# microsoft/ISLE

Hardware: AMD Instinct MI355X
Metric: docs/sec end-to-end ISLETrain (SVD+k-means), k=1000; top-k σ rel-err (higher is better)
Workload: dtype f32

## Files before the change

include/isle_hip.h:

```cpp
#ifndef ISLE_HIP_H
#define ISLE_HIP_H

#include <stddef.h>
#include <stdint.h>

#ifdef __cplusplus
extern "C" {
#endif

typedef struct isle_ctx isle_ctx;

enum {
  ISLE_OK = 0,
  ISLE_E_ARG = -1,
  ISLE_E_HIP = -2,
  ISLE_E_NOCONV = -3,
  ISLE_E_NUMERIC = -4,
  ISLE_E_COMM = -5
};

isle_ctx* isle_hip_create(int device_id);
void isle_hip_destroy(isle_ctx* ctx);
const char* isle_hip_last_error(isle_ctx* ctx);

int isle_hip_comm_unique_id(void* out128);
int isle_hip_comm_init(isle_ctx* ctx, int world_size, int rank, const void* unique_id128);

enum { ISLE_XCHG_ALLREDUCE_SUM = 0, ISLE_XCHG_ALLREDUCE_MAX = 1, ISLE_XCHG_ALLGATHER = 2 };
typedef int (*isle_host_exchange_fn)(void* user, int kind, void* buf, uint64_t count, int dtype);
int isle_hip_comm_init_host(isle_ctx* ctx, int world_size, int rank, isle_host_exchange_fn fn, void* user);

int isle_hip_plan_shards(uint64_t num_docs, const int64_t* offsets_CSC, int parts, uint64_t* bounds);

int isle_hip_upload_csc_u64(isle_ctx* ctx, uint64_t vocab_size, uint64_t num_docs, uint64_t nnz,
                            const float* vals, const uint64_t* rows, const int64_t* offsets,
                            uint64_t doc_offset, uint64_t docs_global);
int isle_hip_upload_csc_u32(isle_ctx* ctx, uint64_t vocab_size, uint64_t num_docs, uint64_t nnz,
                            const float* vals, const uint32_t* rows, const int64_t* offsets,
                            uint64_t doc_offset, uint64_t docs_global);

int isle_hip_upload_counts_u32(isle_ctx* ctx, uint64_t vocab_size, uint64_t num_docs, uint64_t nnz,
                               const float* counts, const uint32_t* rows, const int64_t* offsets,
                               uint64_t doc_offset, uint64_t docs_global);

int isle_hip_ingest_tdf(isle_ctx* ctx, const char* text, uint64_t nbytes, uint64_t vocab_size, uint64_t num_docs,
                        uint64_t max_entries, uint64_t* entries_read, uint64_t* nnz);
int isle_hip_get_A(isle_ctx* ctx, float* counts, uint32_t* rows, int64_t* offsets);

int isle_hip_threshold(isle_ctx* ctx, uint64_t num_topics, double sample_rate, uint64_t sample_seed,
                       uint64_t* docs_kept, uint64_t* nnz_kept, uint64_t* entries_above_threshold,
                       float* avg_doc_sz);

int isle_hip_get_B(isle_ctx* ctx, float* vals, uint32_t* rows, int64_t* offsets,
                   uint64_t* original_cols, float* zetas);
int isle_hip_shape(isle_ctx* ctx, uint64_t* vocab_size, uint64_t* num_docs, uint64_t* nnz,
                   uint64_t* doc_offset, uint64_t* docs_global);

int isle_hip_frobenius(isle_ctx* ctx, float* out);

int isle_hip_gram_apply(isle_ctx* ctx, const float* X_colmajor, int b, float* Z_colmajor);

int isle_hip_operator_form(isle_ctx* ctx, int* form);

int isle_hip_switch_info(int index, const char** name, const char** kind, const char** what);

int isle_hip_block_ks(isle_ctx* ctx, int nev, int ncv, int maxit, int blk, float tol, uint64_t seed,
                      float* evals, int* nconv, int* restarts, int* napplies);

int isle_hip_block_ks_dense(isle_ctx* ctx, const float* A_colmajor, uint64_t n, int nev, int ncv, int maxit, int blk,
                            float tol, uint64_t seed, const float* start_block, float* evals, float* U_colmajor,
                            int* nconv, int* nconv_ref_rule, int* restarts, int* napplies);

int isle_hip_get_U(isle_ctx* ctx, float* U_colmajor);
int isle_hip_set_U(isle_ctx* ctx, const float* U_colmajor, int k);

int isle_hip_eig_sym(isle_ctx* ctx, const float* S_colmajor, int n, float* evals_desc, float* vecs_colmajor);

int isle_hip_kmeanspp_projected(isle_ctx* ctx, int k, const uint64_t* inject_seeds, uint64_t rng_seed,
                                uint64_t* seeds_out, float* C_lowd, float* residual, int* rounds);

int isle_hip_host_rand(uint64_t seed, int n, uint32_t* out);

int isle_hip_get_min_dist(isle_ctx* ctx, float* min_dist);

int isle_hip_lloyds_projected(isle_ctx* ctx, int k, float* C_lowd, int max_reps, int* iters_run,
                              uint32_t* assign_out);

int isle_hip_lift_centers(isle_ctx* ctx, const float* in, int ld_in, int ncols, float* centers);

int isle_hip_lloyds_sparse(isle_ctx* ctx, int k, const float* centers_in, float* centers_out,
                           uint32_t* assign, int max_reps, int* iters_run);

int isle_hip_catchwords(isle_ctx* ctx, int num_topics, const uint32_t* assign, uint64_t r, double rho,
                        float* thresholds, int32_t* catch_topic, uint64_t* num_catchwords);

int isle_hip_topic_model(isle_ctx* ctx, int num_topics, uint64_t rank_threshold, float* model,
                         float* model_threshold, int32_t* top1, int32_t* top2, uint64_t* doc_topic_sums);
int isle_hip_get_doc_topic_sums(isle_ctx* ctx, int64_t* doc_offsets, uint32_t* topic, float* val);

int isle_hip_edge_topics(isle_ctx* ctx, const int64_t* pairs, int n, float primary_ratio, float* edge);

int isle_hip_topic_coherence(isle_ctx* ctx, int num_topics, int M, const uint32_t* top_words, double eps, double* coherence,
                             uint64_t* doc_freq, uint64_t* co_doc_freq);

int isle_hip_avg_topic_model(isle_ctx* ctx, int num_topics, float* model);

#define ISLE_MODEL_CATCH 0
#define ISLE_MODEL_AVG 1
#define ISLE_MODEL_HOST 2
#define ISLE_MODEL_LOADED 3

int isle_hip_model_top_words(isle_ctx* ctx, int which, const float* model_host, uint64_t vocab, int ncols, int n, uint32_t* ids, float* weights);

int isle_hip_topic_diversity(isle_ctx* ctx, int which, int num_topics, double* dist, double* avg);

#define ISLE_TEXT_SPARSE 0
#define ISLE_TEXT_DENSE 1
typedef int (*isle_text_sink_fn)(const char* bytes, uint64_t n, void* user);
int isle_hip_model_text(isle_ctx* ctx, int which, const float* model_host, uint64_t vocab, int ncols, int format, isle_text_sink_fn sink,
                        void* user, uint64_t* nbytes, uint64_t* nentries);
int isle_hip_edge_topics_text(isle_ctx* ctx, const int64_t* pairs, int n, float primary_ratio, int format, isle_text_sink_fn sink, void* user,
                              uint64_t* nbytes, uint64_t* nentries);
int isle_hip_entry_text(float w, int format, char* out16);

int isle_hip_load_model_text(isle_ctx* ctx, const char* text, uint64_t nbytes, uint64_t vocab, int ncols, int format, unsigned base,
                             uint64_t* nentries);
int isle_hip_get_loaded_model(isle_ctx* ctx, float* model_colmajor, uint64_t* vocab, int* ncols);
int isle_hip_parse_weight(const char* token, uint64_t n, int format, float* out);

int isle_hip_log_combinatorial(isle_ctx* ctx, float* out, uint64_t* max_words);

int isle_hip_distinct_top_five(isle_ctx* ctx, int n_m, const int32_t* m, uint64_t* num_distinct, uint64_t* num_quintuples, float* quintuples,
                               uint64_t* run_lengths, uint64_t* num_runs);

int isle_hip_top_five_count_rule(const uint64_t* run_lengths, uint64_t n_runs, int32_t m, uint64_t* out);

int isle_hip_infer(isle_ctx* ctx, uint64_t vocab_size, int num_topics, const float* model_by_word,
                   uint64_t num_docs, uint64_t nnz, const float* counts, const uint32_t* rows,
                   const int64_t* offsets, int iters, float Lf_guess, float avg_doc_sz, float* weights,
                   int32_t* top_topic, float* top_weight, float* llh, uint64_t* nconverged);

int isle_hip_infer_resident(isle_ctx* ctx, int which, const float* model_host, uint64_t vocab, int ncols, uint64_t doc_begin,
                            uint64_t doc_end, int iters, float Lf_guess, float min_weight, uint64_t chunk_docs, int32_t* top_topic,
                            float* top_weight, float* llh, uint64_t* nconverged, uint64_t* nentries);
int isle_hip_get_infer_entries(isle_ctx* ctx, int64_t* doc_offsets, uint32_t* topic, float* weight);
#define ISLE_DOCTEXT_ENTRIES 0
#define ISLE_DOCTEXT_TOP 1
int isle_hip_infer_text(isle_ctx* ctx, int what, uint64_t row_begin, uint64_t row_end, uint64_t number_base, isle_text_sink_fn sink,
                        void* user, uint64_t* nbytes, uint64_t* nlines);
int isle_hip_doc_line_text(uint64_t doc_number, uint64_t topic_number, float w, char* out40);
int isle_hip_avg_doc_sz(isle_ctx* ctx, float* out);

enum {
  ISLE_T_GRAM_PASS1 = 0,
  ISLE_T_GRAM_PASS2 = 1,
  ISLE_T_ORTHO = 2,
  ISLE_T_QR = 3,
  ISLE_T_EVD = 4,
  ISLE_T_ROTATE = 5,
  ISLE_T_PROJECT = 6,
  ISLE_T_KMPP = 7,
  ISLE_T_LLOYD_PROJ = 8,
  ISLE_T_SPARSE_ASSIGN = 9,
  ISLE_T_SPARSE_UPDATE = 10,
  ISLE_T_BAND_BUILD = 11,
  ISLE_T_COMM = 12,
  ISLE_T_THRESHOLD = 13,
  ISLE_T_POST = 14,
  ISLE_T_INGEST = 15,
  ISLE_T_INFER = 16,
  ISLE_T_LIFT = 17,
  ISLE_T_COUNT = 18
};
int isle_hip_timing_enable(isle_ctx* ctx, int on);
int isle_hip_timing_reset(isle_ctx* ctx);
int isle_hip_timing_get(isle_ctx* ctx, double* ms, uint64_t* launches);
int isle_hip_synchronize(isle_ctx* ctx);

#ifdef __cplusplus
}
#endif
#endif
```

isle_amd/_lib.py:

```python
import ctypes as C
import os

_HERE = os.path.dirname(os.path.abspath(__file__))
_LIB = None

_P, _I, _U64, _F = C.c_void_p, C.c_int, C.c_uint64, C.c_float
SYMBOLS = {
    "isle_hip_create": (_P, [_I]),
    "isle_hip_destroy": (None, [_P]),
    "isle_hip_last_error": (C.c_char_p, [_P]),
    "isle_hip_switch_info": (_I, [_I, _P, _P, _P]),
    "isle_hip_comm_unique_id": (_I, [_P]),
    "isle_hip_comm_init": (_I, [_P, _I, _I, _P]),
    "isle_hip_comm_init_host": (_I, [_P, _I, _I, _P, _P]),
    "isle_hip_plan_shards": (_I, [_U64, _P, _I, _P]),
    "isle_hip_upload_csc_u64": (_I, [_P, _U64, _U64, _U64, _P, _P, _P, _U64, _U64]),
    "isle_hip_upload_csc_u32": (_I, [_P, _U64, _U64, _U64, _P, _P, _P, _U64, _U64]),
    "isle_hip_upload_counts_u32": (_I, [_P, _U64, _U64, _U64, _P, _P, _P, _U64, _U64]),
    "isle_hip_ingest_tdf": (_I, [_P, _P, _U64, _U64, _U64, _U64, _P, _P]),
    "isle_hip_get_A": (_I, [_P, _P, _P, _P]),
    "isle_hip_threshold": (_I, [_P, _U64, C.c_double, _U64, _P, _P, _P, _P]),
    "isle_hip_get_B": (_I, [_P, _P, _P, _P, _P, _P]),
    "isle_hip_shape": (_I, [_P, _P, _P, _P, _P, _P]),
    "isle_hip_catchwords": (_I, [_P, _I, _P, _U64, C.c_double, _P, _P, _P]),
    "isle_hip_topic_model": (_I, [_P, _I, _U64, _P, _P, _P, _P, _P]),
    "isle_hip_get_doc_topic_sums": (_I, [_P, _P, _P, _P]),
    "isle_hip_edge_topics": (_I, [_P, _P, _I, _F, _P]),
    "isle_hip_topic_coherence": (_I, [_P, _I, _I, _P, C.c_double, _P, _P, _P]),
    "isle_hip_avg_topic_model": (_I, [_P, _I, _P]),
    "isle_hip_model_top_words": (_I, [_P, _I, _P, _U64, _I, _I, _P, _P]),
    "isle_hip_topic_diversity": (_I, [_P, _I, _I, _P, _P]),
    "isle_hip_model_text": (_I, [_P, _I, _P, _U64, _I, _I, _P, _P, _P, _P]),
    "isle_hip_edge_topics_text": (_I, [_P, _P, _I, _F, _I, _P, _P, _P, _P]),
    "isle_hip_entry_text": (_I, [_F, _I, _P]),
    "isle_hip_load_model_text": (_I, [_P, _P, _U64, _U64, _I, _I, C.c_uint, _P]),
    "isle_hip_get_loaded_model": (_I, [_P, _P, _P, _P]),
    "isle_hip_parse_weight": (_I, [_P, _U64, _I, _P]),
    "isle_hip_log_combinatorial": (_I, [_P, _P, _P]),
    "isle_hip_distinct_top_five": (_I, [_P, _I, _P, _P, _P, _P, _P, _P]),
    "isle_hip_top_five_count_rule": (_I, [_P, _U64, C.c_int32, _P]),
    "isle_hip_frobenius": (_I, [_P, _P]),
    "isle_hip_gram_apply": (_I, [_P, _P, _I, _P]),
    "isle_hip_operator_form": (_I, [_P, _P]),
    "isle_hip_infer": (_I, [_P, C.c_uint64, _I, _P, C.c_uint64, C.c_uint64, _P, _P, _P, _I, C.c_float, C.c_float, _P, _P, _P, _P, _P]),
    "isle_hip_infer_resident": (_I, [_P, _I, _P, _U64, _I, _U64, _U64, _I, _F, _F, _U64, _P, _P, _P, _P, _P]),
    "isle_hip_get_infer_entries": (_I, [_P, _P, _P, _P]),
    "isle_hip_infer_text": (_I, [_P, _I, _U64, _U64, _U64, _P, _P, _P, _P]),
    "isle_hip_doc_line_text": (_I, [_U64, _U64, _F, _P]),
    "isle_hip_avg_doc_sz": (_I, [_P, _P]),
    "isle_hip_block_ks": (_I, [_P, _I, _I, _I, _I, _F, _U64, _P, _P, _P, _P]),
    "isle_hip_block_ks_dense": (_I, [_P, _P, _U64, _I, _I, _I, _I, _F, _U64, _P, _P, _P, _P, _P, _P, _P]),
    "isle_hip_get_U": (_I, [_P, _P]),
    "isle_hip_set_U": (_I, [_P, _P, _I]),
    "isle_hip_eig_sym": (_I, [_P, _P, _I, _P, _P]),
    "isle_hip_kmeanspp_projected": (_I, [_P, _I, _P, _U64, _P, _P, _P, _P]),
    "isle_hip_get_min_dist": (_I, [_P, _P]),
    "isle_hip_host_rand": (_I, [_U64, _I, _P]),
    "isle_hip_lloyds_projected": (_I, [_P, _I, _P, _I, _P, _P]),
    "isle_hip_lift_centers": (_I, [_P, _P, _I, _I, _P]),
    "isle_hip_lloyds_sparse": (_I, [_P, _I, _P, _P, _P, _I, _P]),
    "isle_hip_timing_enable": (_I, [_P, _I]),
    "isle_hip_timing_reset": (_I, [_P]),
    "isle_hip_timing_get": (_I, [_P, _P, _P]),
    "isle_hip_synchronize": (_I, [_P]),
}


class IsleHipError(RuntimeError):
    pass


def library_path():
    return os.environ.get("ISLE_HIP_LIB") or os.path.join(_HERE, "libisle_hip.so")


def load_library():
    global _LIB
    if _LIB is not None:
        return _LIB
    path = library_path()
    if not os.path.exists(path):
        raise IsleHipError(
            "%s not found — build it with `make -C isle_amd/csrc` (or __graft_entry__.build()). "
            "There is no CPU fallback for the ISLE hot path." % path)
    lib = C.CDLL(path)
    for name, (res, args) in SYMBOLS.items():
        fn = getattr(lib, name)
        fn.restype = res
        fn.argtypes = args
    _LIB = lib
    return lib
```

isle_amd/csrc/api_kmeans.cpp:

```cpp
#include <algorithm>
#include <chrono>
#include <cmath>
#include <cstdarg>
#include <cstdlib>
#include <cstring>
#include <numeric>

#include "api_internal.h"

#ifndef ISLE_PROJ_FULL_NUM
#define ISLE_PROJ_FULL_NUM 1
#define ISLE_PROJ_FULL_DEN 3
#endif
static void choose_movers(const std::vector<float>& delta, int k, int group, int G, YyMovers* mv, std::vector<float>* gmax_excl,
                          const std::vector<uint32_t>* slot_of_id = nullptr ) {
  mv->n = 0;
  if ((int)delta.size() != k || k <= 16) return;
  std::vector<int> ord(k);
  std::iota(ord.begin(), ord.end(), 0);
  std::partial_sort(ord.begin(), ord.begin() + 11, ord.end(), [&](int a, int b) { return delta[a] > delta[b] || (delta[a] == delta[b] && a < b); });
  const float ref = delta[ord[10]];
  for (int j = 0; j < 10; ++j)
    if (delta[ord[j]] > 2.0f * ref && delta[ord[j]] > 1e-4f) mv->id[mv->n++] = (uint32_t)ord[j];
  if (!mv->n) return;
// ... 182 lines not shown
    else ISLECHK(kmpp_draw_by_ranks(c, rng, ndraw, inject != nullptr, dice, st, &grand, &last_md));
    new_added = 0;
    std::vector<uint64_t> fresh;
    for (int cc = 0; cc < ndraw && (int)centers.size() < k; ++cc) {
      const uint64_t nc = inject ? inject[centers.size()] : st.drawn[cc];
      if (std::find(centers.begin(), centers.end(), nc) == centers.end()) {
        centers.push_back(nc);
        fresh.push_back(nc);
        new_added++;
      }
    }
    if (new_added) ISLECHK(fetch_rows(c, fresh.data(), new_added, c->Cdev.p + (centers.size() - new_added) * (size_t)ldk));
    if (inject && new_added == 0) return isle_fail(c, ISLE_E_ARG, "injected seeds contain duplicates");
    if (rounds > 100 * k) return isle_fail(c, ISLE_E_NUMERIC, "k-means++ cannot find %d distinct seeds", k);
  }
  isle_host_mark("kmeanspp: rounds done");
  if (plan.track && c->kmpp_track && new_added > 0 && c->kmpp_track_seeds == k - new_added && D > 0) {
    HIPCHK(c, c->kmpp_best.reserve(D));
    HIPCHK(c, hipMemcpyAsync(c->kmpp_best.p, c->min_dist.p, D * sizeof(float), hipMemcpyDeviceToDevice, c->stream));
    ISLECHK(k_kmpp_update(c, c->P.p, c->pnorm.p, D, k, ldk, c->Cdev.p + (size_t)(k - new_added) * ldk, new_added, c->kmpp_best.p, k - new_added, true));
  }
  const size_t ch_bytes = (size_t)k * ldk * sizeof(float);
  HIPCHK(c, c->pin_stage.reserve(ch_bytes));
  HIPCHK(c, hipMemcpyAsync(c->pin_stage.p, c->Cdev.p, ch_bytes, hipMemcpyDeviceToHost, c->stream));
  HIPCHK(c, hipStreamSynchronize(c->stream));
  std::copy(centers.begin(), centers.end(), seeds_out);
  centres_unpack(C_lowd, reinterpret_cast<const float*>(c->pin_stage.p), k, ldk);
  if (residual) *residual = (float)(grand - last_md);
  if (rounds_out) *rounds_out = rounds;
  if (plan.track && c->kmpp_track && c->kmpp_track_seeds == k) {
    c->kmpp_C_host.assign(C_lowd, C_lowd + (size_t)k * k);
    c->kmpp_P_gen = c->P_gen;
    c->kmpp_track_k = k;
  }
  isle_host_mark("kmeanspp: exit");
  return 0;
}

extern "C" int isle_hip_get_min_dist(isle_ctx* c, float* out) {
  if (!c || !out) return ISLE_E_ARG;
  ISLECHK(isle_enter(c));
  if (c->D) HIPCHK(c, hipMemcpy(out, c->min_dist.p, c->D * sizeof(float), hipMemcpyDeviceToHost));
  return 0;
}

namespace {
struct StopRule {
  isle_ctx* c;
  int k;
  std::vector<long long> prev_sizes;
  bool have_prev = false;
  StopRule(isle_ctx* c_, int k_) : c(c_), k(k_), prev_sizes(k_, 0) {}
  int converged(const std::vector<long long>& sizes, const uint32_t* assign, bool* out) {
    bool changed = false;
    for (int i = 0; i < k; ++i)
      if (prev_sizes[i] != sizes[i]) changed = true;
    prev_sizes = sizes;
    if (!changed) {
      if (!have_prev) {
        changed = c->D_global > 0;
      } else {
        HIPCHK(c, c->flags.reserve(16));
        ISLECHK(k_compare_u32(c, assign, c->assign_prev.p, c->D, c->flags.p));
        ISLECHK(allreduce_sum<int>(c, c->flags.p, 1));
        uint32_t differ = 0;
        ISLECHK(isle_fetch_u32(c, reinterpret_cast<const uint32_t*>(c->flags.p), &c->pin_small()->stop_flag, &differ));
        changed = differ != 0;
      }
      HIPCHK(c, c->assign_prev.reserve(c->D ? c->D : 1));
      if (c->D) HIPCHK(c, hipMemcpyAsync(c->assign_prev.p, assign, c->D * sizeof(uint32_t), hipMemcpyDeviceToDevice, c->stream));
      have_prev = true;
    }
    *out = !changed;
    return 0;
  }
};
}

static int fetch_sizes(isle_ctx* c, int k, std::vector<long long>& sizes) {
  ISLECHK(allreduce_sum<int>(c, c->counts.p, k));
  std::vector<int> hv;
  int* h = c->pin_small()->cluster_sizes;
  if ((size_t)k * sizeof(int) > sizeof(c->pin_small()->cluster_sizes)) {
    hv.resize(k);
    h = hv.data();
  }
  HIPCHK(c, hipMemcpyAsync(h, c->counts.p, (size_t)k * sizeof(int), hipMemcpyDeviceToHost, c->stream));
  HIPCHK(c, hipStreamSynchronize(c->stream));
  sizes.assign(h, h + k);
  return 0;
}

static int fetch_delta(isle_ctx* c, const float* delta_dev, int k, std::vector<float>& out) {
  out.resize(k);
  float* h = c->pin_small()->movements;
  if ((size_t)k * sizeof(float) > sizeof(c->pin_small()->movements)) {
    HIPCHK(c, hipStreamSynchronize(c->stream));
    HIPCHK(c, hipMemcpy(out.data(), delta_dev, (size_t)k * sizeof(float), hipMemcpyDeviceToHost));
    return 0;
  }
  HIPCHK(c, hipMemcpyAsync(h, delta_dev, (size_t)k * sizeof(float), hipMemcpyDeviceToHost, c->stream));
  HIPCHK(c, hipStreamSynchronize(c->stream));
  memcpy(out.data(), h, (size_t)k * sizeof(float));
  return 0;
}

static int prepare_movers(isle_ctx* c, const std::vector<float>& delta, int k, int group, int G, const std::vector<uint32_t>* slot_of_id, YyMovers* mv,
                          std::vector<float>* excl) {
  choose_movers(delta, k, group, G, mv, excl, slot_of_id);
  if (!mv->n) return 0;
  HIPCHK(c, c->yy_gmax2.reserve(std::max(G, 64)));
  HIPCHK(c, hipMemcpyAsync(c->yy_gmax2.p, excl->data(), (size_t)G * sizeof(float), hipMemcpyHostToDevice, c->stream));
  return 0;
}

namespace {
struct ProjPlan {
  bool hamerly;
  bool tiles;
  int T, TL;
  bool from_kmpp;
  bool pt_sorted;
  bool delta_sums;
  bool movers;
};
struct ProjScalars {
  float* delta;
  HamTop* top;
  float* tmove;
};
}

static ProjPlan proj_plan(isle_ctx* c, int k, const float* C_lowd) {
  ProjPlan p;
  p.hamerly = !c->knob_on(KN_NO_HAMERLY) && (c->Pt_ready || c->Pt2_ready);
  p.T = (k + 31) / 32;
  p.TL = (p.T + 3) & ~3;
  p.tiles = p.hamerly && k > 224 && p.T <= 32 && !c->knob_is(KN_PROJ_BOUNDS, "hamerly");
  p.from_kmpp = p.tiles && c->kmpp_track_k == k && c->kmpp_P_gen == c->P_gen && c->P_ready && !c->knob_zero(KN_KMPP_TRACK) &&
                c->kmpp_C_host.size() == (size_t)k * k && memcmp(c->kmpp_C_host.data(), C_lowd, (size_t)k * k * sizeof(float)) == 0;
  p.pt_sorted = !c->knob_zero(KN_PT_SORT);
  p.delta_sums = !c->knob_is(KN_PROJ_SUMS, "fresh") && c->D < (1ull << 31);
  p.movers = !c->knob_zero(KN_YY_MOVERS) && c->D > 0;
  return p;
}

static int proj_reserve(isle_ctx* c, const ProjPlan& p, int k, ProjScalars* sc) {
  const uint64_t D = c->D;
  const int ldk = c->ldk;
  if (p.hamerly) {
    HIPCHK(c, c->hub.reserve(D ? D : 1));
    HIPCHK(c, c->hlb.reserve(D ? D : 1));
    HIPCHK(c, c->active.reserve(D + 1));
    HIPCHK(c, c->Pa.reserve((size_t)(D ? D : 1) * ldk));
    HIPCHK(c, c->pna.reserve(D ? D : 1));
    HIPCHK(c, c->Cold.reserve((size_t)k * ldk + k + 8));
  }
  if (p.tiles) {
    HIPCHK(c, c->ptlb.reserve((size_t)(D ? D : 1) * p.TL));
    HIPCHK(c, c->pneed.reserve(D ? D : 1));
    HIPCHK(c, c->pcand.reserve(D + 1));
    HIPCHK(c, c->small.reserve(4096));
  }
  if (p.delta_sums) HIPCHK(c, c->proj_counted.reserve(D ? D : 1));
  if (c->multi()) HIPCHK(c, c->Csum_local.reserve((size_t)k * ldk));
  sc->delta = p.hamerly ? c->Cold.p + (size_t)k * ldk : nullptr;
  sc->top = p.hamerly ? reinterpret_cast<HamTop*>(c->Cold.p + (size_t)k * ldk + round4(k)) : nullptr;
  sc->tmove = p.tiles ? c->small.p : nullptr;
  return 0;
}

static int proj_assign_first(isle_ctx* c, const ProjPlan& p, int k) {
  const uint64_t D = c->D;
  const int ldk = c->ldk;
  if (p.from_kmpp) return k_kmpp_to_tiles(c, D, k, c->pnorm.p, c->cnorm.p, c->kmpp_best.p, c->assign.p, c->hub.p, p.TL);
  if (p.tiles)
    return k_proj_assign_tiles(c, c->P.p, c->pnorm.p, D, k, ldk, c->Cdev.p, c->cnorm.p, c->assign.p, c->hub.p, c->ptlb.p, p.TL, nullptr, 0, nullptr, nullptr,
                               nullptr);
  return k_proj_assign(c, c->P.p, c->pnorm.p, D, k, ldk, c->Cdev.p, c->cnorm.p, c->assign.p, p.hamerly ? c->hub.p : nullptr,
                       p.hamerly ? c->hlb.p : nullptr);
}

static int debug_tile_stats(isle_ctx* c, int it, uint32_t na, int T) {
  const uint64_t D = c->D;
  std::vector<uint32_t> act(na), need(D);
  if (na) HIPCHK(c, hipMemcpy(act.data(), c->active.p, na * sizeof(uint32_t), hipMemcpyDeviceToHost));
  if (D) HIPCHK(c, hipMemcpy(need.data(), c->pneed.p, D * sizeof(uint32_t), hipMemcpyDeviceToHost));
  if (na > 256 && !c->knob_zero(KN_PT_SORT))
    std::stable_sort(act.begin(), act.end(), [&](uint32_t a, uint32_t b) { return need[a] < need[b]; });
  double tiles_sum = 0, union_sum = 0;
  for (uint32_t i = 0; i < na; i += 128) {
    uint32_t u = 0;
    for (uint32_t j = i; j < std::min(na, i + 128); ++j) {
      tiles_sum += __builtin_popcount(need[act[j]]);
      u |= need[act[j]];
    }
    union_sum += __builtin_popcount(u);
  }
  fprintf(stderr, "[tile bounds, projected] iter %d active %u of %llu, tiles per document %.1f, per workgroup (union) %.1f of %d\n", it, na,
          (unsigned long long)D, na ? tiles_sum / na : 0.0, na ? union_sum / ((na + 127) / 128) : 0.0, T);
  return 0;
}

static int proj_reassign_tiles(isle_ctx* c, const ProjPlan& p, const ProjScalars& sc, int k, int it, const std::vector<float>& pdelta_host) {
  const uint64_t D = c->D;
  const int ldk = c->ldk, T = p.T, TL = p.TL;
  uint32_t* nact = c->active.p + D;
  uint32_t* ncand = c->pcand.p + D;
  YyMovers mv;
  const float* tmove_use = sc.tmove;
  if (p.movers && c->gl_mode == 1 && c->band_ready && c->U_k == k) {
    std::vector<float> tm;
    ISLECHK(prepare_movers(c, pdelta_host, k, 32, T, nullptr, &mv, &tm));
    if (mv.n) {
      HIPCHK(c, c->Tmp.reserve((size_t)c->V * 32 + (size_t)16 * ldk));
      float* Cm = c->Tmp.p + (size_t)c->V * 32;
      for (int j = 0; j < mv.n; ++j)
        HIPCHK(c, hipMemcpyAsync(Cm + (size_t)j * ldk, c->Cdev.p + (size_t)mv.id[j] * ldk, (size_t)ldk * sizeof(float), hipMemcpyDeviceToDevice, c->stream));
      HIPCHK(c, hipStreamSynchronize(c->stream));
      HIPCHK(c, c->yy_mdots.reserve((size_t)D * mv.ld));
      ISLECHK(k_gemm_nn(c, c->Ucm.p, c->V, k, Cm, ldk, mv.n, c->Tmp.p, ISLE_T_LLOYD_PROJ));
      {
        TimeScope ts(c, ISLE_T_LLOYD_PROJ);
        ISLECHK(k_gl_thin(c, c->Tmp.p, mv.n, mv.ld, c->yy_mdots.p, true));
      }
      tmove_use = c->yy_gmax2.p;
    }
  }
  ISLECHK(k_pt_filter(c, p.pt_sorted ? nullptr : (c->members_valid ? c->members.p : nullptr), c->assign.p, c->hub.p, c->ptlb.p, T, TL, sc.delta, tmove_use,
                      c->pneed.p, c->pcand.p, ncand, mv, c->yy_mdots.p, c->cnorm.p, c->pnorm.p));
  ISLECHK(k_pt_tighten(c, c->P.p, c->pnorm.p, ldk, c->Cdev.p, c->cnorm.p, c->assign.p, c->pcand.p, ncand, c->hub.p, c->ptlb.p, T, TL, c->pneed.p,
                       c->active.p, nact));
  uint32_t na = 0;
  ISLECHK(isle_fetch_u32(c, nact, &c->pin_small()->active_count, &na));
  if (c->knob_on(KN_DEBUG_HAMERLY)) ISLECHK(debug_tile_stats(c, it, na, T));
  if ((uint64_t)na * ISLE_PROJ_FULL_DEN > (uint64_t)D * ISLE_PROJ_FULL_NUM && k_proj_full_by_gemm(c, D, k))
    return k_proj_assign_tiles(c, c->P.p, c->pnorm.p, D, k, ldk, c->Cdev.p, c->cnorm.p, c->assign.p, c->hub.p, c->ptlb.p, TL, nullptr, 0, nullptr, nullptr,
                               nullptr);
  return k_proj_assign_tiles(c, c->P.p, c->pnorm.p, D, k, ldk, c->Cdev.p, c->cnorm.p, c->assign.p, c->hub.p, c->ptlb.p, TL, c->active.p, na, c->pneed.p, c->Pa.p,
                             c->pna.p);
}

static int proj_reassign_hamerly(isle_ctx* c, const ProjScalars& sc, int k, int it) {
  uint32_t* nact = c->active.p + c->D;
  ISLECHK(k_hamerly_filter(c, nullptr, c->assign.p, c->hub.p, c->hlb.p, sc.delta, sc.top, c->active.p, nact, ISLE_T_LLOYD_PROJ));
  uint32_t na = 0;
  ISLECHK(isle_fetch_u32(c, nact, &c->pin_small()->active_count, &na));
  if (c->knob_on(KN_DEBUG_HAMERLY)) fprintf(stderr, "[hamerly, projected] iter %d active %u of %llu\n", it, na, (unsigned long long)c->D);
  return k_proj_assign_active(c, c->P.p, c->pnorm.p, k, c->ldk, c->Cdev.p, c->cnorm.p, c->active.p, na, c->Pa.p, c->pna.p, c->assign.p, c->hub.p, c->hlb.p);
}

static int proj_update_centres(isle_ctx* c, const ProjPlan& p, int k, int it, std::vector<long long>& sizes) {
  const uint64_t D = c->D;
  const int ldk = c->ldk;
  float* sums = c->multi() ? c->Csum_local.p : c->Csum.p;
  bool updated = false;
  if (p.delta_sums && it > 0) ISLECHK(k_proj_accumulate_delta(c, c->P.p, D, k, ldk, c->assign.p, c->proj_counted.p, sums, c->counts.p, &updated));
  if (!updated) {
    ISLECHK(k_proj_accumulate(c, c->P.p, D, k, ldk, c->assign.p, sums, c->counts.p));
    if (p.delta_sums && D) HIPCHK(c, hipMemcpyAsync(c->proj_counted.p, c->assign.p, D * sizeof(uint32_t), hipMemcpyDeviceToDevice, c->stream));
  } else {
    c->members_valid = false;
  }
  if (c->multi()) HIPCHK(c, hipMemcpyAsync(c->Csum.p, sums, (size_t)k * ldk * sizeof(float), hipMemcpyDeviceToDevice, c->stream));
  ISLECHK(allreduce_sum<float>(c, c->Csum.p, (size_t)k * ldk));
  ISLECHK(fetch_sizes(c, k, sizes));
  if (p.hamerly) HIPCHK(c, hipMemcpyAsync(c->Cold.p, c->Cdev.p, (size_t)k * ldk * sizeof(float), hipMemcpyDeviceToDevice, c->stream));
  return k_proj_finalize(c, c->Csum.p, c->counts.p, k, ldk, c->Cdev.p);
}

static int proj_movements(isle_ctx* c, const ProjPlan& p, const ProjScalars& sc, int k, std::vector<float>& pdelta_host) {
  ISLECHK(k_rownorms_diff(c, c->Cdev.p, c->Cold.p, k, k, c->ldk, sc.delta));
  if (!p.tiles) return k_ham_delta(c, sc.delta, k, sc.top);
  ISLECHK(k_yy_delta(c, sc.delta, k, p.T, 32, sc.tmove));
  return fetch_delta(c, sc.delta, k, pdelta_host);
}

extern "C" int isle_hip_lloyds_projected(isle_ctx* c, int k, float* C_lowd, int max_reps, int* iters_run, uint32_t* assign_out) {
  if (!c || !C_lowd || k < 1) return ISLE_E_ARG;
  ISLECHK(isle_enter(c));
  isle_host_mark("lloyds_projected: entry");
  ISLECHK(ensure_P(c, k));
  const ProjPlan plan = proj_plan(c, k, C_lowd);
  const uint64_t D = c->D;
  const int ldk = c->ldk;
  HIPCHK(c, c->Cdev.reserve((size_t)k * ldk));
  HIPCHK(c, c->Csum.reserve((size_t)k * ldk));
  HIPCHK(c, c->cnorm.reserve(k));
  HIPCHK(c, c->counts.reserve(k));
  HIPCHK(c, c->assign.reserve(D ? D : 1));
  c->assign_valid = false;
  const size_t ch_bytes = (size_t)k * ldk * sizeof(float);
  HIPCHK(c, c->pin_stage.reserve(ch_bytes));
  float* Ch = reinterpret_cast<float*>(c->pin_stage.p);
  centres_pack(Ch, C_lowd, k, ldk);
  HIPCHK(c, hipMemcpyAsync(c->Cdev.p, Ch, ch_bytes, hipMemcpyHostToDevice, c->stream));
  HIPCHK(c, hipStreamSynchronize(c->stream));
  isle_host_mark("lloyds_projected: centres uploaded");
  ProjScalars sc;
  ISLECHK(proj_reserve(c, plan, k, &sc));
  c->kmpp_track_k = 0;
  if (c->knob_on(KN_DEBUG_HAMERLY)) fprintf(stderr, "[projected Lloyd] first assignment %s\n", plan.from_kmpp ? "taken from the k-means++ rounds" : "computed");
  StopRule stop(c, k);
  int it = 0;
  std::vector<float> pdelta_host;
  isle_host_mark("lloyds_projected: loop starts");
  for (; it < max_reps; ++it) {
    ISLECHK(k_rownorms(c, c->Cdev.p, k, k, ldk, c->cnorm.p));
    if (it == 0 || !plan.hamerly) ISLECHK(proj_assign_first(c, plan, k));
    else if (plan.tiles) ISLECHK(proj_reassign_tiles(c, plan, sc, k, it, pdelta_host));
    else ISLECHK(proj_reassign_hamerly(c, sc, k, it));
    ISLECHK(k_count_sizes(c, c->assign.p, D, k, c->counts.p));
    std::vector<long long> sizes;
    ISLECHK(proj_update_centres(c, plan, k, it, sizes));
    if (plan.hamerly && it + 1 < max_reps) ISLECHK(proj_movements(c, plan, sc, k, pdelta_host));
    bool conv = false;
    ISLECHK(stop.converged(sizes, c->assign.p, &conv));
    if (conv) {
      ++it;
      break;
    }
  }
  isle_host_mark("lloyds_projected: loop done");
  HIPCHK(c, hipMemcpyAsync(Ch, c->Cdev.p, ch_bytes, hipMemcpyDeviceToHost, c->stream));
  if (assign_out && D) HIPCHK(c, hipMemcpyAsync(assign_out, c->assign.p, D * sizeof(uint32_t), hipMemcpyDeviceToHost, c->stream));
  HIPCHK(c, hipStreamSynchronize(c->stream));
  centres_unpack(C_lowd, Ch, k, ldk);
  if (iters_run) *iters_run = it;
  isle_host_mark("lloyds_projected: exit");
  return 0;
}

static int install_centers(isle_ctx* c, int ncols) {
  const int ld = round4(ncols);
  HIPCHK(c, c->centers_rm.reserve((size_t)c->V * ld));
  HIPCHK(c, hipMemsetAsync(c->centers_rm.p, 0, (size_t)c->V * ld * sizeof(float), c->stream));
  ISLECHK(k_transpose(c, c->centers_cm.p, c->V, ncols, c->V, c->centers_rm.p, ld));
  c->centers_ready = true;
  c->centers_k = ncols;
  return 0;
}

extern "C" int isle_hip_lift_centers(isle_ctx* c, const float* in, int ld_in, int ncols, float* centers) {
  if (!c || !in || ncols < 1) return ISLE_E_ARG;
  ISLECHK(isle_enter(c));
  if (c->U_k == 0 || ld_in < c->U_k) return isle_fail(c, ISLE_E_ARG, "lift: need U and ld_in >= k");
  isle_host_mark("lift: entry");
  HIPCHK(c, c->Csum.reserve((size_t)ld_in * ncols));
  {
    const size_t in_bytes = (size_t)ld_in * ncols * sizeof(float);
    HIPCHK(c, c->pin_stage.reserve(in_bytes));
    memcpy(c->pin_stage.p, in, in_bytes);
    HIPCHK(c, hipMemcpyAsync(c->Csum.p, c->pin_stage.p, in_bytes, hipMemcpyHostToDevice, c->stream));
  }
  HIPCHK(c, c->centers_cm.reserve((size_t)c->V * ncols));
  ISLECHK(k_gemm_nn(c, c->Ucm.p, c->V, c->U_k, c->Csum.p, ld_in, ncols, c->centers_cm.p, ISLE_T_LIFT));
  ISLECHK(install_centers(c, ncols));
  HIPCHK(c, c->lift_C.reserve((size_t)ld_in * ncols));
  HIPCHK(c, hipMemcpyAsync(c->lift_C.p, c->Csum.p, (size_t)ld_in * ncols * sizeof(float), hipMemcpyDeviceToDevice, c->stream));
  c->lift_ld = ld_in;
  c->lift_k = ncols;
  c->lift_valid = true;
  if (centers) HIPCHK(c, hipMemcpyAsync(centers, c->centers_cm.p, (size_t)c->V * ncols * sizeof(float), hipMemcpyDeviceToHost, c->stream));
  HIPCHK(c, hipStreamSynchronize(c->stream));
  isle_host_mark("lift: exit");
  return 0;
}

namespace {
struct SparsePlan {
  bool hamerly , yinyang;
  int G;
  int yy_mode;
  bool fused;
  bool by_members;
  bool fused_first;
  bool via_projection;
  bool regroup;
  bool movers;
};
struct SparseScalars {
  float* delta;
  float* cn_max;
  HamTop* top;
  float* gmax;
};
struct SparseGroups {
  YyMap ymap;
  std::vector<uint32_t> slot_of_id_host;
};
}
static SparseScalars sparse_scalars(isle_ctx* c, int k) {
  return {c->Csum.p, c->Csum.p + 2 * k + 8, reinterpret_cast<HamTop*>(c->Csum.p + 2 * k + 12), c->Csum.p + 2 * k + 16};
}

static bool first_scratch_had(isle_ctx* c, int k) {
  if (c->dotsT.reserve((size_t)c->D * k) == hipSuccess) return true;
  (void)hipGetLastError();
  fprintf(stderr, "[isle_hip] lloyds_sparse: no memory for the %.1f GB product of the first assignment; taking the sparse route\n",
          (double)c->D * k * sizeof(float) / 1e9);
  return false;
}

static SparsePlan sparse_plan(isle_ctx* c, int k, int ld) {
  const uint64_t D = c->D;
  SparsePlan p;
  p.hamerly = !c->knob_on(KN_NO_HAMERLY) && !c->knob_is(KN_KMEANS_BOUNDS, "none");
  p.yinyang = p.hamerly && !c->knob_is(KN_KMEANS_BOUNDS, "hamerly");
  p.G = (k + 7) / 8;
  int yy_mode_env = -1;
  if (const char* e = c->knob(KN_YY_MODE)) yy_mode_env = !strcmp(e, "doc") ? 0 : !strcmp(e, "docg") ? 1 : !strcmp(e, "group") ? 2 : -1;
  p.yy_mode = !p.yinyang ? 0 : p.G > 256 ? 0 : yy_mode_env >= 0 ? yy_mode_env : (p.G >= 32 ? 2 : 0);
  p.fused = p.yy_mode == 2 && !c->knob_zero(KN_YY_FUSED);
  const char* yord = c->knob(KN_YY_ORDER);
  p.by_members = !p.yinyang || !p.yy_mode || (yord ? strcmp(yord, "doc") != 0 : !p.fused);
  p.movers = p.fused && !c->knob_zero(KN_YY_MOVERS);
  const double t_dense = 2.0 * (double)D * k * k / 130e12, t_sparse = (double)((k + 7) / 8) * (double)c->nnz * 2.8e-12;
  p.fused_first = p.yinyang && k_gemm_assign_fused_ok(c, D, k, k);
  const bool dense_pays = k <= 384 || (t_dense < t_sparse && (p.fused_first || isle_scratch_ok(c, c->dotsT.cap, (double)D * k * sizeof(float))));
  p.via_projection = c->lift_valid && c->lift_k == k && c->U_k == k && c->P_ready && (c->Pt_ready || c->Pt2_ready) && c->ldk == ld && D > 0 &&
                     (dense_pays || c->knob_is(KN_FIRST_ASSIGN, "projection")) && !c->knob_is(KN_FIRST_ASSIGN, "sparse");
  p.regroup = p.yinyang && p.yy_mode == 2 && p.via_projection && p.fused_first && !c->knob_zero(KN_YY_REGROUP);
  return p;
}

static int sparse_regroup_tables(isle_ctx* c, int k, int G, SparseGroups* g) {
  TimeScope ts(c, ISLE_T_SPARSE_ASSIGN);
  float* cn_pin = c->pin_small()->centre_norms;
  HIPCHK(c, hipMemcpyAsync(cn_pin, c->cnorm.p, (size_t)k * sizeof(float), hipMemcpyDeviceToHost, c->stream));
  HIPCHK(c, hipStreamSynchronize(c->stream));
  std::vector<float> cnh(cn_pin, cn_pin + k);
  std::vector<uint32_t> id_of_slot((size_t)8 * G, 0xffffffffu);
  std::iota(id_of_slot.begin(), id_of_slot.begin() + k, 0u);
  std::stable_sort(id_of_slot.begin(), id_of_slot.begin() + k, [&](uint32_t a, uint32_t b) { return cnh[a] < cnh[b]; });
  g->slot_of_id_host.assign(k, 0u);
  for (int s2 = 0; s2 < k; ++s2) g->slot_of_id_host[id_of_slot[s2]] = (uint32_t)s2;
  ISLECHK(k_yy_map_upload(c, id_of_slot.data(), g->slot_of_id_host.data(), k, G, &g->ymap));
  HIPCHK(c, c->yy_cns.reserve((size_t)8 * G));
  return 0;
}

static int sparse_assign_first_via_projection(isle_ctx* c, const SparsePlan& p, const SparseScalars& sc, int k, int ld, const YyMap& ymap, const float* cn_grp) {
  const uint64_t D = c->D;
  TimeScope ts(c, ISLE_T_SPARSE_ASSIGN);
  if (p.yinyang && p.fused_first) {
    ISLECHK(k_max_f32(c, c->cnorm.p, k, sc.cn_max));
    const float* liftC = c->lift_C.p;
    if (p.regroup) {
      HIPCHK(c, c->yy_liftC.reserve((size_t)k * c->lift_ld));
      ISLECHK(k_yy_rows_by_slot(c, ymap, k, c->lift_C.p, c->lift_ld, c->yy_liftC.p));
      liftC = c->yy_liftC.p;
    }
    ISLECHK(k_gemm_assign_yy(c, c->Pt_ready ? c->Pt.p : nullptr, c->P.p, c->ldk, c->pnorm.p, D, k, liftC, c->lift_ld, k, p.G, cn_grp, c->dnorm.p, sc.cn_max,
                             c->assign.p, c->hub.p, c->yglb.p, ISLE_T_SPARSE_ASSIGN, c->Pt2_ready ? c->Pt2.p : nullptr,
                             c->Pt2_ready && c->Pt2_pos ? c->dperm.p : nullptr));
    if (p.regroup) ISLECHK(k_yy_labels_to_ids(c, ymap, c->assign.p, D));
    return 0;
  }
  HIPCHK(c, c->dotsT.reserve((size_t)D * k));
  ISLECHK(k_ensure_pt(c));
  ISLECHK(k_gemm_nn_assign(c, c->Pt.p, D, k, c->lift_C.p, c->lift_ld, k, c->dotsT.p, ISLE_T_SPARSE_ASSIGN));
  if (p.yinyang) {
    ISLECHK(k_max_f32(c, c->cnorm.p, k, sc.cn_max));
    return k_dots_assign_cm(c, c->dotsT.p, k, p.G, c->cnorm.p, c->dnorm.p, sc.cn_max, c->assign.p, c->hub.p, c->yglb.p);
  }
  c->P_ready = false;
  c->Pt_ready = false;
  c->Pt2_ready = false;
  if (ld != k) HIPCHK(c, hipMemsetAsync(c->P.p, 0, (size_t)D * ld * sizeof(float), c->stream));
  ISLECHK(k_transpose(c, c->dotsT.p, D, (uint64_t)k, D, c->P.p, (uint64_t)ld));
  return k_dots_assign(c, k, ld, c->cnorm.p, c->dnorm.p, c->assign.p, c->hub.p, c->hlb.p, 0);
}

static int debug_yy_margins(isle_ctx* c, int it, int G, const YyMap& ymap) {
  unsigned long long hh[16];
  ISLECHK(k_yy_dbg_margins(c, c->active.p, c->active.p + c->D, c->assign.p, c->hub.p, c->yglb.p, G, ymap, hh));
  fprintf(stderr, "[yinyang] iter %d active by (ub - smallest group bound) < 1e-6 | 1e-5 | 1e-4 | 1e-3 | 1e-2 | 1e-1 | 1 | more:  own group", it);
  for (int b = 0; b < 8; ++b) fprintf(stderr, " %llu", hh[b]);
  fprintf(stderr, ";  another group");
  for (int b = 0; b < 8; ++b) fprintf(stderr, " %llu", hh[8 + b]);
  fprintf(stderr, "\n");
  return 0;
// ... 206 lines not shown
```

isle_amd/csrc/common.h:

```cpp
#pragma once
#include <hip/hip_runtime.h>
#include <rccl/rccl.h>

#include <atomic>
#include <cstdint>
#include <cstdio>
#include <functional>
#include <string>
#include <thread>
#include <vector>

struct IsleLaunchRefused {
  const char* file = nullptr;
  int line = 0;
  unsigned long long threads = 0;
};
inline IsleLaunchRefused& isle_launch_refused() {
  static thread_local IsleLaunchRefused r;
  return r;
}
inline bool isle_launch_fits(dim3 g, dim3 b, const char* file, int line) {
  const unsigned long long blocks = (unsigned long long)g.x * g.y * g.z, threads = blocks * ((unsigned long long)b.x * b.y * b.z);
  if (threads < (1ull << 32)) return true;
  IsleLaunchRefused& r = isle_launch_refused();
// ... 116 lines not shown
  const char* knob(int id) const { return knob_set[id] ? knob_val[id].c_str() : nullptr; }
  bool knob_on(int id) const { return knob_set[id]; }
  bool knob_is(int id, const char* v) const { return knob_set[id] && knob_val[id] == v; }
  bool knob_zero(int id) const { return knob_set[id] && atoi(knob_val[id].c_str()) == 0; }
  int device = 0;
  size_t total_mem = 0;
  hipStream_t stream = nullptr;
  std::string err;
  int num_cus = 256;

  char* pin = nullptr;
  PinBuf pin_stage;
  static constexpr size_t PIN_MAIL = 0, PIN_MAIL_SLOT = 1u << 20, PIN_SMALL = 2u << 20, PIN_BYTES = (2u << 20) + (256u << 10);
  IslePinSmall* pin_small() const { return reinterpret_cast<IslePinSmall*>(pin + PIN_SMALL); }

  ncclComm_t comm = nullptr;
  int world = 1, rank = 0;
  isle_host_exchange_fn host_xchg = nullptr;
  void* host_xchg_user = nullptr;
  bool multi() const { return comm != nullptr || host_xchg != nullptr; }
  std::atomic<uint32_t> wd_issued{0};
  volatile uint32_t* wd_done = nullptr;
  std::atomic<int> comm_dead{0};
  std::atomic<bool> wd_stop{false};
  std::thread wd_thread;
  double wd_timeout_s = 300.0;

  uint64_t V = 0, D = 0, nnz = 0, doc_offset = 0, D_global = 0;
  DevBuf<float> vals;
  DevBuf<uint32_t> rows;
  DevBuf<int64_t> offs;

  uint64_t a_V = 0, a_D = 0, a_nnz = 0, a_doc_offset = 0, a_D_global = 0;
  bool a_ready = false;
  DevBuf<float> a_cnt;
  DevBuf<uint32_t> a_rows;
  DevBuf<int64_t> a_offs;
  DevBuf<uint16_t> a_q;
  DevBuf<uint32_t> a_hist;
  DevBuf<uint32_t> a_kept, a_flag;
  DevBuf<float> a_wgt;
  DevBuf<int64_t> a_off_all, a_col_of, a_scan;
  DevBuf<float> zetas;
  DevBuf<uint64_t> original_cols;
  bool b_from_threshold = false;
  float a_avg = 0.f;
  bool a_avg_valid = false;

  DevBuf<float> a_nv;
  DevBuf<int32_t> p_cluster_of;
  DevBuf<uint32_t> p_cnt, p_min, p_slot;
  DevBuf<float> p_thr;
  DevBuf<uint64_t> p_seg_id, p_seg_off, p_counters;
  DevBuf<uint32_t> p_seg_len, p_seg_rank, p_seg_cur;
  DevBuf<float> p_segvals;
  DevBuf<int32_t> p_catch;
  DevBuf<uint32_t> p_nz;
  DevBuf<int64_t> p_dts_off;
  DevBuf<uint32_t> p_dts_topic;
  DevBuf<float> p_dts_val;
  uint64_t p_dts_n = 0;
  DevBuf<int32_t> p_top1, p_top2;
  DevBuf<uint32_t> p_tcnt;
  DevBuf<int64_t> p_toff;
  DevBuf<float> p_mthr;
  DevBuf<float> p_model;
  DevBuf<uint64_t> p_avg_acc;
  DevBuf<float> p_avg_model;
  DevBuf<uint32_t> mt_sizes;
  DevBuf<uint64_t> mt_offs, mt_blk, mt_stat;
  DevBuf<unsigned char> mt_text[2];
  PinBuf mt_pin[2];
  DevBuf<int64_t> inf_off;
  DevBuf<uint32_t> inf_topic;
  DevBuf<float> inf_weight;
  DevBuf<int32_t> inf_top_topic;
  DevBuf<float> inf_top_weight;
  uint64_t inf_docs = 0, inf_n = 0;
  bool inf_valid = false;
  int p_k = 0;
  DevBuf<float> ml_model;
  uint64_t ml_V = 0;
  int ml_cols = 0;
  bool ml_ready = false;
  bool p_catch_ready = false, p_model_ready = false, p_avg_ready = false, assign_valid = false;

  bool band_ready = false;
  uint32_t band_rows = 0;
  uint32_t nbands = 0;
  uint32_t chunk_cols = 0;
  DevBuf<uint32_t> bcol;
  DevBuf<float> bval;
  DevBuf<int64_t> seg_off;
  DevBuf<float> Zpart;

  int gl_mode = -1;
  GlSide gl1, gl2;
  DevBuf<float> rowval;
  DevBuf<int> gl_flag;
  DevBuf<uint32_t> dperm, dpos, wperm, wpos;
  DevBuf<uint64_t> gl_key_a, gl_key_b;
  DevBuf<uint32_t> gl_val_a, gl_val_b;
  DevBuf<uint32_t> gl_bst;
  DevBuf<uint16_t> gl_cellcnt;
  DevBuf<uint32_t> gl_srsum, gl_sbase;
  DevBuf<uint32_t> gl_fb_cnt, gl_fb_tmp;
  DevBuf<int64_t> gl_fb_off;
  DevBuf<uint16_t> gl_scnt;
  DevBuf<uint32_t> gl_biglist;
  DevBuf<uint32_t> ccount;
  DevBuf<uint32_t> ccounted;
  DevBuf<int64_t> gl_scan;
  DevBuf<unsigned long long> gl_blocktot;
  DevBuf<uint32_t> gl_slab0, gl_nch;
  uint32_t gl_block_items = 4096;
  DevBuf<float> gl_Xs, gl_part;
  DevBuf<float> gl_pscratch;
  DevBuf<uint32_t> rs_hist;
  DevBuf<int64_t> rs_hist_off, rs_scratch;

  DevBuf<float> Xrm, Yrm, Zrm;
  DevBuf<float> Xcm, Zcm;

  DevBuf<float> basis;
  DevBuf<float> Fbuf;
  DevBuf<float> Tmp;
  DevBuf<double> part;
  DevBuf<float> coef;
  DevBuf<double> gram;
  DevBuf<double> pq_part, pq_R1;
  DevBuf<float> pq_T;
  DevBuf<int> pq_meta;
  DevBuf<float> small;
  DevBuf<double> jacW, jacV;
  DevBuf<double> jacS;
  DevBuf<float> Wf;
  DevBuf<float> evd_in;
  int U_k = 0;
  DevBuf<float> Ucm;
  DevBuf<float> Urm;
  int ldk = 0;

  DevBuf<float> P;
  DevBuf<float> pnorm;
  bool P_ready = false;
  DevBuf<float> Pt;
  DevBuf<float> dotsT;
  DevBuf<uint4> gemm_b3;
  DevBuf<float> yy_gmax2;
  DevBuf<float> yy_mdots;
  DevBuf<float> cmax_buf;
  DevBuf<uint32_t> ga_redo;
  DevBuf<float> ga_bn;
  DevBuf<float> ga_rows, ga_rown;
  bool ts_open = false;
  bool roctx_open = false;
  uint32_t ga_last_redo = 0;
  DevBuf<float> assign_part;
  DevBuf<float> lift_C;
  int lift_ld = 0, lift_k = 0;
  bool lift_valid = false;
  bool Pt_ready = false;
  DevBuf<uint4> Pt2;
  bool Pt2_ready = false;
  bool Pt2_pos = false;
  DevBuf<float> min_dist;
  DevBuf<double> cum;
  DevBuf<double> scan_blk;
  DevBuf<float> Cdev;
  DevBuf<float> cnorm;
  DevBuf<float> Csum;
  DevBuf<uint32_t> assign, assign_prev;
  DevBuf<int> counts;
  DevBuf<uint32_t> members;
  DevBuf<int> moff;
  bool members_valid = false;
  DevBuf<int> flags;
  DevBuf<float> centers_rm;
  DevBuf<float> centers_cm;
  bool centers_ready = false;
  int centers_k = 0;
  DevBuf<float> dnorm;
  DevBuf<float> hub, hlb;
  DevBuf<float> yglb;
  DevBuf<float> ptlb;
  DevBuf<uint32_t> pneed;
  DevBuf<uint32_t> pcand;
  DevBuf<int> seg_desc;
  DevBuf<float> seg_part;
  DevBuf<uint32_t> proj_counted;
  DevBuf<uint32_t> proj_nch;
  DevBuf<float> proj_dpart;
  DevBuf<float> Csum_local;
  DevBuf<uint32_t> active;
  DevBuf<unsigned long long> dbg_cnt;
  DevBuf<uint32_t> kmpp_arg;
  DevBuf<float> kmpp_m2a;
  DevBuf<float> kmpp_tmin;
  DevBuf<float> kmpp_best;
  bool kmpp_track = false;
  int kmpp_track_seeds = 0;
  int kmpp_track_k = 0;
  uint64_t P_gen = 0, kmpp_P_gen = 0;
  std::vector<float> kmpp_C_host;
  DevBuf<float> yy_cg;
  DevBuf<uint32_t> yy_map;
  DevBuf<float> yy_cns;
  DevBuf<float> yy_liftC;
  DevBuf<uint32_t> yy_own, yy_res;
  DevBuf<unsigned long long> yy_need;
  DevBuf<uint32_t> yy_cnt, yy_off;
  DevBuf<uint8_t> yy_pgrp;
  DevBuf<float> centers_old;
  DevBuf<float> Pa, pna, Cold;

  hipEvent_t ks_ev[2] = {nullptr, nullptr};
  hipEvent_t ks_ev_ready[2] = {nullptr, nullptr};
  hipStream_t copy_stream = nullptr;
  DevBuf<float> ks_mail;
  DevBuf<float> ks_top;
  DevBuf<float> ks_gather;

  std::vector<std::pair<const void*, int>> lds_attr;
  bool td_persist_failed = false;

  bool timing = false;
  uint32_t timing_mask = 0xffffffffu;
  std::vector<isle_event_pair> ev_used;
  std::vector<isle_event_pair> ev_free;
  double t_ms[ISLE_T_COUNT] = {0};
  uint64_t t_n[ISLE_T_COUNT] = {0};
};

static_assert(sizeof(IslePinSmall) <= isle_ctx::PIN_BYTES - isle_ctx::PIN_SMALL, "the small page-locked region holds every slot");

int isle_fail(isle_ctx* c, int code, const char* fmt, ...);
void isle_trim_derived(isle_ctx* c, uint64_t D, uint64_t nnz);
int isle_max_lds(isle_ctx* c, const void* fn, int bytes);
bool isle_scratch_ok(isle_ctx* c, size_t have_elems, double bytes);
void isle_refresh_knobs(isle_ctx* c);
int isle_enter(isle_ctx* c);
void isle_host_mark(const char* what);

#define HIPCHK(ctx, call)                                                                   \
  do {                                                                                      \
    hipError_t e__ = (call);                                                                \
    if ((ctx) && (ctx)->comm_dead.load(std::memory_order_relaxed))                          \
      return isle_fail((ctx), ISLE_E_COMM, "%s:%d: a collective did not complete within %.0f s (ISLE_COMM_TIMEOUT_S): the communicator was aborted", __FILE__, __LINE__, (ctx)->wd_timeout_s); \
    if (e__ != hipSuccess)                                                                  \
      return isle_fail((ctx), ISLE_E_HIP, "%s:%d %s -> %s", __FILE__, __LINE__, #call, hipGetErrorString(e__)); \
    if (isle_launch_refused().file) {                                                       \
      const IsleLaunchRefused r__ = isle_launch_refused();                                  \
      isle_launch_refused() = IsleLaunchRefused();                                          \
      return isle_fail((ctx), ISLE_E_ARG, "%s:%d: kernel launch of %llu threads refused (2^32 or more do not run)", r__.file, r__.line, r__.threads); \
    }                                                                                       \
  } while (0)

#define ISLECHK(call)            \
  do {                           \
    int rc__ = (call);           \
    if (rc__ != 0) return rc__;  \
  } while (0)

inline int isle_fetch_u32(isle_ctx* c, const uint32_t* dev, uint32_t* slot, uint32_t* out) {
  HIPCHK(c, hipMemcpyAsync(slot, dev, sizeof(uint32_t), hipMemcpyDeviceToHost, c->stream));
  HIPCHK(c, hipStreamSynchronize(c->stream));
  *out = *slot;
  return 0;
}

struct TimeScope {
  isle_ctx* c;
  isle_event_pair ep;
  bool on;
  bool marker = false;
  TimeScope(isle_ctx* c_, int fam);
  ~TimeScope();
};

static inline uint64_t isle_scan_scratch(uint64_t n) { return (n + 4095) / 4096 + 1; }
static inline int cdiv(long a, long b) { return (int)((a + b - 1) / b); }

enum { ISLE_DT_F32 = 0, ISLE_DT_F64 = 1, ISLE_DT_I32 = 2, ISLE_DT_U32 = 3, ISLE_DT_U64 = 4 };
int isle_allreduce(isle_ctx* c, void* buf, size_t count, int dtype, bool max_op = false);
int isle_allgather(isle_ctx* c, const void* send, void* recv, size_t count_per_rank, int dtype);
int k_pack_rm(isle_ctx* c, const float* Xcm, uint64_t V, int b, int BP, float* Xrm);
int k_unpack_cm(isle_ctx* c, const float* Zrm, uint64_t V, int b, int BP, float* Zcm);
int k_gram_pass1(isle_ctx* c, int BP);
int k_gram_pass2(isle_ctx* c, int BP);
int k_band_build(isle_ctx* c);
int k_band_build_chunked(isle_ctx* c);
int k_dots_assign(isle_ctx* c, int k, int ldk, const float* cn, const float* dn, uint32_t* assign, float* ub, float* lb, int G);
int k_dots_assign_cm(isle_ctx* c, const float* dotsT, int k, int G, const float* cn, const float* dn, const float* cn_max_dev, uint32_t* assign, float* ub,
                     float* lb);
int k_frobenius(isle_ctx* c, double* out_host);
int k_spmm_wide_project(isle_ctx* c, const float* Mrm, int k, int ldk, float* P, float* norms, void* A2pos = nullptr, bool* a2_done = nullptr);
int k_spmm_wide_assign(isle_ctx* c, const float* Mrm, int k, int ldk, const float* cn, const float* dn, uint32_t* assign,
                       const uint32_t* perm , const uint32_t* nslots = nullptr ,
                       float* ub = nullptr, float* lb = nullptr, int G = 0 );
struct YyMovers {
  int n = 0, ld = 0;
  uint32_t id[10] = {};
};
struct YyMap {
  const uint32_t* id_of_slot = nullptr;
  const uint32_t* slot_of_id = nullptr;
#if defined(__HIPCC__)
  __device__ inline uint32_t id(uint32_t s) const { return id_of_slot ? id_of_slot[s] : s; }
  __device__ inline uint32_t slot(uint32_t i) const { return slot_of_id ? slot_of_id[i] : i; }
#endif
};
int k_yy_filter_tighten(isle_ctx* c, const uint32_t* order, const uint32_t* assign, float* ub, float* glb, int G, const float* delta_dev,
                        const float* gmax_dev, uint32_t* active, uint32_t* nactive, const float* Cg, int k, int ld, const float* cn, const float* dn,
                        const float* cn_max, const YyMovers& mv, const float* Crm, const YyMap& map = YyMap(), const float* cn_by_id = nullptr);
int k_yy_map_upload(isle_ctx* c, const uint32_t* id_of_slot_host, const uint32_t* slot_of_id_host, int k, int G, YyMap* map);
int k_yy_gather_by_slot(isle_ctx* c, const YyMap& map, int k, int G, const float* cn, float* cn_slot);
int k_yy_rows_by_slot(isle_ctx* c, const YyMap& map, int k, const float* in, int ld, float* out);
int k_yy_labels_to_ids(isle_ctx* c, const YyMap& map, uint32_t* assign, uint64_t D);
int k_yy_filter(isle_ctx* c, const uint32_t* order, const uint32_t* assign, float* ub, float* glb, int G, const float* delta_dev, const float* gmax_dev,
                uint32_t* active, uint32_t* nactive);
int k_yy_dbg_margins(isle_ctx* c, const uint32_t* active, const uint32_t* nactive, const uint32_t* assign, const float* ub, const float* glb, int G,
                     const YyMap& map, unsigned long long* hist_host);
int k_yy_pack_groups(isle_ctx* c, const float* Crm, int ld, int G, const YyMap& map = YyMap());
int k_yy_scan(isle_ctx* c, const float* Crm, const float* Cg , int k, int ld, int G, const float* cn, const float* dn, const float* cn_max_dev,
              const uint32_t* active, const uint32_t* nactive, uint32_t* assign, float* ub, float* glb, unsigned long long* dbg = nullptr,
              const YyMap& map = YyMap());
int k_yy2_assign(isle_ctx* c, const float* Cg, int k, int ld, int G, const float* cn, const float* dn, const float* cn_max_dev, const uint32_t* active,
                 const uint32_t* nactive, uint32_t* assign, float* ub, float* glb, bool* done, unsigned long long* pairs_out = nullptr, bool pre_tightened = false,
                 const YyMap& map = YyMap());
struct HamTop {
  uint32_t amax;
  float d1, d2, pad;
};
int k_ham_delta(isle_ctx* c, float* delta_dev , int k, HamTop* top_dev);
int k_hamerly_filter(isle_ctx* c, const uint32_t* order, const uint32_t* assign, float* ub, float* lb, const float* delta_dev, const HamTop* top_dev,
                     uint32_t* active, uint32_t* nactive, int fam = ISLE_T_SPARSE_ASSIGN);
int k_csc_validate(isle_ctx* c, unsigned long long* err_host2);
int k_doc_norms(isle_ctx* c, float* dn);
int k_centers_from_rows(isle_ctx* c, const uint32_t* assign, int k, int ldk, float* Crm, bool first_of_run = true);
int k_pt_filter(isle_ctx* c, const uint32_t* order, const uint32_t* assign, float* ub, float* tlb, int T, int TL, const float* delta_dev,
                const float* tmove_dev, uint32_t* need, uint32_t* active, uint32_t* nactive, const YyMovers& mv, const float* mdots, const float* cn, const float* pn);
int k_pt_tighten(isle_ctx* c, const float* P, const float* pn, int ldk, const float* C, const float* cn, const uint32_t* assign, const uint32_t* cand,
                 const uint32_t* ncand, float* ub, const float* tlb, int T, int TL, uint32_t* need, uint32_t* active, uint32_t* nactive);
int k_gl_detect(isle_ctx* c);
int k_centers_counts(isle_ctx* c, const uint32_t* assign, int k, int ldk, float* Crm, bool fresh);
int k_gl_build(isle_ctx* c);
int k_gl_wide(isle_ctx* c, const float* Mrm, int k, int ld, float* Out, float* norms = nullptr ,
              void* A2pos = nullptr , bool* a2_done = nullptr);
int k_gl_thin(isle_ctx* c, const float* Wcm, int nc, int ld, float* Out, bool by_position = false);
int k_gl_apply_cm(isle_ctx* c, const float* Xcm, int b, int BP, float* Zcm);
int k_gl_panel_width(const isle_ctx* c);

int k_th_stats(isle_ctx* c, uint64_t* tokens_nz_dev);
int k_th_round_hist(isle_ctx* c, float avg, uint32_t maxv);
int k_th_zetas(isle_ctx* c, uint32_t maxv, uint64_t count_gr, uint64_t count_eq);
int k_th_count(isle_ctx* c, bool with_weights);
int k_th_drop(isle_ctx* c, const uint8_t* drop_dev);
int k_th_scans(isle_ctx* c);
int k_th_emit(isle_ctx* c, uint64_t doc_base);

int k_sort_pairs_u64(isle_ctx* c, uint64_t* key_a, uint32_t* val_a, uint64_t* key_b, uint32_t* val_b, uint64_t n, int key_bits, bool* in_a);
int k_ingest_tdf(isle_ctx* c, const unsigned char* text_dev, uint64_t n, uint64_t V, uint64_t D, uint64_t* entries_read, uint64_t* err_out);

int k_infer(isle_ctx* c, uint64_t V, int k, const float* model_by_word, uint64_t D, uint64_t nnz, const float* counts, const uint32_t* rows,
            const int64_t* offs, int iters, float Lfguess, float avg_doc_sz, float* weights, int32_t* top_topic, float* top_weight, float* llh,
            uint64_t* nconverged);
int k_infer_rowok(isle_ctx* c, const float* M, uint64_t V, int k, unsigned char* ok);
int k_infer_docs(isle_ctx* c, const float* M, int k, uint64_t D, const float* counts, const uint32_t* rows, const int64_t* offs,
                 const unsigned char* ok, uint32_t* fw, float* fa, uint32_t* nkeep, int iters, float Lfguess, float avg_doc_sz, float* weights,
                 int32_t* top_topic, float* top_weight, float* llh, unsigned int* nconverged);

int k_infer_resident(isle_ctx* c, const float* model_cm_dev, int k, uint64_t doc_begin, uint64_t doc_end, int iters, float Lfguess,
                     float avg_doc_sz, float min_weight, uint64_t chunk_docs, int32_t* top_topic, float* top_weight, float* llh,
                     uint64_t* nconverged, uint64_t* nentries);

int k_post_normalize(isle_ctx* c, float avg);
int k_post_cluster_of(isle_ctx* c, const uint32_t* assign_dev, bool identity);
int k_post_catch_thresholds(isle_ctx* c, uint32_t k, uint32_t r, const int* sizes_dev);
int k_post_find_catchwords(isle_ctx* c, uint32_t k, double rho, uint64_t* ncatch_host);
int k_post_thr_colmajor(isle_ctx* c, uint32_t k, float* out_dev);
int k_post_doc_topic_sums(isle_ctx* c, uint32_t k, uint64_t* n_out);
int k_post_model_thresholds(isle_ctx* c, uint32_t k, uint32_t rank);
int k_post_model(isle_ctx* c, uint32_t k);
int k_post_edge(isle_ctx* c, const int64_t* pairs_dev, int n, float a, float b, float* edge_dev);

constexpr uint64_t ISLE_TEXT_CHUNK_BYTES = 16ull << 20;
int k_model_text(isle_ctx* c, const float* model_dev, uint64_t V, uint64_t ncols, const int64_t* pairs_dev, float a, float b, int format,
                 isle_text_sink_fn sink, void* user, uint64_t* nbytes, uint64_t* nentries);
int k_text_pump(isle_ctx* c, const char* who, const uint64_t* offs_dev, uint64_t ntiles, uint64_t total, uint64_t group, isle_text_sink_fn sink,
                void* user, const std::function<int(uint64_t, uint64_t, unsigned char*)>& write);

int k_infer_text(isle_ctx* c, int what, uint64_t row_begin, uint64_t row_end, uint64_t base, isle_text_sink_fn sink, void* user, uint64_t* nbytes,
                 uint64_t* nlines);

int k_load_model_text(isle_ctx* c, const unsigned char* text_dev, uint64_t n, uint64_t V, uint32_t ncols, int format, unsigned base, float* model_dev,
                      uint64_t* nentries, uint64_t* err_key);

int k_coherence_counts(isle_ctx* c, const std::vector<uint32_t>& U, const std::vector<uint32_t>& part_off, const std::vector<uint32_t>& part_hi,
                       std::vector<uint32_t>& counts, int* passes);

int k_avg_model(isle_ctx* c, uint32_t k);
int k_model_top_words(isle_ctx* c, const float* model_dev, uint64_t V, uint32_t ncols, int n, uint32_t* ids_dev, float* weights_dev);
int k_topic_diversity(isle_ctx* c, const float* model_dev, uint64_t V, uint32_t k, double* dist_dev, double* abar_dev, int32_t* finite_dev,
                      uint32_t* kprime);

int k_log_combinatorial(isle_ctx* c, float* out, uint64_t* max_words);
int k_top_five_runs(isle_ctx* c, uint64_t* n_out, std::vector<uint64_t>& runs, float* tuples);

int k_ensure_pt(isle_ctx* c);
int k_vtf(isle_ctx* c, const float* Vb, uint64_t n, int m, const float* F, int b, float* coef , uint64_t ld = 0);
int k_update(isle_ctx* c, float* F, uint64_t n, int b, const float* Vb, int m, const float* coef, uint64_t ld = 0);
int k_panel_qr(isle_ctx* c, float* F, uint64_t n, int w, float* Qdst, float* R_host , int* rank_out);
int k_panel_qr_kernels(isle_ctx* c, float* F, uint64_t n, int w, float* Qdst, int* meta_dev , float* Rout_dev );
int k_randu(isle_ctx* c, float* F, uint64_t count, uint64_t seed);
int k_gemm_nn(isle_ctx* c, const float* A, uint64_t M, int K, const float* B, int ldb, int N, float* C, int family = ISLE_T_ROTATE);
int k_gemm_nn_assign(isle_ctx* c, const float* A, uint64_t M, int K, const float* B, int ldb, int N, float* C, int family);
bool k_gemm_assign_fused_ok(isle_ctx* c, uint64_t M, int K, int N);
int k_gemm_assign_yy(isle_ctx* c, const float* A, const float* Arm, int lda_rm, const float* an, uint64_t M, int K, const float* B, int ldb, int N, int G,
                     const float* cn, const float* dn, const float* cn_max, uint32_t* assign, float* ub, float* lb, int family, const void* A2 = nullptr,
                     const uint32_t* map2 = nullptr );
int k_gemm_assign_tiles(isle_ctx* c, const float* A, const float* Arm, int lda_rm, uint64_t M, int K, const float* B, int ldb, int N, int TL, const float* cn,
                        const float* pn, const float* cmax, uint32_t* assign, float* ub, float* tlb, int family, const uint32_t* map0 = nullptr,
                        const void* A2 = nullptr, const uint32_t* map2 = nullptr);
int k_gemm_split_a(isle_ctx* c, const float* A, uint64_t M, int K, void* A2);
size_t k_gemm_split_a_bytes(uint64_t M, int K);
int k_transpose(isle_ctx* c, const float* in, uint64_t rows, uint64_t cols, uint64_t ld_in, float* out, uint64_t ld_out);
int k_jacobi_eig(isle_ctx* c, const float* S_host, int n, float* evals_host, float* vecs_dev );
int k_eig_small(isle_ctx* c, const float* S_host, int n, float* evals_host, float* vecs_dev , int nvec);
int k_colnorms_rm(isle_ctx* c, const float* Mrm, uint64_t rows, int k, int ldk, float* out, const float* Sub = nullptr);
int k_scale_centers(isle_ctx* c, float* Crm, uint64_t rows, int k, int ldk, const int* counts);

int k_tridiag_eig(isle_ctx* c, const float* S_host, int n, float* evals_host, float* vecs_dev, int nvec);

int k_member_lists(isle_ctx* c, const uint32_t* assign, uint64_t D, int k, const int* counts_dev, int* max_out, std::vector<int>* counts_host = nullptr);
int k_member_lists_dev(isle_ctx* c, const uint32_t* assign, uint64_t D, int k, const int* counts_dev);
int k_yy_delta(isle_ctx* c, float* delta_dev, int k, int G, int group, float* gmax_dev, const uint32_t* id_of_slot = nullptr);
int k_max_f32(isle_ctx* c, const float* v, int n, float* out_dev);
int k_compact_rows(isle_ctx* c, const float* P, const float* pn, int ldk, const uint32_t* active, uint32_t n, float* Pa, float* pna);
int k_kmpp_update(isle_ctx* c, const float* P, const float* pn, uint64_t D, int k, int ldk, const float* newC, int nc, float* min_dist, int s_old = -1,
                  bool track = false);
int k_kmpp_to_tiles(isle_ctx* c, uint64_t D, int k, const float* pn, const float* cn, const float* best, uint32_t* assign, float* ub, int TL);
int k_scan_f2d(isle_ctx* c, const float* in, uint64_t n, double* cum );
int k_search(isle_ctx* c, const double* cum, uint64_t n, const double* dice_dev, int nd, uint64_t* out_dev);
int k_search_args(isle_ctx* c, const double* cum, uint64_t n, const double* dice_host, int nd , uint64_t* out_dev);
int k_fetch_rows(isle_ctx* c, const float* P, int ldk, const uint64_t* local_ids , int n, float* dst);
int k_pack2(isle_ctx* c, const double* a, const float* b , double* out2);
int k_search_frac(isle_ctx* c, const double* cum, uint64_t n, const float* last , const double* frac_host, int nd ,
                  uint64_t* out_dev );
int k_proj_assign(isle_ctx* c, const float* P, const float* pn, uint64_t D, int k, int ldk, const float* C, const float* cn, uint32_t* assign,
                  float* ub = nullptr, float* lb = nullptr);
int k_proj_assign_active(isle_ctx* c, const float* P, const float* pn, int k, int ldk, const float* C, const float* cn,
                         const uint32_t* active, uint32_t n, float* Pa, float* pna, uint32_t* assign, float* ub, float* lb);
bool k_proj_full_by_gemm(isle_ctx* c, uint64_t D, int k);
int k_proj_assign_tiles(isle_ctx* c, const float* P, const float* pn, uint64_t D, int k, int ldk, const float* C, const float* cn, uint32_t* assign,
                        float* ub, float* tlb, int TL, const uint32_t* active, uint32_t n, const uint32_t* need, float* Pa, float* pna);
int k_rownorms_diff(isle_ctx* c, const float* A, const float* B, int rows, int k, int ldk, float* out);
int k_rownorms(isle_ctx* c, const float* M, int rows, int k, int ldk, float* out);
int k_proj_accumulate(isle_ctx* c, const float* P, uint64_t D, int k, int ldk, const uint32_t* assign, float* Csum, int* counts);
int k_proj_accumulate_delta(isle_ctx* c, const float* P, uint64_t D, int k, int ldk, const uint32_t* assign, uint32_t* counted, float* Csum,
                            const int* counts, bool* done);
int k_proj_finalize(isle_ctx* c, const float* Csum, const int* counts, int k, int ldk, float* C);
int k_count_sizes(isle_ctx* c, const uint32_t* assign, uint64_t D, int k, int* counts);
int k_compare_u32(isle_ctx* c, const uint32_t* a, const uint32_t* b, uint64_t n, int* flag_dev);
int k_fill_f32(isle_ctx* c, float* p, uint64_t n, float v);
```

isle_amd/csrc/dense.hip:

```cpp
#include <algorithm>
#include <cstdlib>

#include "gemm_f32.h"
#include "gemm_bf16x3.h"

#include "common.h"
#include "gridbar.h"
#include "hamerly.h"

typedef float floatx16 __attribute__((ext_vector_type(16)));

constexpr int VTF_CG = 32;
constexpr int vtf_rc(int BT) { return BT <= 12 ? 1024 : (BT <= 16 ? 512 : 256); }

template <int BT>
__global__ __launch_bounds__(256) void vtf_partial_k(const float* __restrict__ Vb, uint64_t n, uint64_t ld, int m, const float* __restrict__ F,
                                                      int b, double* __restrict__ part ) {
  constexpr int VTF_RC = vtf_rc(BT);
  __shared__ float Fs[BT][VTF_RC];
  const uint64_t r0 = (uint64_t)blockIdx.x * VTF_RC;
  const int rc = (int)min((uint64_t)VTF_RC, n - r0);
  for (int idx = threadIdx.x; idx < BT * VTF_RC; idx += 256) {
    const int j = idx / VTF_RC, r = idx - j * VTF_RC;
    Fs[j][r] = (j < b && r < rc) ? F[(uint64_t)j * ld + r0 + r] : 0.f;
// ... 662 lines not shown
  HIPCHK(c, c->gemm_b3.reserve((size_t)3 * isle_gemm3::kp8_of(K) * isle_gemm3::np_of<Gemm3Huge>(N)));
  HIPCHK(c, isle_gemm3::launch<Gemm3Huge>(c->stream, A, M, K, B, ldb, N, c->gemm_b3.p, isle_gemm3::StoreC{C, M}));
  return 0;
}

constexpr float GA_ETA_TRUNC = 4.65e-5f;
static float ga_eta(int K) { return GA_ETA_TRUNC + 1.05f * 9.f * (float)((K + 15) / 16) * 5.9604645e-8f; }
struct AssignRec {
  float m1;
  uint32_t i1;
  float m2, ax, r2;
};
struct YyGroupEpi {
  static constexpr int kGroup = 8;
  const float* __restrict__ cn;
  const float* __restrict__ dn;
  const float* __restrict__ cn_max;
  float* __restrict__ lb;
  int G, nslot;
  AssignRec* __restrict__ part;
  const uint32_t* __restrict__ map;
  float eta;
  const float* __restrict__ an;
  const float* __restrict__ bmax;
  __device__ inline uint64_t doc(uint64_t m) const { return map ? map[m] : m; }
  __device__ inline float rowdata(uint64_t m) const { return dn[doc(m)]; }
  __device__ inline float dist(float dot, int col, float dnd) const { return fabsf((-2.0f * dot + cn[col]) + dnd); }
  __device__ inline float aux(int) const { return 0.f; }
  __device__ inline void group(uint64_t m, int g, float dnd, float m1, uint32_t, float, float) const {
#ifdef GA_ABLATE_LB
    if (g >= 0) return;
#endif
    const float E = ISLE_SLACK_REL * (dnd + *cn_max), sE = sqrtf(E);
    const float eps = eta > 0.f ? eta * (an[doc(m)] + *bmax) : 0.f;
    lb[doc(m) * (uint64_t)G + g] = yy_slack_down_sq(fmaxf(m1 - eps, 0.f), E, sE);
  }
  __device__ inline void slot(uint64_t m, int sl, float, float m1, uint32_t i1, float m2, float ax, float r2) const {
    part[m * (uint64_t)nslot + sl] = AssignRec{m1, i1, m2, ax, r2};
  }
};
struct AssignPick {
  float best, m2, ax, run2;
  uint32_t bidx;
};
__device__ inline AssignPick assign_pick(const AssignRec* __restrict__ part, size_t row, int nslot) {
  AssignPick p{3.4e38f, 3.4e38f, 0.f, 3.4e38f, 0xffffffffu};
  for (int sl0 = 0; sl0 < nslot; sl0 += 8) {
    AssignRec rr[8];
#pragma unroll
    for (int u = 0; u < 8; ++u) rr[u] = part[row * nslot + min(sl0 + u, nslot - 1)];
#pragma unroll
    for (int u = 0; u < 8; ++u) {
      if (sl0 + u < nslot) {
        const AssignRec r = rr[u];
        if (r.m1 < p.best) {
          p.run2 = fminf(fminf(p.run2, p.best), r.r2);
          p.best = r.m1;
          p.bidx = r.i1;
          p.m2 = r.m2;
          p.ax = r.ax;
        } else {
          p.run2 = fminf(p.run2, r.m1);
        }
      }
    }
  }
  return p;
}
__global__ __launch_bounds__(256) void yy_first_combine_k(const AssignRec* __restrict__ part, int nslot, uint32_t n, int G, const float* __restrict__ dn,
                                                          const float* __restrict__ cn_max, uint32_t* __restrict__ assign, float* __restrict__ ub,
                                                          float* __restrict__ lb, const uint32_t* __restrict__ map, float eta,
                                                          const float* __restrict__ an, const float* __restrict__ bmax,
                                                          uint32_t* __restrict__ redo, uint32_t* __restrict__ nredo) {
  const uint32_t i = blockIdx.x * 256 + threadIdx.x;
  const bool in = i < n;
  bool open = false;
  if (in) {
    const uint32_t d = map ? map[i] : i;
    const AssignPick p = assign_pick(part, i, nslot);
    const float eps = eta > 0.f ? eta * (an[d] + *bmax) : 0.f;
    const float E = ISLE_SLACK_REL * (dn[d] + *cn_max), sE = sqrtf(E);
    lb[(size_t)d * G + p.bidx / 8] = yy_slack_down_sq(fmaxf(p.m2 - eps, 0.f), E, sE);
    const float u = sqrtf(p.best + eps);
    ub[d] = u + fminf(sE, E / fmaxf(u, 1e-30f));
    assign[d] = p.bidx;
    open = eta > 0.f && p.run2 - p.best <= 2.f * eps;
  }
  if (eta > 0.f) {
    const uint32_t at = block_append_slot(open, nredo);
    if (open) redo[at] = map ? map[i] : i;
  }
}
struct TileEpi {
  static constexpr int kGroup = 32;
  const float* __restrict__ cn;
  const float* __restrict__ pn;
  const float* __restrict__ cmax;
  float* __restrict__ lb;
  int TL, nslot;
  AssignRec* __restrict__ part;
  const uint32_t* __restrict__ map;
  float eta;
  __device__ inline uint64_t doc(uint64_t m) const { return map ? map[m] : m; }
  __device__ inline float rowdata(uint64_t m) const { return pn[doc(m)]; }
  __device__ inline float dist(float dot, int col, float nd) const { return fabsf((-2.0f * dot + cn[col]) + nd); }
  __device__ inline float aux(int col) const { return cn[col]; }
  __device__ inline void group(uint64_t m, int T, float nd, float m1, uint32_t, float, float tc) const {
    float uu, ll;
    const float lo = fmaxf(m1 - eta * (nd + *cmax), 0.f);
    hamerly_store_bounds(lo, lo, nd + tc, &uu, &ll);
    lb[doc(m) * (uint64_t)TL + T] = ll;
  }
  __device__ inline void slot(uint64_t m, int sl, float, float m1, uint32_t i1, float m2, float ax, float r2) const {
    part[m * (uint64_t)nslot + sl] = AssignRec{m1, i1, m2, ax, r2};
  }
};
__global__ __launch_bounds__(256) void tiles_combine_k(const AssignRec* __restrict__ part, int nslot, uint32_t n, int TL, const float* __restrict__ pn,
                                                       const float* __restrict__ cmax_p, uint32_t* __restrict__ assign, float* __restrict__ ub,
                                                       float* __restrict__ lb, const uint32_t* __restrict__ map, float eta,
                                                       uint32_t* __restrict__ redo, uint32_t* __restrict__ nredo) {
  const uint32_t i = blockIdx.x * 256 + threadIdx.x;
  const bool in = i < n;
  bool open = false;
  if (in) {
    const uint32_t d = map ? map[i] : i;
    const AssignPick p = assign_pick(part, i, nslot);
    const float nd = pn[d];
    const float eps = eta * (nd + *cmax_p);
    assign[d] = p.bidx;
    float uu, ll, l2;
    hamerly_store_bounds(p.best + eps, fmaxf(p.m2 - eps, 0.f), nd + p.ax, &uu, &l2);
    hamerly_store_bounds(p.best + eps, p.best + eps, nd + *cmax_p, &uu, &ll);
    ub[d] = uu;
    lb[(size_t)d * TL + (p.bidx >> 5)] = l2;
    open = eta > 0.f && p.run2 - p.best <= 2.f * eps;
  }
  if (eta > 0.f) {
    const uint32_t at = block_append_slot(open, nredo);
    if (open) redo[at] = map ? map[i] : i;
  }
}
bool k_gemm_assign_fused_ok(isle_ctx* c, uint64_t M, int K, int N) {
  return !c->knob_zero(KN_GEMM_BF16X3) && !c->knob_zero(KN_GEMM_EPILOGUE) && N >= 64 && K >= 32 && (M + 255) / 256 * (uint64_t)((N + 255) / 256) >= 512 &&
         M < (1ull << 32);
}
using Gemm2Huge = isle_gemm3::Cfg<2, 2, 4, 4, 4, 16, 2>;
using Gemm2Dma = isle_gemm3::CfgDma<2, 16>;
int k_gemm_split_a(isle_ctx* c, const float* A, uint64_t M, int K, void* A2) {
  HIPCHK(c, isle_gemm3::split_a(c->stream, A, M, K, A2, Gemm2Dma::TK));
  return 0;
}
size_t k_gemm_split_a_bytes(uint64_t M, int K) { return isle_gemm3::a2_units(M, K, Gemm2Dma::TK) * 16; }
template <class MakeEpi, class Combine>
static int gemm_assign_two_pass(isle_ctx* c, const float* A, const float* Arm, int lda_rm, const float* rown, uint64_t M, int K, const float* B, int ldb, int N,
                                MakeEpi make, Combine combine, const uint32_t* map0 = nullptr ,
                                const void* A2 = nullptr ,
                                const uint32_t* map2 = nullptr ) {
  auto need_a = [&]() -> int {
    if (A) return 0;
    ISLECHK(k_ensure_pt(c));
    A = c->Pt.p;
    return 0;
  };
  const int nslot = (N + 63) / 64;
  static_assert(sizeof(AssignRec) == 20, "");
  const char* gt = c->knob(KN_GEMM_TERMS);
  const bool two = !(gt && atoi(gt) == 3) && Arm != nullptr;
  HIPCHK(c, c->gemm_b3.reserve((size_t)3 * isle_gemm3::kp8_of(K) * isle_gemm3::np_of<Gemm3Huge>(N)));
  HIPCHK(c, c->assign_part.reserve((size_t)M * nslot * 5));
  AssignRec* part = reinterpret_cast<AssignRec*>(c->assign_part.p);
  if (!two) {
    ISLECHK(need_a());
    HIPCHK(c, isle_gemm3::launch<Gemm3Huge>(c->stream, A, M, K, B, ldb, N, c->gemm_b3.p, make(part, map0, 0.f)));
    combine(part, (uint32_t)M, map0, 0.f, nullptr, nullptr);
    HIPCHK(c, hipGetLastError());
    return 0;
  }
  const float eta2 = ga_eta(K);
  HIPCHK(c, c->ga_redo.reserve(M + 1));
  uint32_t* nredo = c->ga_redo.p + M;
  HIPCHK(c, hipMemsetAsync(nredo, 0, sizeof(uint32_t), c->stream));
  if (A2 && !c->knob_zero(KN_GEMM_DMA)) {
    HIPCHK(c, isle_gemm3::launch_dma<Gemm2Dma>(c->stream, A2, M, K, B, ldb, N, c->gemm_b3.p, make(part, map2 ? map2 : map0, eta2)));
    combine(part, (uint32_t)M, map2 ? map2 : map0, eta2, c->ga_redo.p, nredo);
  } else {
    ISLECHK(need_a());
    HIPCHK(c, isle_gemm3::launch<Gemm2Huge>(c->stream, A, M, K, B, ldb, N, c->gemm_b3.p, make(part, map0, eta2)));
    combine(part, (uint32_t)M, map0, eta2, c->ga_redo.p, nredo);
  }
  HIPCHK(c, hipGetLastError());
  uint32_t n = 0;
  ISLECHK(isle_fetch_u32(c, nredo, &c->pin_small()->redo_count, &n));
  c->ga_last_redo = n;
  if (c->knob_on(KN_DEBUG_HAMERLY)) fprintf(stderr, "[assignment product] the two-term pass left %u of %llu rows open\n", n, (unsigned long long)M);
  if (n == 0) return 0;
  if ((uint64_t)n * 4 > M) {
    ISLECHK(need_a());
    HIPCHK(c, isle_gemm3::launch<Gemm3Huge>(c->stream, A, M, K, B, ldb, N, c->gemm_b3.p, make(part, map0, 0.f)));
    combine(part, (uint32_t)M, map0, 0.f, nullptr, nullptr);
    HIPCHK(c, hipGetLastError());
    return 0;
  }
  HIPCHK(c, c->ga_rows.reserve((size_t)n * lda_rm));
  HIPCHK(c, c->ga_rown.reserve(n));
  ISLECHK(k_compact_rows(c, Arm, rown, lda_rm, c->ga_redo.p, n, c->ga_rows.p, c->ga_rown.p));
  HIPCHK(c, isle_gemm3::launch<Gemm3Huge>(c->stream, c->ga_rows.p, (uint64_t)n, K, B, ldb, N, c->gemm_b3.p, make(part, c->ga_redo.p, 0.f)));
  combine(part, n, c->ga_redo.p, 0.f, nullptr, nullptr);
  HIPCHK(c, hipGetLastError());
  return 0;
}
int k_gemm_assign_yy(isle_ctx* c, const float* A, const float* Arm, int lda_rm, const float* an, uint64_t M, int K, const float* B, int ldb, int N, int G,
                     const float* cn, const float* dn, const float* cn_max, uint32_t* assign, float* ub, float* lb, int family, const void* A2,
                     const uint32_t* map2) {
  TimeScope ts(c, family);
  const int nslot = (N + 63) / 64;
  HIPCHK(c, c->ga_bn.reserve((size_t)N + 4));
  float* bmax = c->ga_bn.p + N;
  if (an) {
    ISLECHK(k_rownorms(c, B, N, K, ldb, c->ga_bn.p));
    ISLECHK(k_max_f32(c, c->ga_bn.p, N, bmax));
  }
  return gemm_assign_two_pass(
      c, A, an ? Arm : nullptr, lda_rm, an, M, K, B, ldb, N,
      [&](AssignRec* part, const uint32_t* map, float eta) { return YyGroupEpi{cn, dn, cn_max, lb, G, nslot, part, map, eta, an, bmax}; },
      [&](const AssignRec* part, uint32_t n, const uint32_t* map, float eta, uint32_t* redo, uint32_t* nredo) {
        hipLaunchKernelGGL(yy_first_combine_k, dim3(cdiv(n, 256)), dim3(256), 0, c->stream, part, nslot, n, G, dn, cn_max, assign, ub, lb, map, eta, an, bmax, redo,
                           nredo);
      },
      nullptr, A2, map2);
}
int k_gemm_assign_tiles(isle_ctx* c, const float* A, const float* Arm, int lda_rm, uint64_t M, int K, const float* B, int ldb, int N, int TL, const float* cn,
                        const float* pn, const float* cmax, uint32_t* assign, float* ub, float* tlb, int family, const uint32_t* map0, const void* A2,
                        const uint32_t* map2) {
  TimeScope ts(c, family);
  const int nslot = (N + 63) / 64;
  return gemm_assign_two_pass(
      c, A, Arm, lda_rm, pn, M, K, B, ldb, N,
      [&](AssignRec* part, const uint32_t* map, float eta) { return TileEpi{cn, pn, cmax, tlb, TL, nslot, part, map, eta}; },
      [&](const AssignRec* part, uint32_t n, const uint32_t* map, float eta, uint32_t* redo, uint32_t* nredo) {
        hipLaunchKernelGGL(tiles_combine_k, dim3(cdiv(n, 256)), dim3(256), 0, c->stream, part, nslot, n, TL, pn, cmax, assign, ub, tlb, map, eta, redo, nredo);
      },
      map0, A2, map2);
}

__global__ __launch_bounds__(256) void transpose_k(const float* __restrict__ in, uint64_t rows, uint64_t cols, uint64_t ld_in,
                                                    float* __restrict__ out, uint64_t ld_out) {
  __shared__ float t[32][33];
  const uint64_t r0 = (uint64_t)blockIdx.x * 32, c0 = (uint64_t)blockIdx.y * 32;
  const int tx = threadIdx.x & 31, ty = threadIdx.x >> 5;
  for (int yy = ty; yy < 32; yy += 8) {
    const uint64_t r = r0 + tx, cc = c0 + yy;
    t[yy][tx] = (r < rows && cc < cols) ? in[cc * ld_in + r] : 0.f;
  }
  __syncthreads();
  for (int yy = ty; yy < 32; yy += 8) {
    const uint64_t r = r0 + yy, cc = c0 + tx;
    if (r < rows && cc < cols) out[r * ld_out + cc] = t[tx][yy];
  }
}
int k_transpose(isle_ctx* c, const float* in, uint64_t rows, uint64_t cols, uint64_t ld_in, float* out, uint64_t ld_out) {
  if (rows == 0 || cols == 0) return 0;
  const uint64_t cb = cdiv(cols, 32);
  const uint64_t rows_per = std::max<uint64_t>(32, ((1ull << 31) / 256 / cb) * 32);
  for (uint64_t r0 = 0; r0 < rows; r0 += rows_per) {
    const uint64_t nr = std::min(rows_per, rows - r0);
    dim3 g((unsigned)cdiv(nr, 32), (unsigned)cb), blk(256);
    hipLaunchKernelGGL(transpose_k, g, blk, 0, c->stream, in + r0, nr, cols, ld_in, out + r0 * ld_out, ld_out);
    HIPCHK(c, hipGetLastError());
  }
  return 0;
}

int k_ensure_pt(isle_ctx* c) {
  if (c->Pt_ready) return 0;
  if (!c->P_ready || !c->D) return isle_fail(c, ISLE_E_ARG, "no projection to transpose");
  HIPCHK(c, c->Pt.reserve((size_t)c->D * c->ldk));
  ISLECHK(k_transpose(c, c->P.p, c->ldk, c->D, c->ldk, c->Pt.p, c->D));
  c->Pt_ready = true;
  return 0;
}

__device__ inline double block_sum(double v, double* sh) {
  const int lane = threadIdx.x & 63, wave = threadIdx.x >> 6;
#pragma unroll
  for (int off = 32; off > 0; off >>= 1) v += __shfl_xor(v, off);
  __syncthreads();
  if (lane == 0) sh[wave] = v;
  __syncthreads();
  double s = 0.0;
  for (int w = 0; w < (int)(blockDim.x >> 6); ++w) s += sh[w];
  return s;
}

constexpr int BJ_W = 16;
constexpr int BJ_P = 2 * BJ_W;

__device__ inline void rr_pair(int nplayers, int round, int slot, int* p, int* q) {
  const int m = nplayers - 1;
  if (slot == 0) {
    *p = nplayers - 1;
    *q = round % m;
  } else {
    *p = (round + slot) % m;
    *q = (round - slot + m) % m;
  }
}

constexpr int BJ_SCR = BJ_P * BJ_P + 8;
constexpr int BJ_ROWS = 64;

__device__ inline void bj_blocks(int nblk2, int round, int slot, int* A, int* Bk) {
  rr_pair(nblk2, round, slot, A, Bk);
  if (*A > *Bk) {
    const int x = *A;
    *A = *Bk;
    *Bk = x;
  }
}
__device__ inline int bj_col(int A, int Bk, int cc) { return cc < BJ_W ? A * BJ_W + cc : Bk * BJ_W + (cc - BJ_W); }

__global__ __launch_bounds__(256) void bj_gram_k(const double* __restrict__ W, int n, int nblk2, int round, double* __restrict__ gpart) {
  __shared__ double T[64][BJ_P + 1];
  int A, Bk;
  bj_blocks(nblk2, round, blockIdx.x, &A, &Bk);
  if (A * BJ_W >= n) return;
  const int t = threadIdx.x;
  const int gi = t >> 3, gj0 = (t & 7) * 4;
  double g0 = 0.0, g1 = 0.0, g2 = 0.0, g3 = 0.0;
  const int rbeg = blockIdx.y * BJ_ROWS, rend = min(n, rbeg + BJ_ROWS);
  for (int r0 = rbeg; r0 < rend; r0 += 64) {
    __syncthreads();
    for (int idx = t; idx < 64 * BJ_P; idx += 256) {
      const int rr = idx & 63, cc = idx >> 6;
      T[rr][cc] = W[(size_t)bj_col(A, Bk, cc) * n + r0 + rr];
    }
    __syncthreads();
#pragma unroll 8
    for (int rr = 0; rr < 64; ++rr) {
      const double a = T[rr][gi];
      g0 = fma(a, T[rr][gj0 + 0], g0);
      g1 = fma(a, T[rr][gj0 + 1], g1);
      g2 = fma(a, T[rr][gj0 + 2], g2);
      g3 = fma(a, T[rr][gj0 + 3], g3);
    }
  }
  double* G = gpart + ((size_t)blockIdx.x * gridDim.y + blockIdx.y) * (BJ_P * BJ_P) + gi * BJ_P + gj0;
  G[0] = g0;
  G[1] = g1;
  G[2] = g2;
  G[3] = g3;
}

__global__ __launch_bounds__(256) void bj_inner_k(int n, int nblk2, int round, double tol, double abs_tol, const double* __restrict__ gpart,
                                                   int nrowch, double* __restrict__ scr, unsigned int* __restrict__ rotated, int cross_only) {
  __shared__ double G[BJ_P][BJ_P + 1];
  __shared__ double Q[BJ_P][BJ_P + 1];
  __shared__ unsigned int nrot;
  int A, Bk;
  bj_blocks(nblk2, round, blockIdx.x, &A, &Bk);
  if (A * BJ_W >= n) return;
  const int t = threadIdx.x;
  double* S = scr + (size_t)blockIdx.x * BJ_SCR;
  const double* gp = gpart + (size_t)blockIdx.x * nrowch * (BJ_P * BJ_P);
  for (int idx = t; idx < BJ_P * BJ_P; idx += 256) {
    const int i = idx / BJ_P, j = idx % BJ_P;
    const int u = (i <= j) ? i * BJ_P + j : j * BJ_P + i;
    double sum = 0.0;
    for (int ch = 0; ch < nrowch; ++ch) sum += gp[(size_t)ch * (BJ_P * BJ_P) + u];
    G[i][j] = sum;
    Q[i][j] = (i == j) ? 1.0 : 0.0;
  }
  if (t == 0) nrot = 0;
  __syncthreads();
  {
    int live = 0;
    for (int idx = t; idx < BJ_P * BJ_P; idx += 256) {
      const int i = idx / BJ_P, j = idx % BJ_P;
      if (i < j && (!cross_only || (i < BJ_W && j >= BJ_W))) {
        const double a = G[i][i], b = G[j][j], g = G[i][j];
        live |= (a > 0.0 && b > 0.0 && g * g > tol * tol * a * b && fabs(g) > abs_tol) ? 1 : 0;
      }
    }
    if (!__syncthreads_or(live)) {
      if (t == 0) S[BJ_P * BJ_P] = 0.0;
      return;
    }
  }
  const int bi = t >> 4, bj = t & 15;
  unsigned int my_rot = 0;
  const int nrounds = cross_only ? BJ_W : BJ_P - 1;
// ... 308 lines not shown
```

isle_amd/csrc/gemm_bf16x3.h:

```cpp
#pragma once
#include <hip/hip_runtime.h>
#include <stdint.h>

namespace isle_gemm3 {

typedef __bf16 bf16x8 __attribute__((ext_vector_type(8)));
typedef __bf16 bf16x4 __attribute__((ext_vector_type(4)));
typedef float f32x16 __attribute__((ext_vector_type(16)));

__device__ inline void split3(float x, __bf16& x0, __bf16& x1, __bf16& x2) {
  x0 = (__bf16)x;
  const float r1 = x - (float)x0;
  x1 = (__bf16)r1;
  const float r2 = r1 - (float)x1;
  x2 = (__bf16)r2;
}

__global__ __launch_bounds__(256) void gemm3_split_b_k(const float* __restrict__ B, int ldb, int K, int N, int Kp8, int Np, bf16x8* __restrict__ B3) {
  const size_t i = (size_t)blockIdx.x * 256 + threadIdx.x;
  if (i >= (size_t)Kp8 * Np) return;
  const int q = (int)(i / Np), n = (int)(i - (size_t)q * Np);
  bf16x8 v[3];
#pragma unroll
  for (int j = 0; j < 8; ++j) {
    const int k = 8 * q + j;
    const float x = (k < K && n < N) ? B[(size_t)n * ldb + k] : 0.f;
    __bf16 t0, t1, t2;
    split3(x, t0, t1, t2);
    v[0][j] = t0;
    v[1][j] = t1;
    v[2][j] = t2;
  }
#pragma unroll
  for (int p = 0; p < 3; ++p) B3[((size_t)p * Kp8 + q) * Np + n] = v[p];
}

template <int WMT_, int WNT_, int WAVES_M_, int WAVES_N_, int OCC_, int TK_ = 16, int NP_ = 3>
struct Cfg {
  static constexpr int WMT = WMT_, WNT = WNT_, WAVES_M = WAVES_M_, WAVES_N = WAVES_N_, OCC = OCC_, TK = TK_;
  static constexpr int NP = NP_;
  static constexpr int KO = TK / 8;
  static constexpr int TM = 32 * WMT * WAVES_M, TN = 32 * WNT * WAVES_N;
  static constexpr int NT = 64 * WAVES_M * WAVES_N;
  static constexpr int A_STAGE = NP * KO * TM, B_STAGE = NP * KO * TN;
  static constexpr size_t LDS_BYTES = (size_t)2 * (A_STAGE + B_STAGE) * 16;
  static constexpr int A_UNITS = TM * (TK / 4) / NT;
  static constexpr int B_UNITS = (B_STAGE + NT - 1) / NT;
  static_assert(TM * (TK / 4) % NT == 0 && (TK == 16 || TK == 32) && (NP == 2 || NP == 3), "tile / thread counts");
};

struct StoreC {
  static constexpr int kGroup = 0;
  float* __restrict__ C;
  uint64_t ldc;
  __device__ inline void operator()(uint64_t m, int n, float v) const { C[(uint64_t)n * ldc + m] = v; }
};

struct Top2 {
  float m1, m2, ax;
  uint32_t i1;
};
__device__ inline void top2_take(Top2& t, float d, uint32_t idx, float ax) {
  if (d < t.m1) {
    t.m2 = t.m1;
    t.m1 = d;
    t.i1 = idx;
  } else {
    t.m2 = fminf(t.m2, d);
  }
  t.ax = fmaxf(t.ax, ax);
}
__device__ inline void top2_merge(Top2& t, float om1, float om2, uint32_t oi1, float oax) {
  if (om1 < t.m1 || (om1 == t.m1 && oi1 < t.i1)) {
    t.m2 = fminf(t.m1, om2);
    t.m1 = om1;
    t.i1 = oi1;
  } else {
    t.m2 = fminf(t.m2, om1);
  }
  t.ax = fmaxf(t.ax, oax);
}
__device__ inline void top2_pair(Top2& t) {
  const float om1 = __shfl_xor(t.m1, 32), om2 = __shfl_xor(t.m2, 32), oax = __shfl_xor(t.ax, 32);
  const uint32_t oi1 = (uint32_t)__shfl_xor((int)t.i1, 32);
  top2_merge(t, om1, om2, oi1, oax);
}

template <class CF, class Epi>
__device__ inline void tile_epilogue(f32x16 (&acc)[CF::WNT][CF::WMT], uint64_t m0, int n0, int wm, int wn, int l31, int h, uint64_t M, int N, const Epi& epi) {
  constexpr int TN = CF::TN, WMT = CF::WMT, WNT = CF::WNT;
  if constexpr (Epi::kGroup != 0) {
    static_assert(Epi::kGroup == 8 || Epi::kGroup == 32, "group epilogue: groups of 8 or 32 columns");
#pragma unroll
    for (int i = 0; i < WMT; ++i) {
      const uint64_t m = m0 + wm * (32 * WMT) + i * 32 + l31;
      const bool live = m < M;
      const float rd = epi.rowdata(live ? m : M - 1);
      Top2 best{3.4e38f, 3.4e38f, 0.f, 0xffffffffu};
      float run2 = 3.4e38f;
      auto fold = [&](const Top2& t) {
        if (t.m1 < best.m1) {
          run2 = fminf(fminf(run2, best.m1), t.m2);
          best = t;
        } else {
          run2 = fminf(run2, t.m1);
        }
      };
#pragma unroll
      for (int j = 0; j < WNT; ++j) {
        const int cb = n0 + wn * (32 * WNT) + j * 32;
        if (cb >= N) continue;
        float dist[16], ax[16];
#pragma unroll
        for (int r = 0; r < 16; ++r) {
          const int col = cb + 4 * h + (r & 3) + 8 * (r >> 2);
          const bool in = col < N;
          dist[r] = in ? epi.dist(acc[j][i][r], col, rd) : 3.4e38f;
          ax[r] = in ? epi.aux(col) : 0.f;
        }
        if constexpr (Epi::kGroup == 8) {
#pragma unroll
          for (int q = 0; q < 4; ++q) {
            Top2 t{3.4e38f, 3.4e38f, 0.f, 0xffffffffu};
#pragma unroll
            for (int u = 0; u < 4; ++u) {
              const int col = cb + 4 * h + u + 8 * q;
              if (col < N) top2_take(t, dist[4 * q + u], (uint32_t)col, ax[4 * q + u]);
            }
            top2_pair(t);
            if (cb + 8 * q < N) {
              if (live && h == (q & 1)) epi.group(m, (cb >> 3) + q, rd, t.m1, t.i1, t.m2, t.ax);
              fold(t);
            }
          }
        } else {
          Top2 t{3.4e38f, 3.4e38f, 0.f, 0xffffffffu};
#pragma unroll
          for (int r = 0; r < 16; ++r) {
            const int col = cb + 4 * h + (r & 3) + 8 * (r >> 2);
            if (col < N) top2_take(t, dist[r], (uint32_t)col, ax[r]);
          }
          top2_pair(t);
          if (live && h == (j & 1)) epi.group(m, cb >> 5, rd, t.m1, t.i1, t.m2, t.ax);
          fold(t);
        }
      }
      if (live && h == 0 && n0 + wn * (32 * WNT) < N) epi.slot(m, (n0 + wn * (32 * WNT)) / (32 * WNT), rd, best.m1, best.i1, best.m2, best.ax, run2);
    }
  } else {
  const bool full_n = n0 + TN <= N;
#pragma unroll
  for (int i = 0; i < WMT; ++i) {
    const uint64_t m = m0 + wm * (32 * WMT) + i * 32 + l31;
    if (m < M) {
#pragma unroll
      for (int j = 0; j < WNT; ++j) {
        const int nb = n0 + wn * (32 * WNT) + j * 32 + 4 * h;
        if (full_n) {
#pragma unroll
          for (int r = 0; r < 16; ++r) epi(m, nb + (r & 3) + 8 * (r >> 2), acc[j][i][r]);
        } else {
#pragma unroll
          for (int r = 0; r < 16; ++r) {
            const int n = nb + (r & 3) + 8 * (r >> 2);
            if (n < N) epi(m, n, acc[j][i][r]);
          }
        }
      }
    }
  }
  }
}

template <class CF, class Epi>
__global__ __launch_bounds__(CF::NT, CF::OCC) void gemm_bf16x3_k(const float* __restrict__ A, uint64_t M, int K, const bf16x8* __restrict__ B3, int Kp8,
                                                                  int Np, int N, uint32_t nMB, uint32_t nNT, Epi epi) {
  constexpr int TM = CF::TM, TN = CF::TN, NT = CF::NT, WMT = CF::WMT, WNT = CF::WNT, TK = CF::TK, KO = CF::KO, NP = CF::NP;
  extern __shared__ bf16x8 lds3[];
  bf16x8* As = lds3;
  bf16x8* Bs = lds3 + 2 * CF::A_STAGE;
  const uint32_t wg = blockIdx.x, xcd = wg & 7u, slot = wg >> 3;
  const uint32_t mb = (slot / nNT) * 8u + xcd, nt = slot % nNT;
  if (mb >= nMB) return;
  const uint64_t m0 = (uint64_t)mb * TM;
  const int n0 = (int)nt * TN;
  const int tid = threadIdx.x, lane = tid & 63, wave = tid >> 6;
  const int l31 = lane & 31, h = lane >> 5;
  const int wm = wave % CF::WAVES_M, wn = wave / CF::WAVES_M;

  uint32_t arow[CF::A_UNITS];
  int akq[CF::A_UNITS];
#pragma unroll
  for (int u = 0; u < CF::A_UNITS; ++u) {
    const int unit = tid + u * NT;
    akq[u] = unit / TM;
    const uint64_t m = m0 + (uint32_t)(unit % TM);
    arow[u] = (uint32_t)(m < M ? m : M - 1);
  }
  float ra[4 * CF::A_UNITS];
  uint4 rb[CF::B_UNITS];
  auto load_slab = [&](int k0) {
#pragma unroll
    for (int u = 0; u < CF::A_UNITS; ++u) {
#pragma unroll
      for (int t = 0; t < 4; ++t) {
        const int k = min(k0 + 4 * akq[u] + t, K - 1);
        ra[4 * u + t] = A[(uint64_t)k * M + arow[u]];
      }
    }
    const int q0 = k0 >> 3;
#pragma unroll
    for (int u = 0; u < CF::B_UNITS; ++u) {
      const int unit = min(tid + u * NT, CF::B_STAGE - 1);
      const int p = unit / (KO * TN), r = unit - p * KO * TN, q = r / TN, n = r - q * TN;
      rb[u] = *reinterpret_cast<const uint4*>(B3 + ((size_t)p * Kp8 + q0 + q) * Np + n0 + n);
    }
  };
  auto store_slab = [&](int stage) {
    char* a = reinterpret_cast<char*>(As + stage * CF::A_STAGE);
#pragma unroll
    for (int u = 0; u < CF::A_UNITS; ++u) {
      const int unit = tid + u * NT;
      const int row = unit % TM;
      bf16x4 v[3];
#pragma unroll
      for (int t = 0; t < 4; ++t) {
        __bf16 t0, t1, t2;
        split3(ra[4 * u + t], t0, t1, t2);
        v[0][t] = t0;
        v[1][t] = t1;
        v[2][t] = t2;
      }
#pragma unroll
      for (int p = 0; p < NP; ++p) *reinterpret_cast<bf16x4*>(a + ((size_t)((p * KO + (akq[u] >> 1)) * TM + row)) * 16 + (akq[u] & 1) * 8) = v[p];
    }
    uint4* b = reinterpret_cast<uint4*>(Bs + stage * CF::B_STAGE);
#pragma unroll
    for (int u = 0; u < CF::B_UNITS; ++u) {
      const int unit = tid + u * NT;
      if (unit < CF::B_STAGE) b[unit] = rb[u];
    }
  };

  f32x16 acc[WNT][WMT];
#pragma unroll
  for (int j = 0; j < WNT; ++j)
#pragma unroll
    for (int i = 0; i < WMT; ++i)
#pragma unroll
      for (int r = 0; r < 16; ++r) acc[j][i][r] = 0.f;

  const int nslab = (K + TK - 1) / TK;
  load_slab(0);
  store_slab(0);
  __syncthreads();
  for (int s = 0; s < nslab; ++s) {
    const int cur = s & 1;
    if (s + 1 < nslab) load_slab((s + 1) * TK);
    const bf16x8* a = As + cur * CF::A_STAGE + wm * (32 * WMT) + l31;
    const bf16x8* b = Bs + cur * CF::B_STAGE + wn * (32 * WNT) + l31;
#pragma unroll
    for (int ks = 0; ks < TK / 16; ++ks) {
      const int oc = 2 * ks + h;
      bf16x8 bv[WNT][NP];
#pragma unroll
      for (int j = 0; j < WNT; ++j)
#pragma unroll
        for (int p = 0; p < NP; ++p) bv[j][p] = b[(p * KO + oc) * TN + 32 * j];
#pragma unroll
      for (int pa = NP - 1; pa >= 0; --pa) {
        bf16x8 av[WMT];
#pragma unroll
        for (int i = 0; i < WMT; ++i) av[i] = a[(pa * KO + oc) * TM + 32 * i];
#pragma unroll
        for (int pb = NP - 1 - pa; pb >= 0; --pb)
#pragma unroll
          for (int i = 0; i < WMT; ++i)
#pragma unroll
            for (int j = 0; j < WNT; ++j) acc[j][i] = __builtin_amdgcn_mfma_f32_32x32x16_bf16(bv[j][pb], av[i], acc[j][i], 0, 0, 0);
      }
    }
    if (s + 1 < nslab) store_slab(cur ^ 1);
    __syncthreads();
  }

  tile_epilogue<CF, Epi>(acc, m0, n0, wm, wn, l31, h, M, N, epi);
}

inline int kp8_of(int K) { return 4 * ((K + 31) / 32); }
template <class CF>
inline int np_of(int N) { return (N + CF::TN - 1) / CF::TN * CF::TN; }

template <class CF, class Epi>
inline hipError_t launch(hipStream_t stream, const float* A, uint64_t M, int K, const float* B, int ldb, int N, void* B3, Epi epi) {
  const int Kp8 = kp8_of(K), Np = np_of<CF>(N);
  const size_t nb = (size_t)Kp8 * Np;
  hipLaunchKernelGGL(gemm3_split_b_k, dim3((unsigned)((nb + 255) / 256)), dim3(256), 0, stream, B, ldb, K, N, Kp8, Np, reinterpret_cast<bf16x8*>(B3));
  const uint32_t nMB = (uint32_t)((M + CF::TM - 1) / CF::TM), nNT = (uint32_t)(Np / CF::TN);
  const uint64_t slots = (uint64_t)((nMB + 7) / 8) * nNT;
  static bool lds_attr_set[64] = {};
  int dev = 0;
  hipError_t e = hipGetDevice(&dev);
  if (e != hipSuccess) return e;
  if (dev < 0 || dev >= 64 || !lds_attr_set[dev]) {
    e = hipFuncSetAttribute(reinterpret_cast<const void*>(&gemm_bf16x3_k<CF, Epi>), hipFuncAttributeMaxDynamicSharedMemorySize, (int)CF::LDS_BYTES);
    if (e != hipSuccess) return e;
    if (dev >= 0 && dev < 64) lds_attr_set[dev] = true;
  }
  hipLaunchKernelGGL((gemm_bf16x3_k<CF, Epi>), dim3((uint32_t)(slots * 8)), dim3(CF::NT), CF::LDS_BYTES, stream, A, M, K, reinterpret_cast<const bf16x8*>(B3), Kp8,
                     Np, N, nMB, nNT, epi);
  return hipGetLastError();
}

template <int NS_, int TK_ = 16>
struct CfgDma {
  static constexpr int NS = NS_;
  static constexpr int WMT = 2, WNT = 2, WAVES_M = 4, WAVES_N = 4, TK = TK_, KO = TK_ / 8, NP = 2, OCC = 4;
  static constexpr int TM = 256, TN = 256, NT = 1024;
  static constexpr int A_STAGE = NP * KO * TM, B_STAGE = NP * KO * TN, STAGE = A_STAGE + B_STAGE;
  static constexpr int PPW = STAGE / 64 / 16;
  static constexpr size_t LDS_BYTES = (size_t)NS * STAGE * 16;
  static_assert(TK_ == 16 || TK_ == 32, "slabs of 16 or 32");
};
inline int nslab_of(int K, int TK) { return (K + TK - 1) / TK; }
inline size_t a2_units(uint64_t M, int K, int TK = 16) { return (size_t)((M + 255) / 256) * nslab_of(K, TK) * (4 * (TK / 8)) * 256; }

__global__ __launch_bounds__(256) void gemm2_split_a_k(const float* __restrict__ A, uint64_t M, int K, int nslab, int KO, bf16x8* __restrict__ A2) {
  const uint64_t mb = blockIdx.x, m = mb * 256 + threadIdx.x;
  const int q = blockIdx.y;
  bf16x8 v0, v1;
#pragma unroll
  for (int j = 0; j < 8; ++j) {
    const int k = 8 * q + j;
    const float x = (m < M && k < K) ? A[(uint64_t)k * M + m] : 0.f;
    const __bf16 x0 = (__bf16)x;
    v0[j] = x0;
    v1[j] = (__bf16)(x - (float)x0);
  }
  const size_t base = ((mb * nslab + (size_t)(q / KO)) * (2 * KO) + (size_t)(q % KO)) * 256 + threadIdx.x;
  A2[base] = v0;
  A2[base + (size_t)KO * 256] = v1;
}
inline hipError_t split_a(hipStream_t stream, const float* A, uint64_t M, int K, void* A2, int TK = 16) {
  const int nslab = nslab_of(K, TK);
  const uint64_t nMB = (M + 255) / 256;
  if (nMB == 0) return hipSuccess;
  if (nMB >= (1ull << 31)) return hipErrorInvalidValue;
  hipLaunchKernelGGL(gemm2_split_a_k, dim3((uint32_t)nMB, (uint32_t)(nslab * (TK / 8))), dim3(256), 0, stream, A, M, K, nslab, TK / 8, reinterpret_cast<bf16x8*>(A2));
  return hipGetLastError();
}

template <class CF, class Epi>
__global__ __launch_bounds__(CF::NT) void gemm_bf16x2_dma_k(const bf16x8* __restrict__ A2, uint64_t M, int K, const bf16x8* __restrict__ B3, int Kp8, int Np,
                                                             int N, uint32_t nMB, uint32_t nNT, Epi epi) {
  constexpr int TM = CF::TM, TN = CF::TN, WMT = CF::WMT, WNT = CF::WNT, KO = CF::KO, NP = CF::NP, NS = CF::NS, TK = CF::TK, PPW = CF::PPW;
  static_assert((NS & (NS - 1)) == 0 && NS >= 2 && NS <= 4, "ring of 2 or 4 stages");
  extern __shared__ bf16x8 ldsr[];
  const uint32_t wg = blockIdx.x, xcd = wg & 7u, slot = wg >> 3;
  const uint32_t mb = (slot / nNT) * 8u + xcd, nt = slot % nNT;
  if (mb >= nMB) return;
  const uint64_t m0 = (uint64_t)mb * TM;
  const int n0 = (int)nt * TN;
  const int tid = threadIdx.x, lane = tid & 63;
  const int wave = __builtin_amdgcn_readfirstlane(tid >> 6);
  const int l31 = lane & 31, h = lane >> 5;
  const int wm = wave % CF::WAVES_M, wn = wave / CF::WAVES_M;
  const int nslab = (K + TK - 1) / TK;
  const bool mine_a = wave < 8;
  const int w8 = mine_a ? wave : wave - 8;
  const bf16x8* ga = A2 + ((size_t)mb * nslab) * CF::A_STAGE + (size_t)(w8 * PPW) * 64 + lane;
  const bf16x8* gb[PPW];
#pragma unroll
  for (int i = 0; i < PPW; ++i) {
    const int u = (w8 * PPW + i) * 64 + lane;
    gb[i] = B3 + ((size_t)((u / (KO * 256)) * Kp8 + ((u >> 8) % KO))) * Np + n0 + (u & 255);
  }
  const uint32_t lpiece = (uint32_t)(((mine_a ? 0 : CF::A_STAGE) + w8 * PPW * 64) * 16);
  auto issue = [&](int s) {
    char* l = reinterpret_cast<char*>(ldsr) + (size_t)(s & (NS - 1)) * CF::STAGE * 16 + lpiece;
    if (mine_a) {
      const bf16x8* g = ga + (size_t)s * CF::A_STAGE;
#pragma unroll
      for (int i = 0; i < PPW; ++i)
        __builtin_amdgcn_global_load_lds((const __attribute__((address_space(1))) void*)(g + 64 * i), (__attribute__((address_space(3))) void*)(l + 1024 * i), 16, 0, 0);
    } else {
      const size_t o = (size_t)(KO * s) * Np;
#pragma unroll
      for (int i = 0; i < PPW; ++i)
        __builtin_amdgcn_global_load_lds((const __attribute__((address_space(1))) void*)(gb[i] + o), (__attribute__((address_space(3))) void*)(l + 1024 * i), 16, 0, 0);
    }
  };

  f32x16 acc[WNT][WMT];
#pragma unroll
  for (int j = 0; j < WNT; ++j)
#pragma unroll
    for (int i = 0; i < WMT; ++i)
#pragma unroll
      for (int r = 0; r < 16; ++r) acc[j][i][r] = 0.f;

#pragma unroll
  for (int s = 0; s < NS - 1; ++s)
    if (s < nslab) issue(s);
  for (int s = 0; s < nslab; ++s) {
    if (s + NS - 2 < nslab) __builtin_amdgcn_s_waitcnt(0x0f70 | (PPW * (NS - 2)));
    else __builtin_amdgcn_s_waitcnt(0x0f70);
    __builtin_amdgcn_s_barrier();
    if (s + NS - 1 < nslab) issue(s + NS - 1);
    const bf16x8* st = ldsr + (size_t)(s & (NS - 1)) * CF::STAGE;
    const bf16x8* a = st + wm * (32 * WMT) + l31;
    const bf16x8* b = st + CF::A_STAGE + wn * (32 * WNT) + l31;
#pragma unroll
    for (int ks = 0; ks < TK / 16; ++ks) {
      const int oc = 2 * ks + h;
      bf16x8 bv[WNT][NP];
#pragma unroll
      for (int j = 0; j < WNT; ++j)
#pragma unroll
        for (int p = 0; p < NP; ++p) bv[j][p] = b[(p * KO + oc) * TN + 32 * j];
#pragma unroll
      for (int pa = NP - 1; pa >= 0; --pa) {
        bf16x8 av[WMT];
#pragma unroll
        for (int i = 0; i < WMT; ++i) av[i] = a[(pa * KO + oc) * TM + 32 * i];
#pragma unroll
        for (int pb = NP - 1 - pa; pb >= 0; --pb)
#pragma unroll
          for (int i = 0; i < WMT; ++i)
#pragma unroll
            for (int j = 0; j < WNT; ++j) acc[j][i] = __builtin_amdgcn_mfma_f32_32x32x16_bf16(bv[j][pb], av[i], acc[j][i], 0, 0, 0);
      }
    }
  }
  tile_epilogue<CF, Epi>(acc, m0, n0, wm, wn, l31, h, M, N, epi);
}

template <class CF, class Epi>
inline hipError_t launch_dma(hipStream_t stream, const void* A2, uint64_t M, int K, const float* B, int ldb, int N, void* B3, Epi epi) {
  const int Kp8 = kp8_of(K), Np = (N + CF::TN - 1) / CF::TN * CF::TN;
  const size_t nb = (size_t)Kp8 * Np;
  hipLaunchKernelGGL(gemm3_split_b_k, dim3((unsigned)((nb + 255) / 256)), dim3(256), 0, stream, B, ldb, K, N, Kp8, Np, reinterpret_cast<bf16x8*>(B3));
  const uint32_t nMB = (uint32_t)((M + CF::TM - 1) / CF::TM), nNT = (uint32_t)(Np / CF::TN);
  const uint64_t slots = (uint64_t)((nMB + 7) / 8) * nNT;
  static bool lds_attr_set[64] = {};
  int dev = 0;
  hipError_t e = hipGetDevice(&dev);
  if (e != hipSuccess) return e;
  if (dev < 0 || dev >= 64 || !lds_attr_set[dev]) {
    e = hipFuncSetAttribute(reinterpret_cast<const void*>(&gemm_bf16x2_dma_k<CF, Epi>), hipFuncAttributeMaxDynamicSharedMemorySize, (int)CF::LDS_BYTES);
    if (e != hipSuccess) return e;
    if (dev >= 0 && dev < 64) lds_attr_set[dev] = true;
  }
  hipLaunchKernelGGL((gemm_bf16x2_dma_k<CF, Epi>), dim3((uint32_t)(slots * 8)), dim3(CF::NT), CF::LDS_BYTES, stream, reinterpret_cast<const bf16x8*>(A2), M, K,
                     reinterpret_cast<const bf16x8*>(B3), Kp8, Np, N, nMB, nNT, epi);
  return hipGetLastError();
}

}
```

isle_amd/csrc/kmeans.hip:

```cpp
#include <algorithm>
#include <cstdlib>
#include <vector>

#include <cstring>

#include "common.h"
#include "hamerly.h"
#include "scan.h"

typedef float floatx16 __attribute__((ext_vector_type(16)));
constexpr int CS_ITEMS = 16;
enum { PR_ARGMIN = 0, PR_MINDIST = 1, PR_TILES = 2 };
template <int MODE>
static int launch_proj_reg(isle_ctx* c, uint64_t D, int k, int ldk, const float* C, const float* cn, const float* pn, uint32_t* assign,
                           float* min_dist, bool* done, const float* Pt = nullptr, const uint32_t* map = nullptr, float* ub = nullptr,
                           float* lb = nullptr, const uint32_t* need = nullptr, int TL = 0);

template <int NIT>
__global__ __launch_bounds__(256) void kmpp_update_k(const float* __restrict__ P, const float* __restrict__ pn, uint32_t D, int ldk,
                                                      const float* __restrict__ newC, const float* __restrict__ cn, int nc,
                                                      float* __restrict__ min_dist) {
  const int lane = threadIdx.x & 63;
  const uint32_t d = blockIdx.x * 4 + (threadIdx.x >> 6);
  if (d >= D) return;
// ... 675 lines not shown
            const float raw = (-2.0f * acc[t][r] + cn[cc]) + nd;
            if (MODE == PR_ARGMIN || MODE == PR_TILES) {
              const float dist = fabsf(raw);
              if (dist < best || (dist == best && (uint32_t)cc < bidx)) {
                second = best;
                best = dist;
                bidx = (uint32_t)cc;
              } else {
                second = fminf(second, dist);
              }
            } else {
              best = fminf(best, fmaxf(raw, 0.0f));
            }
          }
        }
      }
    }
  }
  if (MODE == PR_TILES && !(dbg & 2)) {
    if (h == 0 && myd < D) {
      assign[dst] = bidx;
      float uu, ll, l2;
      hamerly_store_bounds(best, second, nd + btc, &uu, &l2);
      hamerly_store_bounds(best, best, nd + cmax, &uu, &ll);
      ub[dst] = uu;
      lb[(size_t)dst * TL + btile] = l2;
    }
    return;
  }
  const float ob = __shfl_xor(best, 32);
  const float os = __shfl_xor(second, 32);
  const uint32_t oi = __shfl_xor(bidx, 32);
  cmax = fmaxf(cmax, __shfl_xor(cmax, 32));
  if (MODE == PR_ARGMIN || MODE == PR_TILES) {
    if (ob < best || (ob == best && oi < bidx)) {
      second = fminf(best, os);
      best = ob;
      bidx = oi;
    } else {
      second = fminf(second, ob);
    }
    if (h == 0 && myd < D) {
      const uint32_t dst = map ? map[myd] : myd;
      assign[dst] = bidx;
      if (ub) hamerly_store_bounds(best, second, nd + cmax, &ub[dst], &lb[dst]);
    }
  } else {
    best = fminf(best, ob);
    if (h == 0 && myd < D) min_dist[myd] = fminf(min_dist[myd], best);
  }
}

template <int MODE>
static int launch_proj_reg(isle_ctx* c, uint64_t D, int k, int ldk, const float* C, const float* cn, const float* pn, uint32_t* assign,
                           float* min_dist, bool* done, const float* Pt, const uint32_t* map, float* ub, float* lb, const uint32_t* need, int TL) {
  *done = false;
  if (!D) return 0;
  if (!Pt) {
    if (!(c->Pt_ready || c->Pt2_ready)) return 0;
    ISLECHK(k_ensure_pt(c));
    Pt = c->Pt.p;
  }
  const int kpad = (k + 31) & ~31;
  const int ct = kpad / 32;
  const int nslab = cdiv(ldk / 2, PR_SL);
  dim3 g(cdiv(D, 128)), b(256);
#define LR(NS, CM)                                                                                                            \
  do {                                                                                                                        \
    const size_t lds = (size_t)2 * (CM * 32) * (PR_SL + 1) * sizeof(float);                                                   \
    ISLECHK(isle_max_lds(c, (const void*)proj_assign_reg_k<NS, CM, MODE>, (int)lds));                                        \
    hipLaunchKernelGGL((proj_assign_reg_k<NS, CM, MODE>), g, b, lds, c->stream, Pt, pn, (uint32_t)D, k, ldk, C, cn, assign, min_dist, map, ub, lb, \
                       need, TL);                                                                                             \
    *done = true;                                                                                                             \
  } while (0)
  if (MODE == PR_TILES) {
    if (ct > 32) return 0;
    LR(8, 8);
    HIPCHK(c, hipGetLastError());
    return 0;
  }
  if (ct <= 1) {
    if (nslab <= 2) LR(2, 1);
    else if (nslab <= 4) LR(4, 1);
    else if (nslab <= 7) LR(7, 1);
    else LR(8, 1);
  } else if (ct <= 2 && nslab <= 2) LR(2, 2);
  else if (ct <= 4 && nslab <= 4) LR(4, 4);
  else if (ct <= 7 && nslab <= 7) LR(7, 7);
  else LR(8, 8);
#undef LR
  HIPCHK(c, hipGetLastError());
  return 0;
}

__global__ __launch_bounds__(256) void compact_rows_k(const float* __restrict__ P, const float* __restrict__ pn, int ldk,
                                                       const uint32_t* __restrict__ active, uint32_t n, float* __restrict__ Pa,
                                                       float* __restrict__ pna) {
  __shared__ float t[32][33];
  const uint32_t i0 = blockIdx.x * 32;
  const int tx = threadIdx.x & 31, ty = threadIdx.x >> 5;
  for (int j0 = 0; j0 < ldk; j0 += 32) {
    __syncthreads();
    for (int yy = ty; yy < 32; yy += 8) {
      const uint32_t i = i0 + yy;
      const uint32_t d = active[min(i, n - 1)];
      t[yy][tx] = P[(size_t)d * ldk + min(j0 + tx, ldk - 1)];
    }
    __syncthreads();
    for (int yy = ty; yy < 32; yy += 8) {
      const int j = j0 + yy;
      const uint32_t i = i0 + tx;
      if (j < ldk && i < n) Pa[(size_t)j * n + i] = t[tx][yy];
    }
  }
  if (threadIdx.x < 32 && i0 + threadIdx.x < n) pna[i0 + threadIdx.x] = pn[active[i0 + threadIdx.x]];
}

__global__ __launch_bounds__(256) void compact_rows64_k(const float* __restrict__ P, const float* __restrict__ pn, int ldk,
                                                         const uint32_t* __restrict__ active, uint32_t n, float* __restrict__ Pa,
                                                         float* __restrict__ pna) {
  extern __shared__ float t64[];
  const uint32_t i0 = blockIdx.x * 64;
  const int lane = threadIdx.x & 63, w = threadIdx.x >> 6;
  const uint32_t myd = active[min(i0 + (uint32_t)lane, n - 1)];
  for (int j0 = 0; j0 < ldk; j0 += 256) {
    __syncthreads();
    const int j = j0 + 4 * lane;
    float4 v[16];
#pragma unroll
    for (int u = 0; u < 16; ++u) {
      const uint32_t d = (uint32_t)__shfl((int)myd, w * 16 + u);
      v[u] = *reinterpret_cast<const float4*>(P + (size_t)d * ldk + min(j, ldk - 4));
    }
#pragma unroll
    for (int u = 0; u < 16; ++u) {
      float* r = t64 + (size_t)(w * 16 + u) * 257 + 4 * lane;
      r[0] = v[u].x;
      r[1] = v[u].y;
      r[2] = v[u].z;
      r[3] = v[u].w;
    }
    __syncthreads();
    if (i0 + lane < n) {
#pragma unroll 8
      for (int cc = 0; cc < 64; ++cc) {
        const int cj = j0 + w * 64 + cc;
        if (cj < ldk) Pa[(size_t)cj * n + i0 + lane] = t64[(size_t)lane * 257 + w * 64 + cc];
      }
    }
  }
  if (threadIdx.x < 64 && i0 + threadIdx.x < n) pna[i0 + threadIdx.x] = pn[myd];
}

int k_compact_rows(isle_ctx* c, const float* P, const float* pn, int ldk, const uint32_t* active, uint32_t n, float* Pa, float* pna) {
  if (n >= 4096 && ldk >= 256 && ldk % 4 == 0) {
    const size_t lds = (size_t)64 * 257 * sizeof(float);
    ISLECHK(isle_max_lds(c, (const void*)compact_rows64_k, (int)lds));
    hipLaunchKernelGGL(compact_rows64_k, dim3(cdiv(n, 64)), dim3(256), lds, c->stream, P, pn, ldk, active, n, Pa, pna);
  } else {
    hipLaunchKernelGGL(compact_rows_k, dim3(cdiv(n, 32)), dim3(256), 0, c->stream, P, pn, ldk, active, n, Pa, pna);
  }
  HIPCHK(c, hipGetLastError());
  return 0;
}

__global__ __launch_bounds__(256) void pt_need_keys_k(const uint32_t* __restrict__ active, uint32_t n, const uint32_t* __restrict__ need,
                                                       uint64_t* __restrict__ key, uint32_t* __restrict__ val) {
  const uint32_t i = blockIdx.x * 256 + threadIdx.x;
  if (i < n) {
    const uint32_t d = active[i];
    key[i] = need[d];
    val[i] = d;
  }
}

int k_proj_assign_active(isle_ctx* c, const float* P, const float* pn, int k, int ldk, const float* C, const float* cn,
                         const uint32_t* active, uint32_t n, float* Pa, float* pna, uint32_t* assign, float* ub, float* lb) {
  TimeScope ts(c, ISLE_T_LLOYD_PROJ);
  if (n == 0) return 0;
  ISLECHK(k_compact_rows(c, P, pn, ldk, active, n, Pa, pna));
  bool done = false;
  ISLECHK(launch_proj_reg<PR_ARGMIN>(c, n, k, ldk, C, cn, pna, assign, nullptr, &done, Pa, active, ub, lb));
  if (!done) return isle_fail(c, ISLE_E_ARG, "projected assignment: register kernel unavailable");
  return 0;
}

__global__ __launch_bounds__(256) void proj_dots_tiles_k(const float* __restrict__ dotsT, uint32_t D, int k, const float* __restrict__ pn,
                                                          const float* __restrict__ cn, uint32_t* __restrict__ assign, float* __restrict__ ub,
                                                          float* __restrict__ lb, int TL) {
  const uint32_t d = blockIdx.x * 256 + threadIdx.x;
  if (d >= D) return;
  const float nd = pn[d];
  float best = 3.4e38f, second = 3.4e38f, btc = 0.f, cmax = 0.f;
  uint32_t bidx = 0xffffffffu, btile = 0;
  for (int c0 = 0; c0 < k; c0 += 32) {
    float m1 = 3.4e38f, m2 = 3.4e38f, tc = 0.f;
    uint32_t i1 = 0xffffffffu;
    float dot[32];
#pragma unroll
    for (int j = 0; j < 32; ++j) dot[j] = dotsT[(size_t)min(c0 + j, k - 1) * D + d];
#pragma unroll
    for (int j = 0; j < 32; ++j) {
      const int cc = c0 + j;
      if (cc < k) {
        const float cnj = cn[cc];
        tc = fmaxf(tc, cnj);
        const float dist = fabsf((-2.0f * dot[j] + cnj) + nd);
        if (dist < m1) {
          m2 = m1;
          m1 = dist;
          i1 = (uint32_t)cc;
        } else {
          m2 = fminf(m2, dist);
        }
      }
    }
    const uint32_t T = (uint32_t)(c0 >> 5);
    if (m1 < best) {
      best = m1;
      bidx = i1;
      second = m2;
      btile = T;
      btc = tc;
    }
    cmax = fmaxf(cmax, tc);
    float uu, ll;
    hamerly_store_bounds(m1, m1, nd + tc, &uu, &ll);
    lb[(size_t)d * TL + T] = ll;
  }
  assign[d] = bidx;
  float uu, ll, l2;
  hamerly_store_bounds(best, second, nd + btc, &uu, &l2);
  hamerly_store_bounds(best, best, nd + cmax, &uu, &ll);
  ub[d] = uu;
  lb[(size_t)d * TL + btile] = l2;
}

int k_kmpp_to_tiles(isle_ctx* c, uint64_t D, int k, const float* pn, const float* cn, const float* best, uint32_t* assign, float* ub, int TL) {
  TimeScope ts(c, ISLE_T_LLOYD_PROJ);
  if (D == 0) return 0;
  hipLaunchKernelGGL(kmpp_to_tiles_k, dim3(cdiv(D, 256)), dim3(256), 0, c->stream, (uint32_t)D, k, pn, cn, best, c->kmpp_arg.p, c->kmpp_m2a.p, c->kmpp_tmin.p, assign,
                     ub, c->ptlb.p, TL);
  HIPCHK(c, hipGetLastError());
  return 0;
}

bool k_proj_full_by_gemm(isle_ctx* c, uint64_t D, int k) {
  const char* pf = c->knob(KN_PROJ_FULL);
  return (c->Pt_ready || c->Pt2_ready) && D > 0 && k >= 64 && (k_gemm_assign_fused_ok(c, D, k, k) || isle_scratch_ok(c, c->dotsT.cap, (double)D * k * sizeof(float))) &&
         ((2.0 * (double)D * k * k >= 2e10 && !(pf && !strcmp(pf, "fused"))) || (pf && !strcmp(pf, "gemm")));
}
int k_proj_assign_tiles(isle_ctx* c, const float* P, const float* pn, uint64_t D, int k, int ldk, const float* C, const float* cn, uint32_t* assign,
                        float* ub, float* tlb, int TL, const uint32_t* active, uint32_t n, const uint32_t* need, float* Pa, float* pna) {
  TimeScope ts(c, ISLE_T_LLOYD_PROJ);
  bool done = false;
  if (!active) {
    if (k_proj_full_by_gemm(c, D, k)) {
      if (k_gemm_assign_fused_ok(c, D, k, k)) {
        HIPCHK(c, c->cmax_buf.reserve(4));
        ISLECHK(k_max_f32(c, cn, k, c->cmax_buf.p));
        const bool a2 = c->Pt2_ready && P == c->P.p;
        return k_gemm_assign_tiles(c, c->Pt_ready ? c->Pt.p : nullptr, P, ldk, D, k, C, ldk, k, TL, cn, pn, c->cmax_buf.p, assign, ub, tlb, ISLE_T_LLOYD_PROJ, nullptr,
                                   a2 ? c->Pt2.p : nullptr, a2 && c->Pt2_pos ? c->dperm.p : nullptr);
      }
      HIPCHK(c, c->dotsT.reserve((size_t)D * k));
      ISLECHK(k_ensure_pt(c));
      ISLECHK(k_gemm_nn_assign(c, c->Pt.p, D, k, C, ldk, k, c->dotsT.p, ISLE_T_LLOYD_PROJ));
      hipLaunchKernelGGL(proj_dots_tiles_k, dim3(cdiv(D, 256)), dim3(256), 0, c->stream, c->dotsT.p, (uint32_t)D, k, pn, cn, assign, ub, tlb, TL);
      HIPCHK(c, hipGetLastError());
      return 0;
    }
    ISLECHK(launch_proj_reg<PR_TILES>(c, D, k, ldk, C, cn, pn, assign, nullptr, &done, nullptr, nullptr, ub, tlb, nullptr, TL));
  } else {
    if (n == 0) return 0;
    {
      const char* pa = c->knob(KN_PROJ_ACTIVE);
      const bool by_gemm = pa ? !strcmp(pa, "gemm") : true;
      if (by_gemm && k_gemm_assign_fused_ok(c, n, k, k)) {
        ISLECHK(k_compact_rows(c, P, pn, ldk, active, n, Pa, pna));
        HIPCHK(c, c->cmax_buf.reserve(4));
        ISLECHK(k_max_f32(c, cn, k, c->cmax_buf.p));
        return k_gemm_assign_tiles(c, Pa, P, ldk, n, k, C, ldk, k, TL, cn, pn, c->cmax_buf.p, assign, ub, tlb, ISLE_T_LLOYD_PROJ, active);
      }
    }
    if (need && n > 256 && !c->knob_zero(KN_PT_SORT)) {
      HIPCHK(c, c->gl_key_a.reserve(n));
      HIPCHK(c, c->gl_key_b.reserve(n));
      HIPCHK(c, c->gl_val_a.reserve(n));
      HIPCHK(c, c->gl_val_b.reserve(n));
      hipLaunchKernelGGL(pt_need_keys_k, dim3(cdiv(n, 256)), dim3(256), 0, c->stream, active, n, need, c->gl_key_a.p, c->gl_val_a.p);
      HIPCHK(c, hipGetLastError());
      bool in_a = true;
      ISLECHK(k_sort_pairs_u64(c, c->gl_key_a.p, c->gl_val_a.p, c->gl_key_b.p, c->gl_val_b.p, n, ((k + 31) / 32 + 7) & ~7, &in_a));
      active = in_a ? c->gl_val_a.p : c->gl_val_b.p;
    }
    ISLECHK(k_compact_rows(c, P, pn, ldk, active, n, Pa, pna));
    ISLECHK(launch_proj_reg<PR_TILES>(c, n, k, ldk, C, cn, pna, assign, nullptr, &done, Pa, active, ub, tlb, need, TL));
  }
  if (!done) return isle_fail(c, ISLE_E_ARG, "projected assignment with tile bounds: shape not covered (k = %d)", k);
  return 0;
}

int k_proj_assign(isle_ctx* c, const float* P, const float* pn, uint64_t D, int k, int ldk, const float* C, const float* cn,
                  uint32_t* assign, float* ub, float* lb) {
  {
    TimeScope ts(c, ISLE_T_LLOYD_PROJ);
    bool done = false;
    ISLECHK(launch_proj_reg<PR_ARGMIN>(c, D, k, ldk, C, cn, pn, assign, nullptr, &done, nullptr, nullptr, ub, lb));
    if (done) return 0;
  }
  if (ub) return isle_fail(c, ISLE_E_ARG, "generic projected assignment has no bounds output");
  TimeScope ts(c, ISLE_T_LLOYD_PROJ);
  if (D == 0) return 0;
  hipLaunchKernelGGL(proj_assign_k, dim3(cdiv(D, PA_DOCS)), dim3(256), 0, c->stream, P, pn, (uint32_t)D, k, ldk, C, cn, assign);
  HIPCHK(c, hipGetLastError());
  return 0;
}

__global__ __launch_bounds__(256) void member_fill_k(const uint32_t* __restrict__ assign, uint32_t D, int k, const int* __restrict__ off,
                                                      int* __restrict__ cursor, uint32_t* __restrict__ members) {
  extern __shared__ int sh[];
  int* hist = sh;
  int* base = sh + k;
  for (int j = threadIdx.x; j < k; j += 256) hist[j] = 0;
  __syncthreads();
  const uint32_t b0 = blockIdx.x * (256 * CS_ITEMS);
  uint32_t mine[CS_ITEMS];
  int rank[CS_ITEMS];
#pragma unroll
  for (int u = 0; u < CS_ITEMS; ++u) {
    const uint32_t d = b0 + threadIdx.x + 256 * u;
    mine[u] = (d < D) ? assign[d] : 0xffffffffu;
    rank[u] = (d < D) ? atomicAdd(&hist[mine[u]], 1) : 0;
  }
  __syncthreads();
  for (int j = threadIdx.x; j < k; j += 256) base[j] = hist[j] ? off[j] + atomicAdd(&cursor[j], hist[j]) : 0;
  __syncthreads();
#pragma unroll
  for (int u = 0; u < CS_ITEMS; ++u) {
    const uint32_t d = b0 + threadIdx.x + 256 * u;
    if (d < D) members[base[mine[u]] + rank[u]] = d;
  }
}

constexpr int SEG_MC = 256;
struct SegChunk {
  int beg, end;
};
template <int NIT>
__global__ __launch_bounds__(256) void proj_segsum_k(const float* __restrict__ P, int ldk, const SegChunk* __restrict__ chunks,
                                                      const uint32_t* __restrict__ members, float* __restrict__ part ) {
  extern __shared__ float red[];
  const int lane = threadIdx.x & 63, wave = threadIdx.x >> 6;
  const int nq = ldk / 4;
  const int beg = chunks[blockIdx.x].beg, end = chunks[blockIdx.x].end;
  float4 acc[NIT];
#pragma unroll
  for (int it = 0; it < NIT; ++it) acc[it] = make_float4(0.f, 0.f, 0.f, 0.f);
  const int myi = beg + wave + 4 * lane;
  const uint32_t mym = myi < end ? members[myi] : 0u;
  const int cnt = end > beg + wave ? min(64, (end - beg - wave + 3) / 4) : 0;
  for (int j = 0; j < cnt; j += 4) {
    float4 v[4][NIT];
#pragma unroll
    for (int u = 0; u < 4; ++u) {
      const uint32_t mj = (uint32_t)__shfl((int)mym, min(j + u, cnt - 1));
      const float4* row = reinterpret_cast<const float4*>(P + (size_t)mj * ldk);
      const float live = j + u < cnt ? 1.f : 0.f;
#pragma unroll
      for (int it = 0; it < NIT; ++it) {
        const int q = lane + 64 * it;
        const float4 x = q < nq ? row[q] : make_float4(0.f, 0.f, 0.f, 0.f);
        v[u][it] = make_float4(x.x * live, x.y * live, x.z * live, x.w * live);
      }
    }
#pragma unroll
    for (int u = 0; u < 4; ++u)
#pragma unroll
      for (int it = 0; it < NIT; ++it) {
        acc[it].x += v[u][it].x;
        acc[it].y += v[u][it].y;
        acc[it].z += v[u][it].z;
        acc[it].w += v[u][it].w;
      }
  }
#pragma unroll
  for (int it = 0; it < NIT; ++it) {
    const int q = lane + 64 * it;
    if (q < nq) reinterpret_cast<float4*>(red + (size_t)wave * ldk)[q] = acc[it];
  }
  __syncthreads();
  float* out = part + (size_t)blockIdx.x * ldk;
  for (int j = threadIdx.x; j < ldk; j += 256) out[j] = (red[j] + red[ldk + j]) + (red[2 * ldk + j] + red[3 * ldk + j]);
}
__global__ __launch_bounds__(256) void proj_segsum_reduce_k(const float* __restrict__ part, const int* __restrict__ c0, int ldk, float* __restrict__ Csum) {
  const int cc = blockIdx.y;
  const int j = blockIdx.x * 256 + threadIdx.x;
  if (j >= ldk) return;
  float s = 0.f;
  int q = c0[cc];
  const int qe = c0[cc + 1];
  for (; q + 8 <= qe; q += 8) {
    float v[8];
#pragma unroll
    for (int u = 0; u < 8; ++u) v[u] = part[(size_t)(q + u) * ldk + j];
#pragma unroll
    for (int u = 0; u < 8; ++u) s += v[u];
  }
  for (; q < qe; ++q) s += part[(size_t)q * ldk + j];
  Csum[(size_t)cc * ldk + j] = s;
}
__global__ __launch_bounds__(256) void member_keys_k(const uint32_t* __restrict__ assign, uint32_t D, uint64_t* __restrict__ key, uint32_t* __restrict__ val) {
  const uint32_t d = blockIdx.x * 256 + threadIdx.x;
  if (d < D) {
    key[d] = assign[d];
    val[d] = d;
  }
}

__global__ __launch_bounds__(256) void member_offsets_k(const int* __restrict__ counts, int k, int* __restrict__ off , int* __restrict__ cursor ) {
  __shared__ int sh[256];
  int carry = 0;
  for (int base = 0; base < k; base += 256) {
    const int i = base + threadIdx.x;
    const int v = i < k ? counts[i] : 0;
    sh[threadIdx.x] = v;
    __syncthreads();
    for (int o = 1; o < 256; o <<= 1) {
      const int add = threadIdx.x >= o ? sh[threadIdx.x - o] : 0;
      __syncthreads();
      sh[threadIdx.x] += add;
      __syncthreads();
    }
    if (i < k) {
      off[i] = carry + sh[threadIdx.x] - v;
      cursor[i] = 0;
    }
    carry += sh[255];
    __syncthreads();
  }
  if (threadIdx.x == 0) off[k] = carry;
}
int k_member_lists_dev(isle_ctx* c, const uint32_t* assign, uint64_t D, int k, const int* counts_dev) {
  HIPCHK(c, c->members.reserve(D ? D : 1));
  HIPCHK(c, c->moff.reserve(2 * (size_t)k + 2));
  int* offd = c->moff.p;
  int* cur = c->moff.p + k + 1;
  hipLaunchKernelGGL(member_offsets_k, dim3(1), dim3(256), 0, c->stream, counts_dev, k, offd, cur);
  if (D)
// ... 325 lines not shown
```

isle_amd/hot_path.py:

```python
import ctypes as C

import numpy as np

from ._lib import IsleHipError, load_library

TIMING_FAMILIES = ["gram_pass1", "gram_pass2", "ortho", "qr", "evd", "rotate", "project", "kmpp", "lloyd_proj",
                   "sparse_assign", "sparse_update", "op_build", "comm", "threshold", "post", "ingest", "infer", "lift"]

BLOCK_KS_MAX_ITERS = 100
BLOCK_KS_BLOCK_SIZE = 10
BLOCK_KS_TOLERANCE = 1e-4
MAX_KMEANS_LOWD_REPS = 10
MAX_KMEANS_REPS = 10


W0_C, EPS2_C, EPS3_C, RHO_C = 1.0, 1.0 / 3.0, 5.0, 1.1


def catchword_rank(num_docs, num_topics, sample_rate=None):
    x = EPS2_C * W0_C * float(np.float32(num_docs))
    if sample_rate is not None:
        x = x * float(np.float32(sample_rate))
    return int(np.floor(x / float(np.float32(2.0 * num_topics))))

# ... 320 lines not shown
        err = []

        def tramp(ptr, n, user):
            try:
                consume(memoryview((C.c_char * n).from_address(ptr)))
                return 0
            except BaseException as e:
                err.append(e)
                return 1

        sink = _TEXT_SINK(tramp) if consume is not None else None
        nb, ne = C.c_uint64(), C.c_uint64()
        rc = call(C.cast(sink, C.c_void_p) if sink is not None else None, C.byref(nb), C.byref(ne))
        if err:
            raise err[0]
        self._chk(rc)
        return int(nb.value), int(ne.value)

    def _model_text_call(self, which, format, consume):
        if isinstance(which, str):
            code, host = self._MODELS[which], None
            V, cols = self._resident_shape(which)
        else:
            host = np.asfortranarray(which, np.float32)
            if host.ndim != 2:
                raise ValueError("model must be (V, cols)")
            code, (V, cols) = 2, host.shape
        fmt = TEXT_FORMATS[format] if isinstance(format, str) else int(format)
        return self._text_call(lambda sink, nb, ne: self._lib.isle_hip_model_text(self._h, code, _p(host), int(V), int(cols), fmt, sink, None,
                                                                                  nb, ne), consume)

    def model_text(self, which="catch", format="sparse"):
        parts = []
        self._model_text_call(which, format, lambda mv: parts.append(bytes(mv)))
        return b"".join(parts)

    def write_model(self, path, which="catch", format="sparse"):
        with open(path, "wb") as f:
            return self._model_text_call(which, format, f.write)

    def model_text_size(self, which="catch", format="sparse"):
        return self._model_text_call(which, format, None)

    def edge_topics_text(self, pairs, primary_ratio=0.7, format="sparse", path=None):
        pairs = np.ascontiguousarray(pairs, np.int64).reshape(-1, 2)
        fmt = TEXT_FORMATS[format] if isinstance(format, str) else int(format)

        def call(sink, nb, ne):
            return self._lib.isle_hip_edge_topics_text(self._h, _p(pairs), pairs.shape[0], float(primary_ratio), fmt, sink, None, nb, ne)

        if path is not None:
            with open(path, "wb") as f:
                return self._text_call(call, f.write)
        parts = []
        self._text_call(call, lambda mv: parts.append(bytes(mv)))
        return b"".join(parts)

    def log_combinatorial(self):
        D = getattr(self, "_a_shape", (0, 0, 0))[1]
        out = np.empty(max(D, 1), np.float32)
        self._chk(self._lib.isle_hip_log_combinatorial(self._h, _p(out), None))
        return out[:D]

    def distinct_top_five_sets(self, m=(2, 5, 10, 20, 50, 100, 200, 500), fetch_quintuples=False):
        ms = np.ascontiguousarray(m, np.int32).reshape(-1)
        D = getattr(self, "_a_shape", (0, 0, 0))[1]
        cnt = np.empty(max(ms.size, 1), np.uint64)
        nq, nr = C.c_uint64(), C.c_uint64()
        runs = np.empty(max(D, 1), np.uint64)
        q = np.empty((max(D, 1), 5), np.float32) if fetch_quintuples else None
        self._chk(self._lib.isle_hip_distinct_top_five(self._h, int(ms.size), _p(ms), _p(cnt), C.byref(nq), _p(q), _p(runs), C.byref(nr)))
        return dict(counts={int(v): int(c) for v, c in zip(ms, cnt)}, num_quintuples=int(nq.value), run_lengths=runs[:nr.value].copy(),
                    quintuples=None if q is None else q[:nq.value].copy())

    def frobenius(self):
        out = C.c_float()
        self._chk(self._lib.isle_hip_frobenius(self._h, C.byref(out)))
        return out.value

    def gram_apply(self, X):
        X = np.asfortranarray(X, dtype=np.float32)
        assert X.shape[0] == self.V
        Z = np.empty_like(X, order="F")
        self._chk(self._lib.isle_hip_gram_apply(self._h, _p(X), X.shape[1], _p(Z)))
        return Z

    def operator_form(self):
        f = C.c_int()
        self._chk(self._lib.isle_hip_operator_form(self._h, C.byref(f)))
        return f.value

    def compute_block_ks(self, num_topics, blk=BLOCK_KS_BLOCK_SIZE, ncv=None, maxit=BLOCK_KS_MAX_ITERS,
                         tol=BLOCK_KS_TOLERANCE, seed=1, allow_noconv=False):
        ncv = 2 * num_topics + BLOCK_KS_BLOCK_SIZE if ncv is None else ncv
        ev = np.empty(num_topics, np.float32)
        nconv, rst, nap = C.c_int(), C.c_int(), C.c_int()
        rc = self._lib.isle_hip_block_ks(self._h, num_topics, ncv, maxit, blk, tol, seed, _p(ev), C.byref(nconv), C.byref(rst),
                                         C.byref(nap))
        self._chk(rc, allow=(-3,) if allow_noconv else ())
        return dict(rc=rc, evals=ev, nconv=nconv.value, restarts=rst.value, napplies=nap.value)

    def block_ks_dense(self, A, nev, blk=BLOCK_KS_BLOCK_SIZE, ncv=None, maxit=BLOCK_KS_MAX_ITERS, tol=BLOCK_KS_TOLERANCE, seed=1,
                       start_block=None, allow_noconv=False):
        A = np.asfortranarray(A, dtype=np.float32)
        n = A.shape[0]
        assert A.shape == (n, n)
        ncv = 2 * nev + BLOCK_KS_BLOCK_SIZE if ncv is None else ncv
        ev = np.empty(nev, np.float32)
        U = np.empty((n, nev), np.float32, order="F")
        sb = None if start_block is None else np.asfortranarray(start_block, dtype=np.float32)
        nconv, nref, rst, nap = C.c_int(), C.c_int(), C.c_int(), C.c_int()
        rc = self._lib.isle_hip_block_ks_dense(self._h, _p(A), n, nev, ncv, maxit, blk, tol, seed, _p(sb), _p(ev), _p(U), C.byref(nconv),
                                               C.byref(nref), C.byref(rst), C.byref(nap))
        self._chk(rc, allow=(-3,) if allow_noconv else ())
        return dict(rc=rc, evals=ev, U=U, nconv=nconv.value, nconv_ref_rule=nref.value, restarts=rst.value, napplies=nap.value)

    def get_U(self, k):
        U = np.empty((self.V, k), np.float32, order="F")
        self._chk(self._lib.isle_hip_get_U(self._h, _p(U)))
        return U

    def set_U(self, U):
        U = np.asfortranarray(U, dtype=np.float32)
        self._chk(self._lib.isle_hip_set_U(self._h, _p(U), U.shape[1]))

    def eig_sym(self, S):
        S = np.asfortranarray(S, dtype=np.float32)
        n = S.shape[0]
        e = np.empty(n, np.float32)
        v = np.empty((n, n), np.float32, order="F")
        self._chk(self._lib.isle_hip_eig_sym(self._h, _p(S), n, _p(e), _p(v)))
        return e, v

    def kmeans_init_on_projected_space(self, k, inject_seeds=None, rng_seed=1):
        seeds = np.empty(k, np.uint64)
        Cl = np.empty((k, k), np.float32)
        res, rounds = C.c_float(), C.c_int()
        inj = None if inject_seeds is None else np.ascontiguousarray(inject_seeds, np.uint64)
        self._chk(self._lib.isle_hip_kmeanspp_projected(self._h, k, _p(inj), rng_seed, _p(seeds), _p(Cl), C.byref(res),
                                                       C.byref(rounds)))
        return dict(seeds=seeds, C_lowd=Cl, residual=res.value, rounds=rounds.value)

    def get_min_dist(self):
        md = np.empty(self.D, np.float32)
        self._chk(self._lib.isle_hip_get_min_dist(self._h, _p(md)))
        return md

    def run_lloyds_on_projected_space(self, k, C_lowd, max_reps=MAX_KMEANS_LOWD_REPS):
        Cl = np.array(C_lowd, dtype=np.float32, order="C", copy=True)
        it = C.c_int()
        assign = np.empty(self.D, np.uint32)
        self._chk(self._lib.isle_hip_lloyds_projected(self._h, k, _p(Cl), max_reps, C.byref(it), _p(assign)))
        return dict(C_lowd=Cl, iters=it.value, assign=assign)

    def left_multiply_by_U(self, C_lowd, fetch=True):
        Cl = np.ascontiguousarray(C_lowd, dtype=np.float32)
        n, k = Cl.shape
        out = np.empty((self.V, n), np.float32, order="F") if fetch else None
        self._chk(self._lib.isle_hip_lift_centers(self._h, _p(Cl), k, n, _p(out)))
        return out

    def run_lloyds(self, k, centers=None, max_reps=MAX_KMEANS_REPS, fetch_centers=True):
        cin = None if centers is None else np.asfortranarray(centers, dtype=np.float32)
        cout = np.empty((self.V, k), np.float32, order="F") if fetch_centers else None
        assign = np.empty(self.D, np.uint32)
        it = C.c_int()
        self._chk(self._lib.isle_hip_lloyds_sparse(self._h, k, _p(cin), _p(cout), _p(assign), max_reps, C.byref(it)))
        return dict(centers=cout, assign=assign, iters=it.value)

    def infer(self, model_by_word, offs, rows, counts, iters=15, Lf=10.0, avg_doc_sz=None, want_weights=True):
        M = np.ascontiguousarray(model_by_word, np.float32)
        V, k = M.shape
        offs = np.ascontiguousarray(offs, np.int64)
        rows = np.ascontiguousarray(rows, np.uint32)
        counts = np.ascontiguousarray(counts, np.float32)
        D = offs.shape[0] - 1
        if avg_doc_sz is None:
            nz = int((np.diff(offs) > 0).sum())
            avg_doc_sz = float(int(counts.astype(np.float64).sum()) // max(nz, 1))
        W = np.empty((D, k), np.float32) if want_weights else None
        tt = np.empty((D, 5), np.int32)
        tw = np.empty((D, 5), np.float32)
        llh = np.empty((D, 2), np.float32)
        nc = C.c_uint64()
        self._chk(self._lib.isle_hip_infer(self._h, V, k, _p(M), D, rows.shape[0], _p(counts), _p(rows), _p(offs), int(iters), float(Lf),
                                           float(avg_doc_sz), _p(W) if want_weights else None, _p(tt), _p(tw), _p(llh), C.byref(nc)))
        return dict(weights=W, top_topic=tt, top_weight=tw, llh=llh, nconverged=int(nc.value), avg_doc_sz=avg_doc_sz)

    def infer_resident(self, model="catch", docs=None, iters=15, Lf=10.0, min_weight=None, chunk_docs=0, fetch_entries=True):
        if isinstance(model, str):
            which, host = self._MODELS[model], None
            V, cols = self._resident_shape(model)
        else:
            host = np.asfortranarray(model, np.float32)
            if host.ndim != 2:
                raise ValueError("model must be (V, cols)")
            which, (V, cols) = 2, host.shape
        b, e = (0, getattr(self, "_a_shape", (0, 0, 0))[1]) if docs is None else (int(docs[0]), int(docs[1]))
        n = max(e - b, 0)
        tt = np.empty((n, 5), np.int32)
        tw = np.empty((n, 5), np.float32)
        llh = np.empty((n, 2), np.float32)
        nc, ne = C.c_uint64(), C.c_uint64()
        self._chk(self._lib.isle_hip_infer_resident(self._h, which, _p(host), int(V), int(cols), b, e, int(iters), float(Lf),
                                                    -1.0 if min_weight is None else float(min_weight), int(chunk_docs), _p(tt), _p(tw),
                                                    _p(llh), C.byref(nc), C.byref(ne)))
        self._inf_rows = n
        out = dict(top_topic=tt, top_weight=tw, llh=llh, nconverged=int(nc.value), nentries=int(ne.value), avg_doc_sz=self.avg_doc_sz())
        if fetch_entries:
            out.update(zip(("offs", "topic", "weight"), self.infer_entries(n, out["nentries"])))
        return out

    def _infer_text_call(self, what, rows, base, consume):
        kind = DOC_TEXT_KINDS[what] if isinstance(what, str) else int(what)
        b, e = (0, getattr(self, "_inf_rows", 0)) if rows is None else (int(rows[0]), int(rows[1]))
        return self._text_call(lambda sink, nb, nl: self._lib.isle_hip_infer_text(self._h, kind, b, e, int(base), sink, None, nb, nl), consume)

    def infer_text(self, what="entries", rows=None, base=1):
        parts = []
        self._infer_text_call(what, rows, base, lambda mv: parts.append(bytes(mv)))
        return b"".join(parts)

    def write_infer_text(self, path, what="entries", rows=None, base=1):
        with open(path, "wb") as f:
            return self._infer_text_call(what, rows, base, f.write)

    def infer_text_size(self, what="entries", rows=None, base=1):
        return self._infer_text_call(what, rows, base, None)

    def avg_doc_sz(self):
        v = C.c_float()
        self._chk(self._lib.isle_hip_avg_doc_sz(self._h, C.byref(v)))
        return float(v.value)

    def infer_entries(self, num_docs, nentries):
        off = np.empty(num_docs + 1, np.int64)
        tp = np.empty(nentries, np.uint32)
        wt = np.empty(nentries, np.float32)
        self._chk(self._lib.isle_hip_get_infer_entries(self._h, _p(off), _p(tp), _p(wt)))
        return off, tp, wt

    def timing_enable(self, on=True):
        self._chk(self._lib.isle_hip_timing_enable(self._h, int(on)))

    def timing_reset(self):
        self._chk(self._lib.isle_hip_timing_reset(self._h))

    def timing_get(self):
        n = len(TIMING_FAMILIES)
        ms = np.zeros(n, np.float64)
        cnt = np.zeros(n, np.uint64)
        self._chk(self._lib.isle_hip_timing_get(self._h, _p(ms), _p(cnt)))
        return {f: (float(ms[i]), int(cnt[i])) for i, f in enumerate(TIMING_FAMILIES)}

    def synchronize(self):
        self._chk(self._lib.isle_hip_synchronize(self._h))
```

Before: 4.784 million.

## Gather active rows inside the GEMM assignment kernel instead of compacting first

Adds a row-indexed load mode to the bf16x3 GEMM so the assignment product reads active or redo rows straight from the full projected matrix through an index list. This drops the separate compact-rows copy before the GEMM in the Hamerly active path and the redo pass. Compaction buffers are now sized on demand, growing by doubling, rather than reserved at full D. A test entry point for the row-indexed product is also added. The risk is scattered, less coalesced A loads inside the GEMM tile loader.

```diff
diff --git a/include/isle_hip.h b/include/isle_hip.h
--- a/include/isle_hip.h
+++ b/include/isle_hip.h
@@ -85,6 +85,10 @@
 
 int isle_hip_lloyds_projected(isle_ctx* ctx, int k, float* C_lowd, int max_reps, int* iters_run,
                               uint32_t* assign_out);
+
+int isle_hip_assign_product_rows(isle_ctx* ctx, int epilogue, const float* P, uint64_t nrows, int K, int ld, const uint32_t* rows, uint32_t n,
+                                 uint32_t n_list, const float* A_gathered, const float* dn, const float* C, int N, int ldc, int lbw,
+                                 uint32_t* assign, float* ub, float* lb);
 
 int isle_hip_lift_centers(isle_ctx* ctx, const float* in, int ld_in, int ncols, float* centers);
 
diff --git a/isle_amd/_lib.py b/isle_amd/_lib.py
--- a/isle_amd/_lib.py
+++ b/isle_amd/_lib.py
@@ -57,6 +57,7 @@
     "isle_hip_get_min_dist": (_I, [_P, _P]),
     "isle_hip_host_rand": (_I, [_U64, _I, _P]),
     "isle_hip_lloyds_projected": (_I, [_P, _I, _P, _I, _P, _P]),
+    "isle_hip_assign_product_rows": (_I, [_P, _I, _P, _U64, _I, _I, _P, C.c_uint32, C.c_uint32, _P, _P, _P, _I, _I, _I, _P, _P, _P]),
     "isle_hip_lift_centers": (_I, [_P, _P, _I, _I, _P]),
     "isle_hip_lloyds_sparse": (_I, [_P, _I, _P, _P, _P, _I, _P]),
     "isle_hip_timing_enable": (_I, [_P, _I]),
diff --git a/isle_amd/csrc/api_kmeans.cpp b/isle_amd/csrc/api_kmeans.cpp
--- a/isle_amd/csrc/api_kmeans.cpp
+++ b/isle_amd/csrc/api_kmeans.cpp
@@ -358,8 +358,6 @@
     HIPCHK(c, c->hub.reserve(D ? D : 1));
     HIPCHK(c, c->hlb.reserve(D ? D : 1));
     HIPCHK(c, c->active.reserve(D + 1));
-    HIPCHK(c, c->Pa.reserve((size_t)(D ? D : 1) * ldk));
-    HIPCHK(c, c->pna.reserve(D ? D : 1));
     HIPCHK(c, c->Cold.reserve((size_t)k * ldk + k + 8));
   }
   if (p.tiles) {
@@ -381,8 +379,7 @@
   const int ldk = c->ldk;
   if (p.from_kmpp) return k_kmpp_to_tiles(c, D, k, c->pnorm.p, c->cnorm.p, c->kmpp_best.p, c->assign.p, c->hub.p, p.TL);
   if (p.tiles)
-    return k_proj_assign_tiles(c, c->P.p, c->pnorm.p, D, k, ldk, c->Cdev.p, c->cnorm.p, c->assign.p, c->hub.p, c->ptlb.p, p.TL, nullptr, 0, nullptr, nullptr,
-                               nullptr);
+    return k_proj_assign_tiles(c, c->P.p, c->pnorm.p, D, k, ldk, c->Cdev.p, c->cnorm.p, c->assign.p, c->hub.p, c->ptlb.p, p.TL, nullptr, 0, nullptr);
   return k_proj_assign(c, c->P.p, c->pnorm.p, D, k, ldk, c->Cdev.p, c->cnorm.p, c->assign.p, p.hamerly ? c->hub.p : nullptr,
                        p.hamerly ? c->hlb.p : nullptr);
 }
@@ -441,10 +438,9 @@
   ISLECHK(isle_fetch_u32(c, nact, &c->pin_small()->active_count, &na));
   if (c->knob_on(KN_DEBUG_HAMERLY)) ISLECHK(debug_tile_stats(c, it, na, T));
   if ((uint64_t)na * ISLE_PROJ_FULL_DEN > (uint64_t)D * ISLE_PROJ_FULL_NUM && k_proj_full_by_gemm(c, D, k))
-    return k_proj_assign_tiles(c, c->P.p, c->pnorm.p, D, k, ldk, c->Cdev.p, c->cnorm.p, c->assign.p, c->hub.p, c->ptlb.p, TL, nullptr, 0, nullptr, nullptr,
+    return k_proj_assign_tiles(c, c->P.p, c->pnorm.p, D, k, ldk, c->Cdev.p, c->cnorm.p, c->assign.p, c->hub.p, c->ptlb.p, TL, nullptr, 0,
                                nullptr);
-  return k_proj_assign_tiles(c, c->P.p, c->pnorm.p, D, k, ldk, c->Cdev.p, c->cnorm.p, c->assign.p, c->hub.p, c->ptlb.p, TL, c->active.p, na, c->pneed.p, c->Pa.p,
-                             c->pna.p);
+  return k_proj_assign_tiles(c, c->P.p, c->pnorm.p, D, k, ldk, c->Cdev.p, c->cnorm.p, c->assign.p, c->hub.p, c->ptlb.p, TL, c->active.p, na, c->pneed.p);
 }
 
 static int proj_reassign_hamerly(isle_ctx* c, const ProjScalars& sc, int k, int it) {
@@ -453,7 +449,7 @@
   uint32_t na = 0;
   ISLECHK(isle_fetch_u32(c, nact, &c->pin_small()->active_count, &na));
   if (c->knob_on(KN_DEBUG_HAMERLY)) fprintf(stderr, "[hamerly, projected] iter %d active %u of %llu\n", it, na, (unsigned long long)c->D);
-  return k_proj_assign_active(c, c->P.p, c->pnorm.p, k, c->ldk, c->Cdev.p, c->cnorm.p, c->active.p, na, c->Pa.p, c->pna.p, c->assign.p, c->hub.p, c->hlb.p);
+  return k_proj_assign_active(c, c->P.p, c->pnorm.p, k, c->ldk, c->Cdev.p, c->cnorm.p, c->active.p, na, c->assign.p, c->hub.p, c->hlb.p);
 }
 
 static int proj_update_centres(isle_ctx* c, const ProjPlan& p, int k, int it, std::vector<long long>& sizes) {
@@ -534,6 +530,56 @@
   centres_unpack(C_lowd, Ch, k, ldk);
   if (iters_run) *iters_run = it;
   isle_host_mark("lloyds_projected: exit");
+  return 0;
+}
+
+extern "C" int isle_hip_assign_product_rows(isle_ctx* c, int epilogue, const float* P, uint64_t nrows, int K, int ld, const uint32_t* rows, uint32_t n,
+                                            uint32_t n_list, const float* A_gathered, const float* dn, const float* C, int N, int ldc, int lbw, uint32_t* assign,
+                                            float* ub, float* lb) {
+  if (!c || !P || !rows || !C || !assign || !ub || !lb || (epilogue != 0 && epilogue != 1) || (epilogue == 1 && !dn)) return ISLE_E_ARG;
+  ISLECHK(isle_enter(c));
+  if (K < 1 || ld < K || ldc < K || N < 1 || n < 1 || n_list < n || nrows < 1 || nrows >= (1ull << 32))
+    return isle_fail(c, ISLE_E_ARG, "assignment product on rows: bad shape");
+  if (lbw < (epilogue == 0 ? (N + 31) / 32 : (N + 7) / 8)) return isle_fail(c, ISLE_E_ARG, "assignment product on rows: %d bounds per row are too few", lbw);
+  for (uint32_t i = 0; i < n_list; ++i)
+    if (rows[i] >= nrows) return isle_fail(c, ISLE_E_ARG, "assignment product on rows: entry %u of the list names row %u of %llu", i, rows[i], (unsigned long long)nrows);
+  DevBuf<float> dP, dA, dC, dpn, ddn, dcn, dub, dlb;
+  DevBuf<uint32_t> drows, dassign;
+  HIPCHK(c, dP.reserve((size_t)nrows * ld));
+  HIPCHK(c, dC.reserve((size_t)N * ldc));
+  HIPCHK(c, dpn.reserve(nrows));
+  HIPCHK(c, dcn.reserve((size_t)N + 4));
+  HIPCHK(c, drows.reserve(n_list));
+  HIPCHK(c, dassign.reserve(nrows));
+  HIPCHK(c, dub.reserve(nrows));
+  HIPCHK(c, dlb.reserve((size_t)nrows * lbw));
+  HIPCHK(c, hipMemcpyAsync(dP.p, P, (size_t)nrows * ld * sizeof(float), hipMemcpyHostToDevice, c->stream));
+  HIPCHK(c, hipMemcpyAsync(dC.p, C, (size_t)N * ldc * sizeof(float), hipMemcpyHostToDevice, c->stream));
+  HIPCHK(c, hipMemcpyAsync(drows.p, rows, (size_t)n_list * sizeof(uint32_t), hipMemcpyHostToDevice, c->stream));
+  if (A_gathered) {
+    HIPCHK(c, dA.reserve((size_t)n * K));
+    HIPCHK(c, hipMemcpyAsync(dA.p, A_gathered, (size_t)n * K * sizeof(float), hipMemcpyHostToDevice, c->stream));
+  }
+  if (epilogue == 1) {
+    HIPCHK(c, ddn.reserve(nrows));
+    HIPCHK(c, hipMemcpyAsync(ddn.p, dn, nrows * sizeof(float), hipMemcpyHostToDevice, c->stream));
+  }
+  HIPCHK(c, hipMemsetAsync(dassign.p, 0xff, nrows * sizeof(uint32_t), c->stream));
+  HIPCHK(c, hipMemsetAsync(dub.p, 0xff, nrows * sizeof(float), c->stream));
+  HIPCHK(c, hipMemsetAsync(dlb.p, 0xff, (size_t)nrows * lbw * sizeof(float), c->stream));
+  ISLECHK(k_rownorms(c, dP.p, (int)nrows, K, ld, dpn.p));
+  ISLECHK(k_rownorms(c, dC.p, N, K, ldc, dcn.p));
+  float* cmax = dcn.p + N;
+  ISLECHK(k_max_f32(c, dcn.p, N, cmax));
+  if (epilogue == 0)
+    ISLECHK(k_gemm_assign_tiles(c, dA.p, dP.p, ld, n, K, dC.p, ldc, N, lbw, dcn.p, dpn.p, cmax, dassign.p, dub.p, dlb.p, ISLE_T_LLOYD_PROJ, drows.p));
+  else
+    ISLECHK(k_gemm_assign_yy(c, dA.p, dP.p, ld, dpn.p, n, K, dC.p, ldc, N, lbw, dcn.p, ddn.p, cmax, dassign.p, dub.p, dlb.p, ISLE_T_SPARSE_ASSIGN, nullptr, nullptr,
+                             drows.p));
+  HIPCHK(c, hipMemcpyAsync(assign, dassign.p, nrows * sizeof(uint32_t), hipMemcpyDeviceToHost, c->stream));
+  HIPCHK(c, hipMemcpyAsync(ub, dub.p, nrows * sizeof(float), hipMemcpyDeviceToHost, c->stream));
+  HIPCHK(c, hipMemcpyAsync(lb, dlb.p, (size_t)nrows * lbw * sizeof(float), hipMemcpyDeviceToHost, c->stream));
+  HIPCHK(c, hipStreamSynchronize(c->stream));
   return 0;
 }
 
diff --git a/isle_amd/csrc/common.h b/isle_amd/csrc/common.h
--- a/isle_amd/csrc/common.h
+++ b/isle_amd/csrc/common.h
@@ -292,7 +292,6 @@
   DevBuf<float> cmax_buf;
   DevBuf<uint32_t> ga_redo;
   DevBuf<float> ga_bn;
-  DevBuf<float> ga_rows, ga_rown;
   bool ts_open = false;
   bool roctx_open = false;
   uint32_t ga_last_redo = 0;
@@ -558,7 +557,8 @@
 bool k_gemm_assign_fused_ok(isle_ctx* c, uint64_t M, int K, int N);
 int k_gemm_assign_yy(isle_ctx* c, const float* A, const float* Arm, int lda_rm, const float* an, uint64_t M, int K, const float* B, int ldb, int N, int G,
                      const float* cn, const float* dn, const float* cn_max, uint32_t* assign, float* ub, float* lb, int family, const void* A2 = nullptr,
-                     const uint32_t* map2 = nullptr );
+                     const uint32_t* map2 = nullptr ,
+                     const uint32_t* map0 = nullptr );
 int k_gemm_assign_tiles(isle_ctx* c, const float* A, const float* Arm, int lda_rm, uint64_t M, int K, const float* B, int ldb, int N, int TL, const float* cn,
                         const float* pn, const float* cmax, uint32_t* assign, float* ub, float* tlb, int family, const uint32_t* map0 = nullptr,
                         const void* A2 = nullptr, const uint32_t* map2 = nullptr);
@@ -576,7 +576,6 @@
 int k_member_lists_dev(isle_ctx* c, const uint32_t* assign, uint64_t D, int k, const int* counts_dev);
 int k_yy_delta(isle_ctx* c, float* delta_dev, int k, int G, int group, float* gmax_dev, const uint32_t* id_of_slot = nullptr);
 int k_max_f32(isle_ctx* c, const float* v, int n, float* out_dev);
-int k_compact_rows(isle_ctx* c, const float* P, const float* pn, int ldk, const uint32_t* active, uint32_t n, float* Pa, float* pna);
 int k_kmpp_update(isle_ctx* c, const float* P, const float* pn, uint64_t D, int k, int ldk, const float* newC, int nc, float* min_dist, int s_old = -1,
                   bool track = false);
 int k_kmpp_to_tiles(isle_ctx* c, uint64_t D, int k, const float* pn, const float* cn, const float* best, uint32_t* assign, float* ub, int TL);
@@ -590,10 +589,10 @@
 int k_proj_assign(isle_ctx* c, const float* P, const float* pn, uint64_t D, int k, int ldk, const float* C, const float* cn, uint32_t* assign,
                   float* ub = nullptr, float* lb = nullptr);
 int k_proj_assign_active(isle_ctx* c, const float* P, const float* pn, int k, int ldk, const float* C, const float* cn,
-                         const uint32_t* active, uint32_t n, float* Pa, float* pna, uint32_t* assign, float* ub, float* lb);
+                         const uint32_t* active, uint32_t n, uint32_t* assign, float* ub, float* lb);
 bool k_proj_full_by_gemm(isle_ctx* c, uint64_t D, int k);
 int k_proj_assign_tiles(isle_ctx* c, const float* P, const float* pn, uint64_t D, int k, int ldk, const float* C, const float* cn, uint32_t* assign,
-                        float* ub, float* tlb, int TL, const uint32_t* active, uint32_t n, const uint32_t* need, float* Pa, float* pna);
+                        float* ub, float* tlb, int TL, const uint32_t* active, uint32_t n, const uint32_t* need);
 int k_rownorms_diff(isle_ctx* c, const float* A, const float* B, int rows, int k, int ldk, float* out);
 int k_rownorms(isle_ctx* c, const float* M, int rows, int k, int ldk, float* out);
 int k_proj_accumulate(isle_ctx* c, const float* P, uint64_t D, int k, int ldk, const uint32_t* assign, float* Csum, int* counts);
diff --git a/isle_amd/csrc/dense.hip b/isle_amd/csrc/dense.hip
--- a/isle_amd/csrc/dense.hip
+++ b/isle_amd/csrc/dense.hip
@@ -838,10 +838,11 @@
 }
 size_t k_gemm_split_a_bytes(uint64_t M, int K) { return isle_gemm3::a2_units(M, K, Gemm2Dma::TK) * 16; }
 template <class MakeEpi, class Combine>
-static int gemm_assign_two_pass(isle_ctx* c, const float* A, const float* Arm, int lda_rm, const float* rown, uint64_t M, int K, const float* B, int ldb, int N,
-                                MakeEpi make, Combine combine, const uint32_t* map0 = nullptr ,
+static int gemm_assign_two_pass(isle_ctx* c, const float* A, const float* Arm, int lda_rm, uint64_t M, int K, const float* B, int ldb, int N, MakeEpi make,
+                                Combine combine, const uint32_t* map0 = nullptr ,
                                 const void* A2 = nullptr ,
                                 const uint32_t* map2 = nullptr ) {
+  const bool by_rows = !A && map0 && Arm;
   auto need_a = [&]() -> int {
     if (A) return 0;
     ISLECHK(k_ensure_pt(c));
@@ -855,18 +856,26 @@
   HIPCHK(c, c->gemm_b3.reserve((size_t)3 * isle_gemm3::kp8_of(K) * isle_gemm3::np_of<Gemm3Huge>(N)));
   HIPCHK(c, c->assign_part.reserve((size_t)M * nslot * 5));
   AssignRec* part = reinterpret_cast<AssignRec*>(c->assign_part.p);
-  if (!two) {
-    ISLECHK(need_a());
-    HIPCHK(c, isle_gemm3::launch<Gemm3Huge>(c->stream, A, M, K, B, ldb, N, c->gemm_b3.p, make(part, map0, 0.f)));
+  auto three = [&]() -> int {
+    if (by_rows) {
+      HIPCHK(c, isle_gemm3::launch_rows<Gemm3Huge>(c->stream, Arm, (uint64_t)lda_rm, map0, M, K, B, ldb, N, c->gemm_b3.p, make(part, map0, 0.f)));
+    } else {
+      ISLECHK(need_a());
+      HIPCHK(c, isle_gemm3::launch<Gemm3Huge>(c->stream, A, M, K, B, ldb, N, c->gemm_b3.p, make(part, map0, 0.f)));
+    }
     combine(part, (uint32_t)M, map0, 0.f, nullptr, nullptr);
     HIPCHK(c, hipGetLastError());
     return 0;
-  }
+  };
+  if (!two) return three();
   const float eta2 = ga_eta(K);
   HIPCHK(c, c->ga_redo.reserve(M + 1));
   uint32_t* nredo = c->ga_redo.p + M;
   HIPCHK(c, hipMemsetAsync(nredo, 0, sizeof(uint32_t), c->stream));
-  if (A2 && !c->knob_zero(KN_GEMM_DMA)) {
+  if (by_rows) {
+    HIPCHK(c, isle_gemm3::launch_rows<Gemm2Huge>(c->stream, Arm, (uint64_t)lda_rm, map0, M, K, B, ldb, N, c->gemm_b3.p, make(part, map0, eta2)));
+    combine(part, (uint32_t)M, map0, eta2, c->ga_redo.p, nredo);
+  } else if (A2 && !c->knob_zero(KN_GEMM_DMA)) {
     HIPCHK(c, isle_gemm3::launch_dma<Gemm2Dma>(c->stream, A2, M, K, B, ldb, N, c->gemm_b3.p, make(part, map2 ? map2 : map0, eta2)));
     combine(part, (uint32_t)M, map2 ? map2 : map0, eta2, c->ga_redo.p, nredo);
   } else {
@@ -880,24 +889,15 @@
   c->ga_last_redo = n;
   if (c->knob_on(KN_DEBUG_HAMERLY)) fprintf(stderr, "[assignment product] the two-term pass left %u of %llu rows open\n", n, (unsigned long long)M);
   if (n == 0) return 0;
-  if ((uint64_t)n * 4 > M) {
-    ISLECHK(need_a());
-    HIPCHK(c, isle_gemm3::launch<Gemm3Huge>(c->stream, A, M, K, B, ldb, N, c->gemm_b3.p, make(part, map0, 0.f)));
-    combine(part, (uint32_t)M, map0, 0.f, nullptr, nullptr);
-    HIPCHK(c, hipGetLastError());
-    return 0;
-  }
-  HIPCHK(c, c->ga_rows.reserve((size_t)n * lda_rm));
-  HIPCHK(c, c->ga_rown.reserve(n));
-  ISLECHK(k_compact_rows(c, Arm, rown, lda_rm, c->ga_redo.p, n, c->ga_rows.p, c->ga_rown.p));
-  HIPCHK(c, isle_gemm3::launch<Gemm3Huge>(c->stream, c->ga_rows.p, (uint64_t)n, K, B, ldb, N, c->gemm_b3.p, make(part, c->ga_redo.p, 0.f)));
+  if ((uint64_t)n * 4 > M) return three();
+  HIPCHK(c, isle_gemm3::launch_rows<Gemm3Huge>(c->stream, Arm, (uint64_t)lda_rm, c->ga_redo.p, (uint64_t)n, K, B, ldb, N, c->gemm_b3.p, make(part, c->ga_redo.p, 0.f)));
   combine(part, n, c->ga_redo.p, 0.f, nullptr, nullptr);
   HIPCHK(c, hipGetLastError());
   return 0;
 }
 int k_gemm_assign_yy(isle_ctx* c, const float* A, const float* Arm, int lda_rm, const float* an, uint64_t M, int K, const float* B, int ldb, int N, int G,
                      const float* cn, const float* dn, const float* cn_max, uint32_t* assign, float* ub, float* lb, int family, const void* A2,
-                     const uint32_t* map2) {
+                     const uint32_t* map2, const uint32_t* map0) {
   TimeScope ts(c, family);
   const int nslot = (N + 63) / 64;
   HIPCHK(c, c->ga_bn.reserve((size_t)N + 4));
@@ -907,13 +907,13 @@
     ISLECHK(k_max_f32(c, c->ga_bn.p, N, bmax));
   }
   return gemm_assign_two_pass(
-      c, A, an ? Arm : nullptr, lda_rm, an, M, K, B, ldb, N,
+      c, A, an ? Arm : nullptr, lda_rm, M, K, B, ldb, N,
       [&](AssignRec* part, const uint32_t* map, float eta) { return YyGroupEpi{cn, dn, cn_max, lb, G, nslot, part, map, eta, an, bmax}; },
       [&](const AssignRec* part, uint32_t n, const uint32_t* map, float eta, uint32_t* redo, uint32_t* nredo) {
         hipLaunchKernelGGL(yy_first_combine_k, dim3(cdiv(n, 256)), dim3(256), 0, c->stream, part, nslot, n, G, dn, cn_max, assign, ub, lb, map, eta, an, bmax, redo,
                            nredo);
       },
-      nullptr, A2, map2);
+      map0, A2, map2);
 }
 int k_gemm_assign_tiles(isle_ctx* c, const float* A, const float* Arm, int lda_rm, uint64_t M, int K, const float* B, int ldb, int N, int TL, const float* cn,
                         const float* pn, const float* cmax, uint32_t* assign, float* ub, float* tlb, int family, const uint32_t* map0, const void* A2,
@@ -921,7 +921,7 @@
   TimeScope ts(c, family);
   const int nslot = (N + 63) / 64;
   return gemm_assign_two_pass(
-      c, A, Arm, lda_rm, pn, M, K, B, ldb, N,
+      c, A, Arm, lda_rm, M, K, B, ldb, N,
       [&](AssignRec* part, const uint32_t* map, float eta) { return TileEpi{cn, pn, cmax, tlb, TL, nslot, part, map, eta}; },
       [&](const AssignRec* part, uint32_t n, const uint32_t* map, float eta, uint32_t* redo, uint32_t* nredo) {
         hipLaunchKernelGGL(tiles_combine_k, dim3(cdiv(n, 256)), dim3(256), 0, c->stream, part, nslot, n, TL, pn, cmax, assign, ub, tlb, map, eta, redo, nredo);
diff --git a/isle_amd/csrc/gemm_bf16x3.h b/isle_amd/csrc/gemm_bf16x3.h
--- a/isle_amd/csrc/gemm_bf16x3.h
+++ b/isle_amd/csrc/gemm_bf16x3.h
@@ -172,10 +172,17 @@
   }
 }
 
-template <class CF, class Epi>
+struct ARows {
+  const uint32_t* __restrict__ rows;
+  uint64_t lda;
+  int vec;
+};
+
+template <class CF, class Epi, bool ROWS = false>
 __global__ __launch_bounds__(CF::NT, CF::OCC) void gemm_bf16x3_k(const float* __restrict__ A, uint64_t M, int K, const bf16x8* __restrict__ B3, int Kp8,
-                                                                  int Np, int N, uint32_t nMB, uint32_t nNT, Epi epi) {
+                                                                  int Np, int N, uint32_t nMB, uint32_t nNT, Epi epi, ARows ar) {
   constexpr int TM = CF::TM, TN = CF::TN, NT = CF::NT, WMT = CF::WMT, WNT = CF::WNT, TK = CF::TK, KO = CF::KO, NP = CF::NP;
+  constexpr int KQ = TK / 4;
   extern __shared__ bf16x8 lds3[];
   bf16x8* As = lds3;
   bf16x8* Bs = lds3 + 2 * CF::A_STAGE;
@@ -189,23 +196,40 @@
   const int wm = wave % CF::WAVES_M, wn = wave / CF::WAVES_M;
 
   uint32_t arow[CF::A_UNITS];
-  int akq[CF::A_UNITS];
+  int akq[CF::A_UNITS], alr[CF::A_UNITS];
 #pragma unroll
   for (int u = 0; u < CF::A_UNITS; ++u) {
     const int unit = tid + u * NT;
-    akq[u] = unit / TM;
-    const uint64_t m = m0 + (uint32_t)(unit % TM);
-    arow[u] = (uint32_t)(m < M ? m : M - 1);
+    akq[u] = ROWS ? unit % KQ : unit / TM;
+    alr[u] = ROWS ? unit / KQ : unit % TM;
+    const uint64_t m = m0 + (uint32_t)alr[u];
+    const uint64_t mc = m < M ? m : M - 1;
+    arow[u] = ROWS ? ar.rows[mc] : (uint32_t)mc;
   }
   float ra[4 * CF::A_UNITS];
   uint4 rb[CF::B_UNITS];
   auto load_slab = [&](int k0) {
 #pragma unroll
     for (int u = 0; u < CF::A_UNITS; ++u) {
-#pragma unroll
-      for (int t = 0; t < 4; ++t) {
-        const int k = min(k0 + 4 * akq[u] + t, K - 1);
-        ra[4 * u + t] = A[(uint64_t)k * M + arow[u]];
+      if constexpr (ROWS) {
+        const int kb = k0 + 4 * akq[u];
+        const float* __restrict__ r = A + (uint64_t)arow[u] * ar.lda;
+        if (ar.vec && kb + 3 < K) {
+          const float4 v = *reinterpret_cast<const float4*>(r + kb);
+          ra[4 * u + 0] = v.x;
+          ra[4 * u + 1] = v.y;
+          ra[4 * u + 2] = v.z;
+          ra[4 * u + 3] = v.w;
+        } else {
+#pragma unroll
+          for (int t = 0; t < 4; ++t) ra[4 * u + t] = r[min(kb + t, K - 1)];
+        }
+      } else {
+#pragma unroll
+        for (int t = 0; t < 4; ++t) {
+          const int k = min(k0 + 4 * akq[u] + t, K - 1);
+          ra[4 * u + t] = A[(uint64_t)k * M + arow[u]];
+        }
       }
     }
     const int q0 = k0 >> 3;
@@ -220,8 +244,7 @@
     char* a = reinterpret_cast<char*>(As + stage * CF::A_STAGE);
 #pragma unroll
     for (int u = 0; u < CF::A_UNITS; ++u) {
-      const int unit = tid + u * NT;
-      const int row = unit % TM;
+      const int row = alr[u];
       bf16x4 v[3];
 #pragma unroll
       for (int t = 0; t < 4; ++t) {
@@ -291,8 +314,8 @@
 template <class CF>
 inline int np_of(int N) { return (N + CF::TN - 1) / CF::TN * CF::TN; }
 
-template <class CF, class Epi>
-inline hipError_t launch(hipStream_t stream, const float* A, uint64_t M, int K, const float* B, int ldb, int N, void* B3, Epi epi) {
+template <class CF, class Epi, bool ROWS>
+inline hipError_t launch_form(hipStream_t stream, const float* A, ARows ar, uint64_t M, int K, const float* B, int ldb, int N, void* B3, Epi epi) {
   const int Kp8 = kp8_of(K), Np = np_of<CF>(N);
   const size_t nb = (size_t)Kp8 * Np;
   hipLaunchKernelGGL(gemm3_split_b_k, dim3((unsigned)((nb + 255) / 256)), dim3(256), 0, stream, B, ldb, K, N, Kp8, Np, reinterpret_cast<bf16x8*>(B3));
@@ -303,13 +326,24 @@
   hipError_t e = hipGetDevice(&dev);
   if (e != hipSuccess) return e;
   if (dev < 0 || dev >= 64 || !lds_attr_set[dev]) {
-    e = hipFuncSetAttribute(reinterpret_cast<const void*>(&gemm_bf16x3_k<CF, Epi>), hipFuncAttributeMaxDynamicSharedMemorySize, (int)CF::LDS_BYTES);
+    e = hipFuncSetAttribute(reinterpret_cast<const void*>(&gemm_bf16x3_k<CF, Epi, ROWS>), hipFuncAttributeMaxDynamicSharedMemorySize, (int)CF::LDS_BYTES);
     if (e != hipSuccess) return e;
     if (dev >= 0 && dev < 64) lds_attr_set[dev] = true;
   }
-  hipLaunchKernelGGL((gemm_bf16x3_k<CF, Epi>), dim3((uint32_t)(slots * 8)), dim3(CF::NT), CF::LDS_BYTES, stream, A, M, K, reinterpret_cast<const bf16x8*>(B3), Kp8,
-                     Np, N, nMB, nNT, epi);
+  hipLaunchKernelGGL((gemm_bf16x3_k<CF, Epi, ROWS>), dim3((uint32_t)(slots * 8)), dim3(CF::NT), CF::LDS_BYTES, stream, A, M, K, reinterpret_cast<const bf16x8*>(B3),
+                     Kp8, Np, N, nMB, nNT, epi, ar);
   return hipGetLastError();
+}
+template <class CF, class Epi>
+inline hipError_t launch(hipStream_t stream, const float* A, uint64_t M, int K, const float* B, int ldb, int N, void* B3, Epi epi) {
+  return launch_form<CF, Epi, false>(stream, A, ARows{nullptr, 0, 0}, M, K, B, ldb, N, B3, epi);
+}
+template <class CF, class Epi>
+inline hipError_t launch_rows(hipStream_t stream, const float* A, uint64_t lda, const uint32_t* rows, uint64_t M, int K, const float* B, int ldb, int N, void* B3,
+                              Epi epi) {
+  if (M == 0 || !rows || lda < (uint64_t)K) return hipErrorInvalidValue;
+  const int vec = lda % 4 == 0 && reinterpret_cast<uintptr_t>(A) % 16 == 0;
+  return launch_form<CF, Epi, true>(stream, A, ARows{rows, lda, vec}, M, K, B, ldb, N, B3, epi);
 }
 
 template <int NS_, int TK_ = 16>
diff --git a/isle_amd/csrc/kmeans.hip b/isle_amd/csrc/kmeans.hip
--- a/isle_amd/csrc/kmeans.hip
+++ b/isle_amd/csrc/kmeans.hip
@@ -851,7 +851,7 @@
   if (threadIdx.x < 64 && i0 + threadIdx.x < n) pna[i0 + threadIdx.x] = pn[myd];
 }
 
-int k_compact_rows(isle_ctx* c, const float* P, const float* pn, int ldk, const uint32_t* active, uint32_t n, float* Pa, float* pna) {
+static int k_compact_rows(isle_ctx* c, const float* P, const float* pn, int ldk, const uint32_t* active, uint32_t n, float* Pa, float* pna) {
   if (n >= 4096 && ldk >= 256 && ldk % 4 == 0) {
     const size_t lds = (size_t)64 * 257 * sizeof(float);
     ISLECHK(isle_max_lds(c, (const void*)compact_rows64_k, (int)lds));
@@ -861,6 +861,17 @@
   }
   HIPCHK(c, hipGetLastError());
   return 0;
+}
+
+static int compact_active(isle_ctx* c, const float* P, const float* pn, int ldk, const uint32_t* active, uint32_t n, float** Pa, float** pna) {
+  uint64_t room = 1024;
+  while (room < n) room *= 2;
+  room = std::max<uint64_t>(n, std::min<uint64_t>(room, c->D));
+  HIPCHK(c, c->Pa.reserve((size_t)room * ldk));
+  HIPCHK(c, c->pna.reserve(room));
+  *Pa = c->Pa.p;
+  *pna = c->pna.p;
+  return k_compact_rows(c, P, pn, ldk, active, n, *Pa, *pna);
 }
 
 __global__ __launch_bounds__(256) void pt_need_keys_k(const uint32_t* __restrict__ active, uint32_t n, const uint32_t* __restrict__ need,
@@ -874,10 +885,11 @@
 }
 
 int k_proj_assign_active(isle_ctx* c, const float* P, const float* pn, int k, int ldk, const float* C, const float* cn,
-                         const uint32_t* active, uint32_t n, float* Pa, float* pna, uint32_t* assign, float* ub, float* lb) {
+                         const uint32_t* active, uint32_t n, uint32_t* assign, float* ub, float* lb) {
   TimeScope ts(c, ISLE_T_LLOYD_PROJ);
   if (n == 0) return 0;
-  ISLECHK(k_compact_rows(c, P, pn, ldk, active, n, Pa, pna));
+  float *Pa, *pna;
+  ISLECHK(compact_active(c, P, pn, ldk, active, n, &Pa, &pna));
   bool done = false;
   ISLECHK(launch_proj_reg<PR_ARGMIN>(c, n, k, ldk, C, cn, pna, assign, nullptr, &done, Pa, active, ub, lb));
   if (!done) return isle_fail(c, ISLE_E_ARG, "projected assignment: register kernel unavailable");
@@ -950,7 +962,7 @@
          ((2.0 * (double)D * k * k >= 2e10 && !(pf && !strcmp(pf, "fused"))) || (pf && !strcmp(pf, "gemm")));
 }
 int k_proj_assign_tiles(isle_ctx* c, const float* P, const float* pn, uint64_t D, int k, int ldk, const float* C, const float* cn, uint32_t* assign,
-                        float* ub, float* tlb, int TL, const uint32_t* active, uint32_t n, const uint32_t* need, float* Pa, float* pna) {
+                        float* ub, float* tlb, int TL, const uint32_t* active, uint32_t n, const uint32_t* need) {
   TimeScope ts(c, ISLE_T_LLOYD_PROJ);
   bool done = false;
   if (!active) {
@@ -976,10 +988,9 @@
       const char* pa = c->knob(KN_PROJ_ACTIVE);
       const bool by_gemm = pa ? !strcmp(pa, "gemm") : true;
       if (by_gemm && k_gemm_assign_fused_ok(c, n, k, k)) {
-        ISLECHK(k_compact_rows(c, P, pn, ldk, active, n, Pa, pna));
         HIPCHK(c, c->cmax_buf.reserve(4));
         ISLECHK(k_max_f32(c, cn, k, c->cmax_buf.p));
-        return k_gemm_assign_tiles(c, Pa, P, ldk, n, k, C, ldk, k, TL, cn, pn, c->cmax_buf.p, assign, ub, tlb, ISLE_T_LLOYD_PROJ, active);
+        return k_gemm_assign_tiles(c, nullptr, P, ldk, n, k, C, ldk, k, TL, cn, pn, c->cmax_buf.p, assign, ub, tlb, ISLE_T_LLOYD_PROJ, active);
       }
     }
     if (need && n > 256 && !c->knob_zero(KN_PT_SORT)) {
@@ -993,7 +1004,8 @@
       ISLECHK(k_sort_pairs_u64(c, c->gl_key_a.p, c->gl_val_a.p, c->gl_key_b.p, c->gl_val_b.p, n, ((k + 31) / 32 + 7) & ~7, &in_a));
       active = in_a ? c->gl_val_a.p : c->gl_val_b.p;
     }
-    ISLECHK(k_compact_rows(c, P, pn, ldk, active, n, Pa, pna));
+    float *Pa, *pna;
+    ISLECHK(compact_active(c, P, pn, ldk, active, n, &Pa, &pna));
     ISLECHK(launch_proj_reg<PR_TILES>(c, n, k, ldk, C, cn, pna, assign, nullptr, &done, Pa, active, ub, tlb, need, TL));
   }
   if (!done) return isle_fail(c, ISLE_E_ARG, "projected assignment with tile bounds: shape not covered (k = %d)", k);
diff --git a/isle_amd/hot_path.py b/isle_amd/hot_path.py
--- a/isle_amd/hot_path.py
+++ b/isle_amd/hot_path.py
@@ -496,6 +496,25 @@
         assign = np.empty(self.D, np.uint32)
         self._chk(self._lib.isle_hip_lloyds_projected(self._h, k, _p(Cl), max_reps, C.byref(it), _p(assign)))
         return dict(C_lowd=Cl, iters=it.value, assign=assign)
+
+    def assign_product_rows(self, epilogue, P, K, rows, n, centres, gathered=None, dn=None):
+        P = np.ascontiguousarray(P, np.float32)
+        Cc = np.ascontiguousarray(centres, np.float32)
+        rows = np.ascontiguousarray(rows, np.uint32)
+        nrows, ld = P.shape
+        N, ldc = Cc.shape
+        yy = {"tiles": 0, "yy": 1}[epilogue]
+        lbw = (N + 7) // 8 if yy else ((N + 31) // 32 + 3) & ~3
+        g = None
+        if gathered is not None:
+            g = np.ascontiguousarray(gathered, np.float32)
+            assert g.shape == (K, n)
+        d = None if dn is None else np.ascontiguousarray(dn, np.float32)
+        assert d is None or d.shape == (nrows,)
+        assign, ub, lb = np.empty(nrows, np.uint32), np.empty(nrows, np.float32), np.empty((nrows, lbw), np.float32)
+        self._chk(self._lib.isle_hip_assign_product_rows(self._h, yy, _p(P), nrows, K, ld, _p(rows), n, rows.shape[0], _p(g), _p(d), _p(Cc), N, ldc, lbw,
+                                                         _p(assign), _p(ub), _p(lb)))
+        return dict(assign=assign, ub=ub, lb=lb)
 
     def left_multiply_by_U(self, C_lowd, fetch=True):
         Cl = np.ascontiguousarray(C_lowd, dtype=np.float32)
```

Result: no change. 4.796 million, median of 6 (+0.3%).
